# yuz1wan/unified_video_action

Measured on AMD Instinct MI355X. Metric: train samples/sec (video+action step) at 1/2/4/8 MI355X; loss parity, higher is better.
Workload: dtype bf16; 1 GPU; pusht_video: PushT video_model (BASELINE configs[1]); step = frame select+resize -> KL-VAE encode (8 frames) -> mar_base MAR fwd/bwd (N=1024) -> diffusion loss -> backward -> fused AdamW + EMA -> LR step; dropout 0.1; model=UVA mar_base + KL-VAE f16, global_batch=32, seq_len=1024, parallelism=dp1

## Files before the change

include/uva_hip.h:

```cpp
#ifndef UVA_HIP_H
#define UVA_HIP_H
#include <hip/hip_runtime_api.h>

#ifdef __cplusplus
extern "C" {
#endif

#define UVA_DT_F32 0
#define UVA_DT_BF16 1
#define UVA_ACT_NONE 0
#define UVA_ACT_GELU 1
#define UVA_ACT_SILU 2
#define UVA_ACT_RELU 3

int uva_gemm(int in_dtype, int out_dtype, int ta, int tb, const void* A, const void* B, void* C, int M, int N,
             int K, long long lda, long long ldb, long long ldc, int batch, int batch_inner, long long sAo,
             long long sAi, long long sBo, long long sBi, long long sCo, long long sCi, const float* bias,
             const void* residual, long long ldr, long long sRo, long long sRi, void* aux, int act, float alpha,
             float beta, float drop_p, unsigned long long drop_seed, int res_dtype, const void* gate,
             long long ldg, int gate_dtype, int force_generic, float* workspace, long long ws_floats,
             hipStream_t stream);

long long uva_gemm_plan(int in_dtype, int ta, int tb, int M, int N, int K, int batch, int gn_prologue,
                        long long ws_floats);
int uva_gemm_set_persist(int on);
int uva_gemm4_set(int on, int force);
int uva_gemm8w_set(int on, int mode);
int uva_linear_gelu_drop(const void* X, const void* W, const float* bias, void* pre_out, void* out, int M, int N, int K,
                         float drop_p, unsigned long long seed, const void* plane, hipStream_t stream);
int uva_linear_drop_res(const void* X, const void* W, const float* bias, const float* R, float* out, int M, int N,
                        int K, float drop_p, unsigned long long seed, const void* plane, hipStream_t stream);
int uva_linear_dgelu_drop(const void* dY, const void* Wt, const void* pre, void* dpre, float* dbias, int accum_bias,
                          float* part, int M, int N, int K, float drop_p, unsigned long long seed, const void* plane,
                          hipStream_t stream);
int uva_layernorm_bwd_drop(const float* x, const float* w, const void* dy, const float* mean, const float* rstd,
                           const float* dx_base, float* dx, float* dw, float* db, int accum_wb, void* drop_out,
                           float drop_p, unsigned long long seed, float* dbias, int accum_dbias, float* workspace,
                           int rows, int D, hipStream_t stream);
long long uva_dropout_plane_words(long long n);
int uva_dropout_plane(void* plane, long long n, float drop_p, unsigned long long seed, hipStream_t stream);
long long uva_gemm4_plan(int M, int N, int K);
long long uva_gemm4_plan_tt(int M, int N, int K, long long ws_floats);
int uva_conv2d(int dtype, const void* in, const void* w, void* out, const float* bias, const void* residual, int Nimg,
               int Hin, int Win, int Ci, int Co, int ks, int stride, int pad_t, int pad_l, int Hout, int Wout,
               const float* gn_scale, const float* gn_shift, int gn_silu, int act, float* gn_part,
               int force_generic, hipStream_t stream);
int uva_pool4x4_cwh(int dtype, const void* in, void* out, int n, int C, hipStream_t stream);
int uva_pool4x4_relu_bwd(int dtype, const void* post, int gdtype, const void* gpool, void* dpre, int n, int C,
                         hipStream_t stream);
int uva_im2col3x3(int dtype, const void* in, void* cols, int n, int H, int W, int Ci, hipStream_t stream);
int uva_im2col3x3_tc(int dtype, const void* in, void* cols, int n, int H, int W, int Ci, hipStream_t stream);
int uva_pad_nhwc(int dtype, const void* in, void* out, int n, int H, int W, int C, int G, hipStream_t stream);
int uva_conv3x3_dw_scatter_add(const float* part, float* grad, int Co, int Ci, hipStream_t stream);
int uva_conv3x3_weight_layout(const float* w, int out_dtype, void* out, int Co, int Ci, int mode, hipStream_t stream);
int uva_conv3x3_halo_bn(int Nimg, int H, int W, int Ci, int Co);
int uva_conv3x3_halo(const void* in, const void* w, void* out, const float* bias, const void* residual, int Nimg,
                     int H, int W, int Ci, int Co, const float* gn_scale, const float* gn_shift, int gn_silu,
                     float* gn_part, hipStream_t stream);
int uva_conv3x3s2_ok(int Nimg, int Hin, int Win, int Ci, int Co);
int uva_conv3x3s2_halo(const void* in, const void* w, void* out, const float* bias, int Nimg, int Hin, int Win,
                       int Ci, int Co, float* gn_part, hipStream_t stream);
int uva_conv_in8(const void* in, const void* w, void* out, const float* bias, int Nimg, int H, int W,
                 float* gn_part, hipStream_t stream);

int uva_layernorm_fwd(int in_dtype, int out_dtype, const void* x, const float* w, const float* b, const void* scale,
                      const void* shift, long long ldm, void* y, float* mean, float* rstd, int rows, int D, float eps,
                      hipStream_t stream);
int uva_layernorm_bwd(int in_dtype, int out_dtype, const void* x, const float* w, const float* b, const void* scale,
                      long long ldm,
                      const void* dy, int dy_dtype, const float* mean, const float* rstd, const float* dx_base, float* dx,
                      int accum, void* dscale,
                      void* dshift, float* dw, float* db, int accum_wb, float* workspace, int rows, int D,
                      hipStream_t stream);
long long uva_layernorm_bwd_workspace(int rows, int D);

int uva_colsum(int dtype, const void* in, long long ld, float* out, int rows, int cols, int accum, float* workspace,
               hipStream_t stream);
long long uva_colsum_workspace(int rows, int cols);

int uva_softmax_fwd(int dtype, const void* S, void* P, void* Pd, long long rows, int L, float scale, float drop_p,
                    unsigned long long seed, hipStream_t stream);
int uva_softmax_bwd(int dtype, const void* P, const void* dPd, void* dS, long long rows, int L, float scale,
                    float drop_p, unsigned long long seed, hipStream_t stream);

int uva_cast(int sdt, const void* src, long long lds, int ddt, void* dst, long long ldd, long long rows, int cols,
             hipStream_t stream);
int uva_act_fwd(int xdt, const void* x, int ydt, void* y, long long n, int act, hipStream_t stream);
int uva_transpose_bf16(const void* src, void* dst, int rows, int cols, hipStream_t stream);
int uva_act_drop_fwd(int xdt, const void* x, int ydt, void* y, int rdt, const void* residual, long long n, int act,
                     float drop_p, unsigned long long seed, hipStream_t stream);
int uva_act_bwd(int pdt, const void* pre, int gdt, const void* dy, long long ld_dy, int xdt, void* dx,
                long long ld_dx, long long rows, int cols, int act, float drop_p, unsigned long long seed, int accum,
                hipStream_t stream);
int uva_act_bwd_bias(int pdt, const void* pre, int gdt, const void* dy, long long ld_dy, int xdt, void* dx,
                     long long ld_dx, long long rows, int cols, int act, float drop_p, unsigned long long seed,
                     int accum, float* dbias, int accum_bias, float* workspace, hipStream_t stream);
long long uva_act_bwd_bias_workspace(long long rows, int cols);
int uva_gate_bwd(const float* dout, int hdt, const void* h, int gtdt, const void* gate, long long ldg, int dhdt,
                 void* dh, void* dgate, long long rows, int cols, hipStream_t stream);
int uva_fill(float* p, long long n, float v, hipStream_t stream);

int uva_q_sample(const float* x0, const float* noise, const long long* t, const float* const* tables, int xdt,
                 void* xt, int rows, int C, hipStream_t stream);
int uva_timestep_features(const long long* t, const float* freqs, int odt, void* out, int rows, int half,
                          hipStream_t stream);
int uva_diffusion_loss(const float* x0, const float* noise, const long long* t, int odt, const void* out,
                       long long ld_out, const float* const* tables, float* loss_row, float* dl, int rows, int C,
                       hipStream_t stream);
int uva_weighted_mean(const float* l, const float* w, int n, float* res, hipStream_t stream);
int uva_loss_grad(const float* dl, const float* w, const float* wsum, const float* g_up, int ddt, void* dout,
                  long long ld, int rows, int C2, hipStream_t stream);

int uva_p_sample_step(int odt, const void* out, long long ld_out, const float* x, const float* noise,
                      const float* coef, float* x_new, int xdt, void* x_net, int clip, int rows, int C,
                      hipStream_t stream);

int uva_sampler_linear(int ln, const void* A, long long lda, const float* lnw, const float* lnb, const void* shift,
                       const void* scale, long long ldm, float eps, const void* W, const float* bias, int act,
                       const void* gate, long long ldg, const float* res, long long ldr, int odt, void* out,
                       long long ldo, int R, int N, int K, hipStream_t stream);

long long uva_sampler_persistent_workspace(int W);
int uva_sampler_persistent(int R, int C, int W, int depth, int S, int clip, float eps, const void* w1, const float* b1,
                           const void* w2, const float* b2, const float* lnw, const float* lnb, const void* win,
                           const float* bin, const void* wf, const float* bfin, const void* mod, long long ldmod,
                           const float* coef, const float* noise, const float* x0, float* x_out, void* work,
                           long long work_bytes, hipStream_t stream);
int uva_sampler_persistent_status(const void* work, unsigned* flag, hipStream_t stream);
int uva_sampler_persistent_test_hook(int no_publish);

int uva_adamw_ema(float* p, const float* g, float* m, float* v, float* ema, void* p_bf16, long long n,
                  long long n_decay, float lr, float b1, float b2, float eps, float wd, int step, float grad_scale,
                  float ema_decay, hipStream_t stream);
int uva_ema_update(float* ema, const float* p, long long n, float decay, hipStream_t stream);

long long uva_attn_fp8_workspace(int B, int N, int H);
int uva_attn_quant_fp8(void* qkv, void* workspace, int B, int N, int H, hipStream_t stream);
int uva_attn_fwd_fp8(const void* workspace, void* out, float* lse2, const void* mask, int B, int N, int H, float scale,
                     float drop_p, hipStream_t stream);

long long uva_attn_mask_bytes(int B, int N, int H);
long long uva_attn_bwd_workspace(int B, int N, int H, float drop_p);
int uva_attn_dropmask(void* mask, int B, int N, int H, float drop_p, unsigned long long seed, hipStream_t stream);
int uva_attn_fwd(const void* qkv, void* out, float* lse2, const void* mask, int B, int N, int H, float scale,
                 float drop_p, hipStream_t stream);
int uva_attn_bwd(const void* qkv, const void* out, const void* dout, const float* lse2, const void* mask, float* Dvec,
                 void* dqkv, void* workspace, int B, int N, int H, float scale, float drop_p, hipStream_t stream);
int uva_attn_bwd_bias(const void* qkv, const void* out, const void* dout, const float* lse2, const void* mask,
                      float* Dvec, void* dqkv, float* dbias, int accum, float* part, int B, int N, int H, float scale,
                      float drop_p, hipStream_t stream);

int uva_attn_hd_supported(int head_dim);
int uva_attn_fwd_hd(const void* qkv, void* out, float* lse2, const void* mask, int B, int N, int H, int head_dim,
                    float scale, float drop_p, hipStream_t stream);
long long uva_attn_bwd_hd_part_floats(int B, int N, int H, int head_dim);
int uva_attn_bwd_hd(const void* qkv, const void* out, const void* dout, const float* lse2, const void* mask,
                    float* Dvec, void* dqkv, float* dbias, int accum, float* part, int B, int N, int H, int head_dim,
                    float scale, float drop_p, hipStream_t stream);

int uva_resize_select(const float* img, int B, int T, int Hin, int Win, const int* sel, int nsel, int odt, void* out,
                      int Cpad, hipStream_t stream);
long long uva_groupnorm_workspace(int Nimg, int HW);
int uva_groupnorm_stats(int dtype, const void* x, int Nimg, int HW, int C, const float* gamma, const float* beta,
                        float eps, float* scale, float* shift, float* workspace, hipStream_t stream);
int uva_groupnorm_finalize_tiles(const float* part, int Nimg, int HW, int C, int tile_rows, const float* gamma,
                                 const float* beta, float eps, float* scale, float* shift, hipStream_t stream);
int uva_groupnorm_apply(const void* x, const float* scale, const float* shift, void* y, int Nimg, int HW, int C,
                        int do_silu, hipStream_t stream);
int uva_upsample_nearest2x(int dtype, const void* x, void* y, int n, int H, int W, int C, hipStream_t stream);
int uva_pusht_augment(const float* img, float* out, const float* params, int B, int T, int C, int S, int crop_size,
                      hipStream_t stream);
int uva_video_augment(const float* img, float* out, float* scratch, const float* params, int B, int T, int S,
                      hipStream_t stream);
int uva_posterior_sample(int mdt, const void* moments, const float* eps, float* z, int Nimg, float scale,
                         hipStream_t stream);

#ifdef __cplusplus
}
#endif
#endif
```

unified_video_action_amd/csrc/attention.hip:

```cpp
#include "common.h"

#ifndef UVA_ATT_PIPE
#define UVA_ATT_PIPE 0
#endif
#ifndef UVA_ATT_PIPE_DQ
#define UVA_ATT_PIPE_DQ 0
#endif
#ifndef UVA_ATT_PRIO
#define UVA_ATT_PRIO 1
#endif
#ifndef UVA_ATT_PRIO_BWD
#define UVA_ATT_PRIO_BWD 0
#endif
#define ATT_PRIO_HI() do { if (UVA_ATT_PRIO) __builtin_amdgcn_s_setprio(1); } while (0)
#define ATT_PRIO_LO() do { if (UVA_ATT_PRIO) __builtin_amdgcn_s_setprio(0); } while (0)
#define ATT_PRIO_HI_BWD() do { if (UVA_ATT_PRIO_BWD) __builtin_amdgcn_s_setprio(1); } while (0)
#define ATT_PRIO_LO_BWD() do { if (UVA_ATT_PRIO_BWD) __builtin_amdgcn_s_setprio(0); } while (0)
#define AT_LD 80
#define AT_TILE (64 * AT_LD)

__device__ __forceinline__ bf16x8 lds_row_frag(const bf16* lds, int row0, int ks) {
  const int l = threadIdx.x & 63;
  return *(const bf16x8*)(lds + (row0 + (l & 15)) * AT_LD + ks * 32 + 8 * (l >> 4));
}
// ... 690 lines not shown
#pragma unroll
    for (int i = 0; i < 8; ++i) {
      __builtin_amdgcn_sched_group_barrier(0x008, 1, 2);
      __builtin_amdgcn_sched_group_barrier(0x002, 10, 2);
    }
    __builtin_amdgcn_sched_barrier(0);
    dqk(1);
#else
    ATT_PRIO_HI_BWD();
#pragma unroll
    for (int ks = 0; ks < 2; ++ks)
#pragma unroll
      for (int kt = 0; kt < 4; ++kt) {
        const bf16x8 ka = lds_row_frag(sK[cur], kt * 16, ks);
        const bf16x8 va = lds_row_frag(sV[cur], kt * 16, ks);
#pragma unroll
        for (int qt = 0; qt < 2; ++qt) {
          s[kt][qt] = mfma16(ka, qf[qt][ks], s[kt][qt]);
          dp[kt][qt] = mfma16(va, of[qt][ks], dp[kt][qt]);
        }
      }
    ATT_PRIO_LO_BWD();
#pragma unroll
    for (int qt = 0; qt < 2; ++qt)
#pragma unroll
      for (int kt = 0; kt < 4; ++kt)
#pragma unroll
        for (int r = 0; r < 4; ++r) {
          const float p = exp2_fast(fmaf(s[kt][qt][r], c, -L[qt]));
          float dpt = dp[kt][qt][r];
          if (DROP) dpt = keep_bfe(dpt, mw[qt], kt * 4 + r);
          s[kt][qt][r] = p * (dpt - Dq[qt]);
        }
    ATT_PRIO_HI_BWD();
#pragma unroll
    for (int ks = 0; ks < 2; ++ks) {
      bf16x8 sb[2];
#pragma unroll
      for (int qt = 0; qt < 2; ++qt) sb[qt] = pack_pi(s[2 * ks][qt], s[2 * ks + 1][qt]);
#pragma unroll
      for (int dt = 0; dt < 4; ++dt) {
        const bf16x8 ka = lds_tr_frag(sK[cur], 32 * ks, 32 * ks + 16, dt * 16);
#pragma unroll
        for (int qt = 0; qt < 2; ++qt) dq[dt][qt] = mfma16(ka, sb[qt], dq[dt][qt]);
      }
    }
    ATT_PRIO_LO_BWD();
#endif
    if (more) {
      stage_store(sK[cur ^ 1], rk);
      stage_store(sV[cur ^ 1], rv);
      if (DROP) { mw[0] = mwn[0]; mw[1] = mwn[1]; }
    }
    lds_barrier();
    cur ^= 1;
  }
  if (cpart) {
    float* red = (float*)&sK[0][0];
#pragma unroll
    for (int dt = 0; dt < 4; ++dt)
#pragma unroll
      for (int r = 0; r < 4; ++r) {
        float sq = 0.f;
#pragma unroll
        for (int qt = 0; qt < 2; ++qt)
          sq += q0 + qt * 16 + li < N ? (float)(bf16)(dq[dt][qt][r] * scale) : 0.f;
        sq = row16_sum(sq);
        if (li == 0) red[w * 64 + dt * 16 + 4 * g + r] = sq;
      }
    __syncthreads();
    if (threadIdx.x < 64) {
      const int t = threadIdx.x;
      const float v = (red[t] + red[64 + t]) + (red[128 + t] + red[192 + t]);
      const long long rowp = (long long)b * gridDim.x + bx;
      cpart[rowp * (3LL * H * 64) + h * 64 + t] = v;
    }
  }
#pragma unroll
  for (int qt = 0; qt < 2; ++qt) {
    const int q = q0 + qt * 16 + li;
    if (q >= N) continue;
    bf16* qrow = dqkv + ((long long)b * N + q) * ld + h * 64;
#pragma unroll
    for (int dt = 0; dt < 4; ++dt) {
      bf16x4 a = {(bf16)(dq[dt][qt][0] * scale), (bf16)(dq[dt][qt][1] * scale), (bf16)(dq[dt][qt][2] * scale),
                  (bf16)(dq[dt][qt][3] * scale)};
      *(bf16x4*)(qrow + dt * 16 + 4 * g) = a;
    }
  }
}

extern "C" long long uva_attn_mask_bytes(int B, int N, int H) {
  return 2LL * B * H * (long long)N * (N / 64) * 8;
}

extern "C" long long uva_attn_bwd_workspace(int B, int N, int H, float drop_p) {
  (void)B; (void)N; (void)H; (void)drop_p;
  return 0;
}

extern "C" int uva_attn_dropmask(void* mask, int B, int N, int H, float drop_p, unsigned long long seed,
                                 hipStream_t s) {
  if (N % 64 != 0 || !(drop_p > 0.f) || mask == nullptr) return (int)hipErrorInvalidValue;
  uint32_t th;
  float ds;
  uva_drop_params(drop_p, &th, &ds);
  const int nt = N / 64;
  uint64_t* MQ = (uint64_t*)mask;
  uint64_t* MK = MQ + (long long)B * H * N * nt;
  const long long waves = (long long)B * H * nt * ((nt + MASK_TPW - 1) / MASK_TPW);
  if (waves > 0x7FFFFFFFLL) return (int)hipErrorInvalidValue;
  attn_mask_kernel<<<dim3((unsigned)((waves + 3) / 4)), 256, 0, s>>>(MQ, MK, N, nt, waves, th, seed);
  UVA_LAUNCH_CHECK();
  return 0;
}

extern "C" int uva_attn_fwd(const void* qkv, void* out, float* lse2, const void* mask, int B, int N, int H,
                            float scale, float drop_p, hipStream_t s) {
  if (N % 64 != 0) return (int)hipErrorInvalidValue;
  const bool drop = drop_p > 0.f;
  if (drop && mask == nullptr) return (int)hipErrorInvalidValue;
  uint32_t th;
  float ds;
  uva_drop_params(drop_p, &th, &ds);
  dim3 grid((N + 127) / 128, B * H);
  const float c = scale * 1.4426950408889634f;
  const uint64_t* MQ = drop ? (const uint64_t*)mask : nullptr;
  if (drop)
    attn_fwd_kernel<true, 64, 3><<<grid, 256, 0, s>>>((const bf16*)qkv, (bf16*)out, lse2, MQ, N, H, c, ds);
  else
    attn_fwd_kernel<false, 64, 3><<<grid, 256, 0, s>>>((const bf16*)qkv, (bf16*)out, lse2, nullptr, N, H, c, 1.0f);
  UVA_LAUNCH_CHECK();
  return 0;
}

static int attn_bwd_launch(const void* qkv, const void* out, const void* dout, const float* lse2, const void* mask,
                           float* Dvec, void* dqkv, int B, int N, int H, float scale, float drop_p, float* cpart,
                           hipStream_t s);

extern "C" int uva_attn_bwd(const void* qkv, const void* out, const void* dout, const float* lse2, const void* mask,
                            float* Dvec, void* dqkv, void* workspace, int B, int N, int H, float scale, float drop_p,
                            hipStream_t s) {
  (void)workspace;
  return attn_bwd_launch(qkv, out, dout, lse2, mask, Dvec, dqkv, B, N, H, scale, drop_p, nullptr, s);
}

int uva_colsum_final_launch(const float* part, int nrows, int cols, float* out, int accum, hipStream_t s);

extern "C" int uva_attn_bwd_bias(const void* qkv, const void* out, const void* dout, const float* lse2,
                                 const void* mask, float* Dvec, void* dqkv, float* dbias, int accum, float* part, int B,
                                 int N, int H, float scale, float drop_p, hipStream_t s) {
  if (!dbias || !part) return (int)hipErrorInvalidValue;
  int r = attn_bwd_launch(qkv, out, dout, lse2, mask, Dvec, dqkv, B, N, H, scale, drop_p, part, s);
  if (r) return r;
  return uva_colsum_final_launch(part, B * ((N + 127) / 128), 3 * H * 64, dbias, accum, s);
}

static int attn_bwd_launch(const void* qkv, const void* out, const void* dout, const float* lse2, const void* mask,
                           float* Dvec, void* dqkv, int B, int N, int H, float scale, float drop_p, float* cpart,
                           hipStream_t s) {
  if (N % 64 != 0) return (int)hipErrorInvalidValue;
  const bool drop = drop_p > 0.f;
  if (drop && mask == nullptr) return (int)hipErrorInvalidValue;
  uint32_t th;
  float ds;
  uva_drop_params(drop_p, &th, &ds);
  const long long rows = (long long)B * N * H;
  (void)rows;
  const int nt = N / 64;
  const uint64_t* MQ = (const uint64_t*)mask;
  const uint64_t* MK = drop ? MQ + (long long)B * H * N * nt : nullptr;
  const bf16* dO = (const bf16*)dout;
  dim3 grid((N + 127) / 128, B * H);
  const float c = scale * 1.4426950408889634f;
  const float sk = scale * ds;
  const bf16* O = (const bf16*)out;
  if (drop) {
    attn_bwd_dq_kernel<true><<<grid, 256, 0, s>>>((const bf16*)qkv, dO, O, lse2, Dvec, MQ, (bf16*)dqkv, N, H, sk, c,
                                                  1.0f / ds, cpart);
    attn_bwd_dkdv_kernel<true><<<grid, 256, 0, s>>>((const bf16*)qkv, dO, lse2, Dvec, MK, (bf16*)dqkv, N, H, sk, c, ds,
                                                    cpart);
  } else {
    attn_bwd_dq_kernel<false><<<grid, 256, 0, s>>>((const bf16*)qkv, dO, O, lse2, Dvec, nullptr, (bf16*)dqkv, N, H,
                                                   sk, c, 1.0f, cpart);
    attn_bwd_dkdv_kernel<false><<<grid, 256, 0, s>>>((const bf16*)qkv, dO, lse2, Dvec, nullptr, (bf16*)dqkv, N, H,
                                                     sk, c, ds, cpart);
  }
  UVA_LAUNCH_CHECK();
  return 0;
}
```

unified_video_action_amd/csrc/attention_hd.hip:

```cpp
#include "common.h"

namespace {

template <int HD> struct HdCfg;
template <> struct HdCfg<80> { static constexpr int KS = 3, DT = 5, LD = 112; };
template <> struct HdCfg<128> { static constexpr int KS = 4, DT = 8, LD = 144; };

template <int LD>
__device__ __forceinline__ bf16x8 row_frag(const bf16* lds, int row0, int ks) {
  const int l = threadIdx.x & 63;
  return *(const bf16x8*)(lds + (row0 + (l & 15)) * LD + ks * 32 + 8 * (l >> 4));
}

template <int LD>
__device__ __forceinline__ bf16x8 tr_frag(const bf16* lds, int rowA, int rowB, int col0) {
  const int l = threadIdx.x & 63, g = l >> 4, q = (l >> 2) & 3, p = l & 3;
  const bf16* a0 = lds + (rowA + 4 * g + q) * LD + col0 + 4 * p;
  const bf16* a1 = lds + (rowB + 4 * g + q) * LD + col0 + 4 * p;
  s16x4 lo = __builtin_amdgcn_ds_read_tr16_b64_v4i16(LDS_PTR(s16x4, a0));
  s16x4 hi = __builtin_amdgcn_ds_read_tr16_b64_v4i16(LDS_PTR(s16x4, a1));
  s16x8 v = {lo[0], lo[1], lo[2], lo[3], hi[0], hi[1], hi[2], hi[3]};
  return __builtin_bit_cast(bf16x8, v);
}

// ... 428 lines not shown
    for (int ks = 0; ks < 2; ++ks) {
      const bf16x8 pb = pack_pi(s[2 * ks], s[2 * ks + 1]);
      const bf16x8 sb = pack_pi(dp[2 * ks], dp[2 * ks + 1]);
#pragma unroll
      for (int dt = 0; dt < DT; ++dt) {
        const bf16x8 oa = tr_frag<LD>(sO[cur], 32 * ks, 32 * ks + 16, dt * 16);
        const bf16x8 qa = tr_frag<LD>(sQ[cur], 32 * ks, 32 * ks + 16, dt * 16);
        dv[dt] = mfma16(oa, pb, dv[dt]);
        dk[dt] = mfma16(qa, sb, dk[dt]);
      }
    }
    if (more) {
      rq.store(sQ[cur ^ 1]);
      ro.store(sO[cur ^ 1]);
      if (threadIdx.x < 64) { sL[cur ^ 1][threadIdx.x] = nl; sD[cur ^ 1][threadIdx.x] = nd; }
      if (DROP) mw = mwn;
    }
    __syncthreads();
    cur ^= 1;
  }
  if (cpart) {
    float* red = (float*)&sQ[0][0];
#pragma unroll
    for (int dt = 0; dt < DT; ++dt)
#pragma unroll
      for (int r = 0; r < 4; ++r) {
        float sk = ok ? (float)(bf16)(dk[dt][r] * scale) : 0.f;
        float sv = ok ? (float)(bf16)(dv[dt][r] * vsc) : 0.f;
        sk = row16_sum(sk);
        sv = row16_sum(sv);
        if (li == 0) {
          red[w * 2 * HD + dt * 16 + 4 * g + r] = sk;
          red[w * 2 * HD + HD + dt * 16 + 4 * g + r] = sv;
        }
      }
    __syncthreads();
    if (threadIdx.x < 2 * HD) {
      const int t = threadIdx.x;
      float v = 0.f;
#pragma unroll
      for (int ww = 0; ww < 8; ++ww) v += red[ww * 2 * HD + t];
      const long long rowp = (long long)b * gridDim.x + bx;
      cpart[rowp * (3LL * H * HD) + (t < HD ? H * HD + t : 2 * H * HD + t - HD) + h * HD] = v;
    }
  }
  if (ok) {
    bf16* krow = dqkv + ((long long)b * N + row) * ld + H * HD + h * HD;
    bf16* vrow = krow + H * HD;
#pragma unroll
    for (int dt = 0; dt < DT; ++dt) {
      bf16x4 a = {(bf16)(dk[dt][0] * scale), (bf16)(dk[dt][1] * scale), (bf16)(dk[dt][2] * scale),
                  (bf16)(dk[dt][3] * scale)};
      bf16x4 e = {(bf16)(dv[dt][0] * vsc), (bf16)(dv[dt][1] * vsc), (bf16)(dv[dt][2] * vsc),
                  (bf16)(dv[dt][3] * vsc)};
      *(bf16x4*)(krow + dt * 16 + 4 * g) = a;
      *(bf16x4*)(vrow + dt * 16 + 4 * g) = e;
    }
  }
}

template <int HD>
int fwd_launch(const void* qkv, void* out, float* lse2, const void* mask, int B, int N, int H, float scale, bool drop,
               float ds, hipStream_t s) {
  dim3 grid((N + 127) / 128, B * H);
  const float c = scale * 1.4426950408889634f;
  constexpr int lds = 4 * 64 * HdCfg<HD>::LD * (int)sizeof(bf16);
  static const bool once = [] {
    (void)hipFuncSetAttribute((const void*)attn_hd_fwd_kernel<HD, true>, hipFuncAttributeMaxDynamicSharedMemorySize, lds);
    (void)hipFuncSetAttribute((const void*)attn_hd_fwd_kernel<HD, false>, hipFuncAttributeMaxDynamicSharedMemorySize, lds);
    return true;
  }();
  (void)once;
  if (drop)
    attn_hd_fwd_kernel<HD, true><<<grid, 256, lds, s>>>((const bf16*)qkv, (bf16*)out, lse2, (const uint64_t*)mask, N, H,
                                                      c, ds);
  else
    attn_hd_fwd_kernel<HD, false><<<grid, 256, lds, s>>>((const bf16*)qkv, (bf16*)out, lse2, nullptr, N, H, c, 1.0f);
  UVA_LAUNCH_CHECK();
  return 0;
}

template <int HD>
int bwd_launch(const void* qkv, const void* out, const void* dout, const float* lse2, const void* mask, float* Dvec,
               void* dqkv, float* cpart, int B, int N, int H, float scale, bool drop, float ds, hipStream_t s) {
  const int nt = N / 64;
  const uint64_t* MQ = (const uint64_t*)mask;
  const uint64_t* MK = drop ? MQ + (long long)B * H * N * nt : nullptr;
  dim3 grid((N + 127) / 128, B * H);
  const float c = scale * 1.4426950408889634f;
  const float sk = scale * ds;
  constexpr int lds = 4 * 64 * HdCfg<HD>::LD * (int)sizeof(bf16);
  constexpr int ldsk = lds + 4 * 64 * (int)sizeof(float);
  static const bool once = [] {
    (void)hipFuncSetAttribute((const void*)attn_hd_bwd_dq_kernel<HD, true>, hipFuncAttributeMaxDynamicSharedMemorySize, lds);
    (void)hipFuncSetAttribute((const void*)attn_hd_bwd_dq_kernel<HD, false>, hipFuncAttributeMaxDynamicSharedMemorySize, lds);
    (void)hipFuncSetAttribute((const void*)attn_hd_bwd_dkdv_kernel<HD, true>, hipFuncAttributeMaxDynamicSharedMemorySize, ldsk);
    (void)hipFuncSetAttribute((const void*)attn_hd_bwd_dkdv_kernel<HD, false>, hipFuncAttributeMaxDynamicSharedMemorySize, ldsk);
    return true;
  }();
  (void)once;
  if (drop) {
    attn_hd_bwd_dq_kernel<HD, true><<<grid, 512, lds, s>>>((const bf16*)qkv, (const bf16*)dout, (const bf16*)out, lse2,
                                                         Dvec, MQ, (bf16*)dqkv, N, H, sk, c, 1.0f / ds, cpart);
    attn_hd_bwd_dkdv_kernel<HD, true><<<grid, 512, ldsk, s>>>((const bf16*)qkv, (const bf16*)dout, lse2, Dvec, MK,
                                                           (bf16*)dqkv, N, H, sk, c, ds, cpart);
  } else {
    attn_hd_bwd_dq_kernel<HD, false><<<grid, 512, lds, s>>>((const bf16*)qkv, (const bf16*)dout, (const bf16*)out, lse2,
                                                          Dvec, nullptr, (bf16*)dqkv, N, H, sk, c, 1.0f, cpart);
    attn_hd_bwd_dkdv_kernel<HD, false><<<grid, 512, ldsk, s>>>((const bf16*)qkv, (const bf16*)dout, lse2, Dvec, nullptr,
                                                            (bf16*)dqkv, N, H, sk, c, ds, cpart);
  }
  UVA_LAUNCH_CHECK();
  return 0;
}

}

int uva_colsum_final_launch(const float* part, int nrows, int cols, float* out, int accum, hipStream_t s);

extern "C" int uva_attn_hd_supported(int head_dim) { return head_dim == 80 || head_dim == 128; }

extern "C" long long uva_attn_bwd_hd_part_floats(int B, int N, int H, int head_dim) {
  return (long long)B * ((N + 127) / 128) * 3LL * H * head_dim;
}

extern "C" int uva_attn_fwd_hd(const void* qkv, void* out, float* lse2, const void* mask, int B, int N, int H,
                               int head_dim, float scale, float drop_p, hipStream_t s) {
  if (!uva_attn_hd_supported(head_dim) || N <= 0 || N % 64 != 0 || B <= 0 || H <= 0)
    return (int)hipErrorInvalidValue;
  const bool drop = drop_p > 0.f;
  if (drop && mask == nullptr) return (int)hipErrorInvalidValue;
  uint32_t th;
  float ds;
  uva_drop_params(drop_p, &th, &ds);
  return head_dim == 80 ? fwd_launch<80>(qkv, out, lse2, mask, B, N, H, scale, drop, ds, s)
                        : fwd_launch<128>(qkv, out, lse2, mask, B, N, H, scale, drop, ds, s);
}

extern "C" int uva_attn_bwd_hd(const void* qkv, const void* out, const void* dout, const float* lse2, const void* mask,
                               float* Dvec, void* dqkv, float* dbias, int accum, float* part, int B, int N, int H,
                               int head_dim, float scale, float drop_p, hipStream_t s) {
  if (!uva_attn_hd_supported(head_dim) || N <= 0 || N % 64 != 0 || B <= 0 || H <= 0)
    return (int)hipErrorInvalidValue;
  const bool drop = drop_p > 0.f;
  if (drop && mask == nullptr) return (int)hipErrorInvalidValue;
  if (dbias && !part) return (int)hipErrorInvalidValue;
  uint32_t th;
  float ds;
  uva_drop_params(drop_p, &th, &ds);
  float* cpart = dbias ? part : nullptr;
  const int r = head_dim == 80
                    ? bwd_launch<80>(qkv, out, dout, lse2, mask, Dvec, dqkv, cpart, B, N, H, scale, drop, ds, s)
                    : bwd_launch<128>(qkv, out, dout, lse2, mask, Dvec, dqkv, cpart, B, N, H, scale, drop, ds, s);
  if (r || !dbias) return r;
  return uva_colsum_final_launch(part, B * ((N + 127) / 128), 3 * H * head_dim, dbias, accum, s);
}
```

unified_video_action_amd/csrc/common.h:

```cpp
#pragma once
#include <hip/hip_runtime.h>
#include <math.h>
#include <stdint.h>

typedef __bf16 bf16;
typedef __attribute__((ext_vector_type(8))) __bf16 bf16x8;
typedef __attribute__((ext_vector_type(4))) __bf16 bf16x4;
typedef __attribute__((ext_vector_type(2))) float f32x2;
typedef __attribute__((ext_vector_type(4))) float f32x4;
typedef __attribute__((ext_vector_type(16))) float f32x16;
typedef __attribute__((ext_vector_type(4))) short s16x4;
typedef __attribute__((ext_vector_type(8))) short s16x8;

#define UVA_DT_F32 0
#define UVA_DT_BF16 1

#define LDS_PTR(T, p) ((__attribute__((address_space(3))) T*)(p))

__device__ __forceinline__ float to_f32(float x) { return x; }
__device__ __forceinline__ float to_f32(bf16 x) { return (float)x; }
template <typename T> __device__ __forceinline__ T from_f32(float x);
template <> __device__ __forceinline__ float from_f32<float>(float x) { return x; }
template <> __device__ __forceinline__ bf16 from_f32<bf16>(float x) { return (bf16)x; }

__device__ __forceinline__ float wave_sum(float v) {
#pragma unroll
  for (int o = 32; o > 0; o >>= 1) v += __shfl_xor(v, o, 64);
  return v;
}
__device__ __forceinline__ float wave_max(float v) {
#pragma unroll
  for (int o = 32; o > 0; o >>= 1) v = fmaxf(v, __shfl_xor(v, o, 64));
  return v;
}
__device__ __forceinline__ float group16_sum(float v) {
#pragma unroll
  for (int o = 8; o > 0; o >>= 1) v += __shfl_xor(v, o, 64);
  return v;
}
__device__ __forceinline__ float group16_max(float v) {
#pragma unroll
  for (int o = 8; o > 0; o >>= 1) v = fmaxf(v, __shfl_xor(v, o, 64));
  return v;
}

__host__ __device__ __forceinline__ uint32_t drop_key(uint64_t seed) {
  uint32_t k = (uint32_t)seed ^ (((uint32_t)(seed >> 32)) * 0x9E3779B1u);
  k ^= k >> 16;
  k *= 0x7feb352du;
  k ^= k >> 15;
  return k;
}
__host__ __device__ __forceinline__ uint32_t drop_first(uint32_t key, uint64_t pair) {
  return (uint32_t)pair ^ (key + __builtin_rotateleft32((uint32_t)(pair >> 32), 11));
}
__host__ __device__ __forceinline__ uint32_t drop_mix(uint32_t x) {
  x ^= x >> 16;
  x *= 0x7feb352du;
  x ^= x >> 15;
  x *= 0x846ca68bu;
  x ^= x >> 16;
  return x;
}
__host__ __device__ __forceinline__ uint32_t drop_hash(uint32_t key, uint64_t pair) {
  return drop_mix(drop_first(key, pair));
}
__host__ __device__ __forceinline__ bool dropout_keep(uint64_t seed, uint64_t idx, uint32_t thresh) {
  const uint32_t h = drop_hash(drop_key(seed), idx >> 1);
  return ((idx & 1) ? (h >> 16) : (h & 0xFFFFu)) >= thresh;
}
__device__ __forceinline__ void dropout_keep2(uint64_t seed, uint64_t idx_even, uint32_t thresh, bool& k0, bool& k1) {
  const uint32_t h = drop_hash(drop_key(seed), idx_even >> 1);
  k0 = (h & 0xFFFFu) >= thresh;
  k1 = (h >> 16) >= thresh;
}

static inline void uva_drop_params(float p, uint32_t* thresh, float* scale) {
  if (!(p > 0.f)) {
    *thresh = 0;
    *scale = 1.0f;
    return;
  }
  long t = lrintf(p * 65536.0f);
  if (t < 1) t = 1;
  if (t > 65535) t = 65535;
  *thresh = (uint32_t)t;
  *scale = 65536.0f / (float)(65536 - t);
}

#define ACT_NONE 0
#define ACT_GELU 1
#define ACT_SILU 2
#define ACT_RELU 3

__device__ __forceinline__ float erf_fast(float x) {
  const float ax = fabsf(x);
  const float t = __builtin_amdgcn_rcpf(fmaf(0.3275911f, ax, 1.0f));
  float p = fmaf(1.061405429f, t, -1.453152027f);
  p = fmaf(p, t, 1.421413741f);
  p = fmaf(p, t, -0.284496736f);
  p = fmaf(p, t, 0.254829592f);
  p *= t;
  const float e = __builtin_amdgcn_exp2f(-1.4426950408889634f * ax * ax);
  return copysignf(fmaf(-p, e, 1.0f), x);
}
__device__ __forceinline__ float gelu_erf(float x) { return 0.5f * x * (1.0f + erf_fast(x * 0.70710678118654752f)); }
__device__ __forceinline__ float gelu_erf_grad(float x) {
  const float e = __builtin_amdgcn_exp2f(-0.72134752044448170f * x * x);
  const float ax = fabsf(x) * 0.70710678118654752f;
  const float t = __builtin_amdgcn_rcpf(fmaf(0.3275911f, ax, 1.0f));
  float p = fmaf(1.061405429f, t, -1.453152027f);
  p = fmaf(p, t, 1.421413741f);
  p = fmaf(p, t, -0.284496736f);
  p = fmaf(p, t, 0.254829592f);
  p *= t;
  const float erf_ = copysignf(fmaf(-p, e, 1.0f), x);
  return fmaf(x, 0.39894228040143268f * e, fmaf(0.5f, erf_, 0.5f));
}
__device__ __forceinline__ float sigmoid_fast(float x) {
  return __builtin_amdgcn_rcpf(1.0f + __builtin_amdgcn_exp2f(-1.4426950408889634f * x));
}
__device__ __forceinline__ float silu(float x) { return x * sigmoid_fast(x); }
__device__ __forceinline__ float silu_grad(float x) {
  const float s = sigmoid_fast(x);
  return s * (1.0f + x * (1.0f - s));
}
__device__ __forceinline__ float apply_act(int act, float x) {
  switch (act) {
    case ACT_GELU: return gelu_erf(x);
    case ACT_SILU: return silu(x);
    case ACT_RELU: return x > 0.f ? x : 0.f;
    default: return x;
  }
}
__device__ __forceinline__ float act_grad(int act, float x) {
  switch (act) {
    case ACT_GELU: return gelu_erf_grad(x);
    case ACT_SILU: return silu_grad(x);
    case ACT_RELU: return x > 0.f ? 1.f : 0.f;
    default: return 1.f;
  }
}

__device__ __forceinline__ int xcd_remap(int bid, int nblk) {
  const int q = nblk / 8, r = nblk % 8, x = bid % 8;
  return (x < r ? x * (q + 1) : r * (q + 1) + (x - r) * q) + bid / 8;
}
__device__ __forceinline__ void xcd_grid2(int& bx, int& by) {
  const int gx = gridDim.x, T = gx * gridDim.y;
  const int L = blockIdx.y * gx + blockIdx.x;
  const int q = T / 8, r = T % 8, x = L % 8;
  const int Lp = (x < r ? x * (q + 1) : r * (q + 1) + (x - r) * q) + L / 8;
  bx = Lp % gx;
  by = Lp / gx;
}

__device__ __forceinline__ float row16_sum(float v) {
  v += __builtin_bit_cast(float, __builtin_amdgcn_update_dpp(0, __builtin_bit_cast(int, v), 0xB1, 0xF, 0xF, false));
  v += __builtin_bit_cast(float, __builtin_amdgcn_update_dpp(0, __builtin_bit_cast(int, v), 0x4E, 0xF, 0xF, false));
  v += __builtin_bit_cast(float, __builtin_amdgcn_update_dpp(0, __builtin_bit_cast(int, v), 0x124, 0xF, 0xF, false));
  v += __builtin_bit_cast(float, __builtin_amdgcn_update_dpp(0, __builtin_bit_cast(int, v), 0x128, 0xF, 0xF, false));
  return v;
}

__device__ __forceinline__ void lds_barrier() {
  asm volatile("s_waitcnt lgkmcnt(0)" ::: "memory");
  __builtin_amdgcn_s_barrier();
  asm volatile("" ::: "memory");
// ... 5 lines not shown
```

unified_video_action_amd/csrc/elementwise.hip:

```cpp
#include "common.h"

__device__ __forceinline__ float ldx(const void* p, int dt, long long i) {
  return dt == UVA_DT_BF16 ? (float)((const bf16*)p)[i] : ((const float*)p)[i];
}
__device__ __forceinline__ void stx(void* p, int dt, long long i, float v) {
  if (dt == UVA_DT_BF16) ((bf16*)p)[i] = (bf16)v;
  else ((float*)p)[i] = v;
}

#define GRID_STRIDE(i, n) for (long long i = (long long)blockIdx.x * blockDim.x + threadIdx.x; i < (n); i += (long long)gridDim.x * blockDim.x)

static inline dim3 ew_grid(long long n) {
  long long b = (n + 255) / 256;
  if (b > 8192) b = 8192;
  if (b < 1) b = 1;
  return dim3((unsigned)b);
}

__global__ void cast_kernel(const void* src, int sdt, long long lds, void* dst, int ddt, long long ldd, long long rows,
                            int cols) {
  GRID_STRIDE(i, rows * cols) {
    long long r = i / cols, c = i % cols;
    stx(dst, ddt, r * ldd + c, ldx(src, sdt, r * lds + c));
  }
}

__global__ void cast_f32_bf16_vec(const float* __restrict__ src, bf16* __restrict__ dst, long long n8) {
  GRID_STRIDE(i, n8) {
    float4 a = ((const float4*)src)[2 * i], b = ((const float4*)src)[2 * i + 1];
    bf16x8 o = {(bf16)a.x, (bf16)a.y, (bf16)a.z, (bf16)a.w, (bf16)b.x, (bf16)b.y, (bf16)b.z, (bf16)b.w};
    ((bf16x8*)dst)[i] = o;
  }
}

__global__ void act_fwd_kernel(const void* x, int xdt, void* y, int ydt, long long n, int act) {
  GRID_STRIDE(i, n) stx(y, ydt, i, apply_act(act, ldx(x, xdt, i)));
}

__global__ void act_bwd_kernel(const void* pre, int pdt, const void* dy, int gdt, void* dx, int xdt, long long rows,
                               int cols, long long ld_dy, long long ld_dx, int act, uint32_t thresh, float dscale,
                               uint64_t seed, int accum) {
  GRID_STRIDE(i, rows * (long long)cols) {
    long long r = i / cols, c = i % cols;
    float g = ldx(dy, gdt, r * ld_dy + c);
    if (thresh) g = dropout_keep(seed, (uint64_t)i, thresh) ? g * dscale : 0.f;
    if (act != ACT_NONE) g *= act_grad(act, ldx(pre, pdt, i));
    long long o = r * ld_dx + c;
    if (accum) g += ldx(dx, xdt, o);
    stx(dx, xdt, o, g);
  }
}

template <typename T>
__device__ __forceinline__ void ld8(const T* p, float (&v)[8]) {
  if constexpr (sizeof(T) == 2) {
    const bf16x8 x = *(const bf16x8*)p;
#pragma unroll
    for (int e = 0; e < 8; ++e) v[e] = (float)x[e];
  } else {
    const float4 a = *(const float4*)p, b = *(const float4*)(p + 4);
    v[0] = a.x; v[1] = a.y; v[2] = a.z; v[3] = a.w; v[4] = b.x; v[5] = b.y; v[6] = b.z; v[7] = b.w;
  }
}
template <typename T>
__device__ __forceinline__ void st8(T* p, const float (&v)[8]) {
  if constexpr (sizeof(T) == 2) {
    bf16x8 x;
#pragma unroll
    for (int e = 0; e < 8; ++e) x[e] = (bf16)v[e];
    *(bf16x8*)p = x;
  } else {
    *(float4*)p = make_float4(v[0], v[1], v[2], v[3]);
    *(float4*)(p + 4) = make_float4(v[4], v[5], v[6], v[7]);
  }
}

template <typename GT, typename XT>
__global__ void act_bwd_vec_kernel(const void* pre, int pdt, const GT* __restrict__ dy, XT* __restrict__ dx, int rows,
                                   int cols, long long ld_dy, long long ld_dx, int act, uint32_t thresh, float dscale,
                                   uint64_t seed, int accum) {
  const unsigned c8n = (unsigned)cols >> 3;
  const unsigned n8 = (unsigned)rows * c8n;
  for (unsigned i = blockIdx.x * blockDim.x + threadIdx.x; i < n8; i += gridDim.x * blockDim.x) {
    const unsigned r = i / c8n, c0 = (i - r * c8n) * 8;
    float g[8];
    ld8<GT>(dy + (long long)r * ld_dy + c0, g);
    if (thresh) {
      const uint64_t e0 = (uint64_t)r * cols + c0;
#pragma unroll
      for (int e = 0; e < 8; e += 2) {
        bool k0, k1;
        dropout_keep2(seed, e0 + e, thresh, k0, k1);
        g[e] = k0 ? g[e] * dscale : 0.f;
        g[e + 1] = k1 ? g[e + 1] * dscale : 0.f;
      }
    }
    if (act != ACT_NONE) {
      float pv[8];
      const long long pi = (long long)r * cols + c0;
      if (pdt == UVA_DT_BF16) ld8<bf16>((const bf16*)pre + pi, pv);
      else ld8<float>((const float*)pre + pi, pv);
#pragma unroll
      for (int e = 0; e < 8; ++e) g[e] *= act_grad(act, pv[e]);
    }
    XT* o = dx + (long long)r * ld_dx + c0;
    if (accum) {
      float prev[8];
      ld8<XT>(o, prev);
#pragma unroll
      for (int e = 0; e < 8; ++e) g[e] += prev[e];
    }
    st8<XT>(o, g);
  }
}

#define COLSUM_RPB 128
template <typename GT, typename XT, bool STORE>
__global__ __launch_bounds__(256) void act_bwd_colsum_kernel(const void* pre, int pdt, const GT* __restrict__ dy,
                                                             XT* __restrict__ dx, int rows, int cols, long long ld_dy,
                                                             long long ld_dx, int act, uint32_t thresh, float dscale,
                                                             uint64_t seed, int accum, float* __restrict__ part) {
  __shared__ float red[8][32 * 8 + 4];
  const int cg = threadIdx.x & 31, rl = threadIdx.x >> 5;
  const int c0 = (blockIdx.x * 32 + cg) * 8;
  const int r0 = blockIdx.y * COLSUM_RPB, r1 = min(rows, r0 + COLSUM_RPB);
  float s[8] = {0.f, 0.f, 0.f, 0.f, 0.f, 0.f, 0.f, 0.f};
  if (c0 < cols) {
#pragma unroll 4
    for (int r = r0 + rl; r < r1; r += 8) {
      float g[8];
      ld8<GT>(dy + (long long)r * ld_dy + c0, g);
      if (STORE) {
        if (thresh) {
          const uint64_t e0 = (uint64_t)r * cols + c0;
#pragma unroll
          for (int e = 0; e < 8; e += 2) {
            bool k0, k1;
            dropout_keep2(seed, e0 + e, thresh, k0, k1);
            g[e] = k0 ? g[e] * dscale : 0.f;
            g[e + 1] = k1 ? g[e + 1] * dscale : 0.f;
          }
        }
        if (act != ACT_NONE) {
          float pv[8];
          const long long pi = (long long)r * cols + c0;
          if (pdt == UVA_DT_BF16) ld8<bf16>((const bf16*)pre + pi, pv);
          else ld8<float>((const float*)pre + pi, pv);
#pragma unroll
          for (int e = 0; e < 8; ++e) g[e] *= act_grad(act, pv[e]);
        }
        XT* o = dx + (long long)r * ld_dx + c0;
        if (accum) {
          float prev[8];
          ld8<XT>(o, prev);
#pragma unroll
          for (int e = 0; e < 8; ++e) g[e] += prev[e];
        }
        st8<XT>(o, g);
#pragma unroll
        for (int e = 0; e < 8; ++e) s[e] += to_f32(from_f32<XT>(g[e]));
      } else {
#pragma unroll
        for (int e = 0; e < 8; ++e) s[e] += g[e];
      }
    }
  }
#pragma unroll
  for (int e = 0; e < 8; ++e) red[rl][cg * 8 + e] = s[e];
  __syncthreads();
  const int c = blockIdx.x * 256 + threadIdx.x;
  if (c < cols) {
    float t = 0.f;
#pragma unroll
    for (int j = 0; j < 8; ++j) t += red[j][threadIdx.x];
    part[(long long)blockIdx.y * cols + c] = t;
  }
}

__global__ __launch_bounds__(256) void colsum_final_kernel(const float* __restrict__ part, int nrows, int cols,
                                                           float* __restrict__ out, int accum) {
  __shared__ float red[8][33];
  const int cl = threadIdx.x & 31, rl = threadIdx.x >> 5;
  const int c = blockIdx.x * 32 + cl;
  float s = 0.f;
  if (c < cols) {
#pragma unroll 8
    for (int j = rl; j < nrows; j += 8) s += part[(long long)j * cols + c];
  }
  red[rl][cl] = s;
  __syncthreads();
  if (rl == 0 && c < cols) {
    float t = 0.f;
#pragma unroll
    for (int j = 0; j < 8; ++j) t += red[j][cl];
    out[c] = accum ? out[c] + t : t;
  }
}

extern "C" long long uva_act_bwd_bias_workspace(long long rows, int cols) {
  return (rows + COLSUM_RPB - 1) / COLSUM_RPB * (long long)cols;
}

extern "C" int uva_act_bwd_bias(int pdt, const void* pre, int gdt, const void* dy, long long ld_dy, int xdt, void* dx,
                                long long ld_dx, long long rows, int cols, int act, float drop_p,
                                unsigned long long seed, int accum, float* dbias, int accum_bias, float* workspace,
                                hipStream_t s) {
  if (rows <= 0 || cols <= 0) return 0;
  if (cols % 8 || ld_dy % 8 || ld_dx % 8 || rows >= (1ll << 31) ||
      (((uintptr_t)dy | (uintptr_t)dx | (uintptr_t)pre) % 16) || !dbias || !workspace)
    return (int)hipErrorInvalidValue;
  uint32_t th;
  float ds;
  uva_drop_params(drop_p, &th, &ds);
  const int nch = (int)((rows + COLSUM_RPB - 1) / COLSUM_RPB);
  dim3 g1((cols / 8 + 31) / 32, nch);
#define AB(GT, XT)                                                                                               \
  act_bwd_colsum_kernel<GT, XT, true><<<g1, 256, 0, s>>>(pre, pdt, (const GT*)dy, (XT*)dx, (int)rows, cols, ld_dy, \
                                                         ld_dx, act, th, ds, seed, accum, workspace)
  if (gdt == UVA_DT_BF16 && xdt == UVA_DT_BF16) AB(bf16, bf16);
  else if (gdt == UVA_DT_BF16) AB(bf16, float);
  else if (xdt == UVA_DT_BF16) AB(float, bf16);
  else AB(float, float);
#undef AB
  UVA_LAUNCH_CHECK();
  colsum_final_kernel<<<dim3((cols + 31) / 32), 256, 0, s>>>(workspace, nch, cols, dbias, accum_bias);
  UVA_LAUNCH_CHECK();
  return 0;
}

int uva_colsum_final_launch(const float* part, int nrows, int cols, float* out, int accum, hipStream_t s) {
  colsum_final_kernel<<<dim3((cols + 31) / 32), 256, 0, s>>>(part, nrows, cols, out, accum);
  return (int)hipGetLastError();
}

int uva_colsum_vec(int dtype, const void* in, long long ld, float* out, int rows, int cols, int accum,
                   float* workspace, hipStream_t s) {
  if (cols % 8 || ld % 8 || ((uintptr_t)in % 16) || !workspace || rows < 2 * COLSUM_RPB) return 0;
  const int nch = (rows + COLSUM_RPB - 1) / COLSUM_RPB;
  dim3 g1((cols / 8 + 31) / 32, nch);
  if (dtype == UVA_DT_BF16)
    act_bwd_colsum_kernel<bf16, bf16, false><<<g1, 256, 0, s>>>(nullptr, 0, (const bf16*)in, nullptr, rows, cols, ld,
                                                                0, 0, 0, 1.f, 0, 0, workspace);
  else
    act_bwd_colsum_kernel<float, float, false><<<g1, 256, 0, s>>>(nullptr, 0, (const float*)in, nullptr, rows, cols,
                                                                  ld, 0, 0, 0, 1.f, 0, 0, workspace);
  if (hipGetLastError() != hipSuccess) return -1;
  colsum_final_kernel<<<dim3((cols + 31) / 32), 256, 0, s>>>(workspace, nch, cols, out, accum);
  if (hipGetLastError() != hipSuccess) return -1;
  return 1;
}

__global__ void gate_bwd_kernel(const float* dout, const void* h, int hdt, const void* gate, int gtdt, long long ldg,
                                void* dh, int dhdt, void* dgate, long long rows, int cols) {
  GRID_STRIDE(i, rows * (long long)cols) {
    long long r = i / cols, c = i % cols;
    float d = dout[i];
    float g = ldx(gate, gtdt, r * ldg + c);
    stx(dgate, gtdt, r * ldg + c, d * ldx(h, hdt, i));
    stx(dh, dhdt, i, d * g);
  }
}

__global__ void fill_kernel(float* p, long long n, float v) {
  GRID_STRIDE(i, n) p[i] = v;
}

extern "C" int uva_cast(int sdt, const void* src, long long lds, int ddt, void* dst, long long ldd, long long rows,
                        int cols, hipStream_t s) {
  long long n = rows * cols;
  if (n <= 0) return 0;
  if (sdt == UVA_DT_F32 && ddt == UVA_DT_BF16 && lds == cols && ldd == cols && n % 8 == 0 &&
      ((uintptr_t)src % 16 == 0) && ((uintptr_t)dst % 16 == 0)) {
    cast_f32_bf16_vec<<<ew_grid(n / 8), 256, 0, s>>>((const float*)src, (bf16*)dst, n / 8);
  } else {
    cast_kernel<<<ew_grid(n), 256, 0, s>>>(src, sdt, lds, dst, ddt, ldd, rows, cols);
  }
  UVA_LAUNCH_CHECK();
  return 0;
}

__global__ __launch_bounds__(256) void transpose_bf16_kernel(const bf16* __restrict__ src, bf16* __restrict__ dst,
                                                             int rows, int cols) {
  __shared__ bf16 t[64][64 + 8];
  const int r0 = blockIdx.y * 64, c0 = blockIdx.x * 64;
  const int tid = threadIdx.x;
#pragma unroll
  for (int i = 0; i < 2; ++i) {
    const int id = tid + i * 256, rr = id >> 3, cc = (id & 7) * 8;
    const int r = r0 + rr, c = c0 + cc;
    bf16x8 v;
    if (r < rows && c + 8 <= cols) {
      v = *(const bf16x8*)(src + (long long)r * cols + c);
    } else {
#pragma unroll
      for (int e = 0; e < 8; ++e) v[e] = (r < rows && c + e < cols) ? src[(long long)r * cols + c + e] : (bf16)0.f;
    }
#pragma unroll
    for (int e = 0; e < 8; ++e) t[rr][cc + e] = v[e];
  }
  __syncthreads();
#pragma unroll
  for (int i = 0; i < 2; ++i) {
    const int id = tid + i * 256, cc = id >> 3, rr = (id & 7) * 8;
    const int c = c0 + cc, r = r0 + rr;
    bf16x8 v;
#pragma unroll
    for (int e = 0; e < 8; ++e) v[e] = t[rr + e][cc];
    if (c < cols && r + 8 <= rows) {
      *(bf16x8*)(dst + (long long)c * rows + r) = v;
    } else if (c < cols) {
#pragma unroll
      for (int e = 0; e < 8; ++e)
        if (r + e < rows) dst[(long long)c * rows + r + e] = v[e];
    }
  }
}

extern "C" int uva_transpose_bf16(const void* src, void* dst, int rows, int cols, hipStream_t s) {
  if (rows <= 0 || cols <= 0) return 0;
  if ((rows % 8) || (cols % 8) || (((uintptr_t)src | (uintptr_t)dst) % 16)) return (int)hipErrorInvalidValue;
  transpose_bf16_kernel<<<dim3((cols + 63) / 64, (rows + 63) / 64), 256, 0, s>>>((const bf16*)src, (bf16*)dst, rows,
                                                                                 cols);
  UVA_LAUNCH_CHECK();
  return 0;
}

template <typename TX, typename TY, typename TR>
__global__ __launch_bounds__(256) void act_drop_fwd_kernel(const TX* __restrict__ x, TY* __restrict__ y,
                                                           const TR* __restrict__ res, long long n8, int act,
                                                           uint32_t thresh, float dscale, uint64_t seed) {
  GRID_STRIDE(i, n8) {
    float v[8], r[8];
    ld8<TX>(x + i * 8, v);
    if (res) ld8<TR>(res + i * 8, r);
    switch (act) {
      case ACT_GELU:
#pragma unroll
        for (int e = 0; e < 8; ++e) v[e] = gelu_erf(v[e]);
        break;
      case ACT_SILU:
#pragma unroll
        for (int e = 0; e < 8; ++e) v[e] = silu(v[e]);
        break;
      case ACT_RELU:
#pragma unroll
        for (int e = 0; e < 8; ++e) v[e] = v[e] > 0.f ? v[e] : 0.f;
        break;
      default:
        break;
    }
    if (thresh) {
      bool keep[8];
#pragma unroll
      for (int e = 0; e < 8; e += 2) dropout_keep2(seed, (uint64_t)(i * 8 + e), thresh, keep[e], keep[e + 1]);
#pragma unroll
      for (int e = 0; e < 8; ++e) v[e] = keep[e] ? v[e] * dscale : 0.f;
    }
    if (res) {
#pragma unroll
      for (int e = 0; e < 8; ++e) v[e] += r[e];
    }
    st8<TY>(y + i * 8, v);
  }
}

extern "C" int uva_act_drop_fwd(int xdt, const void* x, int ydt, void* y, int rdt, const void* residual, long long n,
                                int act, float drop_p, unsigned long long seed, hipStream_t s) {
  if (n <= 0) return 0;
  if (n % 8 || (((uintptr_t)x | (uintptr_t)y | (uintptr_t)residual) % 16)) return (int)hipErrorInvalidValue;
  uint32_t th;
  float ds;
  uva_drop_params(drop_p, &th, &ds);
  const long long n8 = n / 8;
#define ADF(TX, TY, TR) \
  act_drop_fwd_kernel<TX, TY, TR><<<ew_grid(n8), 256, 0, s>>>((const TX*)x, (TY*)y, (const TR*)residual, n8, act, th, ds, seed)
  if (xdt == UVA_DT_BF16 && ydt == UVA_DT_BF16 && (!residual || rdt == UVA_DT_BF16)) ADF(bf16, bf16, bf16);
  else if (xdt == UVA_DT_BF16 && ydt == UVA_DT_F32 && (!residual || rdt == UVA_DT_F32)) ADF(bf16, float, float);
  else if (xdt == UVA_DT_F32 && ydt == UVA_DT_F32 && (!residual || rdt == UVA_DT_F32)) ADF(float, float, float);
  else return (int)hipErrorInvalidValue;
#undef ADF
  UVA_LAUNCH_CHECK();
  return 0;
}

__global__ __launch_bounds__(256) void drop_plane_kernel(uint32_t* __restrict__ plane, long long nwords, uint32_t key,
                                                         uint32_t thresh) {
  GRID_STRIDE(w, nwords) {
    const uint32_t f0 = drop_first(key, (uint64_t)w * 16);
    uint32_t bits = 0;
#pragma unroll
    for (int j = 0; j < 16; ++j) {
      const uint32_t h = drop_mix(f0 ^ (uint32_t)j);
      bits |= ((h & 0xFFFFu) >= thresh ? 1u : 0u) << (2 * j);
      bits |= ((h >> 16) >= thresh ? 1u : 0u) << (2 * j + 1);
    }
    plane[w] = bits;
  }
}

extern "C" long long uva_dropout_plane_words(long long n) { return (n + 31) / 32; }

extern "C" int uva_dropout_plane(void* plane, long long n, float drop_p, unsigned long long seed, hipStream_t s) {
  if (n <= 0) return 0;
  if (!plane || ((uintptr_t)plane % 4)) return (int)hipErrorInvalidValue;
  uint32_t th;
  float ds;
  uva_drop_params(drop_p, &th, &ds);
  const long long nw = (n + 31) / 32;
  drop_plane_kernel<<<ew_grid(nw), 256, 0, s>>>((uint32_t*)plane, nw, drop_key(seed), th);
  UVA_LAUNCH_CHECK();
  return 0;
}

extern "C" int uva_act_fwd(int xdt, const void* x, int ydt, void* y, long long n, int act, hipStream_t s) {
  if (n <= 0) return 0;
  act_fwd_kernel<<<ew_grid(n), 256, 0, s>>>(x, xdt, y, ydt, n, act);
  UVA_LAUNCH_CHECK();
  return 0;
}

extern "C" int uva_act_bwd(int pdt, const void* pre, int gdt, const void* dy, long long ld_dy, int xdt, void* dx,
                           long long ld_dx, long long rows, int cols, int act, float drop_p, unsigned long long seed,
                           int accum, hipStream_t s) {
  long long n = rows * cols;
  if (n <= 0) return 0;
  uint32_t th;
  float ds;
  uva_drop_params(drop_p, &th, &ds);
  const bool vec = cols % 8 == 0 && ld_dy % 8 == 0 && ld_dx % 8 == 0 && n / 8 < (1ll << 31) &&
                   (((uintptr_t)dy | (uintptr_t)dx | (uintptr_t)pre) % 16 == 0);
  if (vec) {
    const long long n8 = n / 8;
#define AB(GT, XT)                                                                                              \
  act_bwd_vec_kernel<GT, XT><<<ew_grid(n8), 256, 0, s>>>(pre, pdt, (const GT*)dy, (XT*)dx, (int)rows, cols, ld_dy, \
                                                         ld_dx, act, th, ds, seed, accum)
    if (gdt == UVA_DT_BF16 && xdt == UVA_DT_BF16) AB(bf16, bf16);
    else if (gdt == UVA_DT_BF16) AB(bf16, float);
    else if (xdt == UVA_DT_BF16) AB(float, bf16);
    else AB(float, float);
#undef AB
  } else {
    act_bwd_kernel<<<ew_grid(n), 256, 0, s>>>(pre, pdt, dy, gdt, dx, xdt, rows, cols, ld_dy, ld_dx, act, th, ds, seed,
                                              accum);
  }
  UVA_LAUNCH_CHECK();
  return 0;
}

extern "C" int uva_gate_bwd(const float* dout, int hdt, const void* h, int gtdt, const void* gate, long long ldg,
                            int dhdt, void* dh, void* dgate, long long rows, int cols, hipStream_t s) {
  long long n = rows * cols;
  if (n <= 0) return 0;
  gate_bwd_kernel<<<ew_grid(n), 256, 0, s>>>(dout, h, hdt, gate, gtdt, ldg, dh, dhdt, dgate, rows, cols);
  UVA_LAUNCH_CHECK();
  return 0;
}

extern "C" int uva_fill(float* p, long long n, float v, hipStream_t s) {
  if (n <= 0) return 0;
  fill_kernel<<<ew_grid(n), 256, 0, s>>>(p, n, v);
  UVA_LAUNCH_CHECK();
  return 0;
}
```

unified_video_action_amd/csrc/gemm8w.hip:

```cpp
#include "common.h"

#include <algorithm>
#include <type_traits>

typedef __attribute__((ext_vector_type(4))) unsigned u32x4;

#ifndef UVA_G8_DBG
#define UVA_G8_DBG 0
#endif
#ifndef UVA_G8_PREFETCH
#define UVA_G8_PREFETCH 1
#endif

namespace {

template <int FM_, int FN_, int NW_>
struct G8Cfg {
  static constexpr int FM = FM_, FN = FN_, NW = NW_;
  static constexpr int WM = NW / 2, WN = 2;
  static constexpr int BM = 16 * FM * WM, BN = 16 * FN * WN;
  static constexpr int GA = BM / (8 * NW), GB = BN / (8 * NW), G = GA + GB;
  static constexpr int A_BYTES = BM * 128, REGION = (BM + BN) * 128, RING = 2 * REGION;
  static_assert(GA * 8 * NW == BM && GB * 8 * NW == BN, "DMA split");
};
// ... 527 lines not shown
  const long long tiles = (long long)((M + G::BM - 1) / G::BM) * tn;
  const int grid = (int)std::min<long long>(tiles, (long long)g8_cus() * (8 / NW));
  const int lds = G::RING + (NW == 8 && ep.bias ? tn * G::BN * 4 : 0);
  static bool attr = false;
  if (!attr) {
    (void)hipFuncSetAttribute((const void*)gemm_8w<4, FN, NW, EPI, NDEF, TC, DM>,
                              hipFuncAttributeMaxDynamicSharedMemorySize, NW == 8 ? 163840 : G::RING);
    attr = true;
  }
  const int w1ok = (M % G::BM == 0) && (N % G::BN == 0);
  gemm_8w<4, FN, NW, EPI, NDEF, TC, DM><<<dim3(grid), 64 * NW, lds, s>>>((const bf16*)A, (const bf16*)B, (TC*)C, M, N,
                                                                       K, lda, ldb, ldc, ep, w1ok, 1, K, 0);
  UVA_LAUNCH_CHECK();
  return 0;
}

struct G8Split {
  int splits, kps, grid;
};
static G8Split g8_plan_tt(int M, int N, int K, long long ws_floats, bool need_ws) {
  G8Split p{0, 0, 0};
  if (K % 128 != 0 || K < 256 || M < 256 || N < 192) return p;
  const int cus = g8_cus();
  const long long tiles = (long long)((M + 255) / 256) * ((N + 191) / 192);
  int splits = (int)std::max<long long>(1, (cus + tiles / 2) / tiles);
  if (splits > K / 256) splits = K / 256;
  while (splits > 1 && (long long)splits * M * N > ws_floats) --splits;
  if (splits == 1 && need_ws && (long long)M * N > ws_floats) return p;
  int kps = K;
  for (; splits > 1; --splits) {
    kps = ((K + splits - 1) / splits + 127) / 128 * 128;
    const int sp = (K + kps - 1) / kps;
    if (K - (sp - 1) * kps >= 256) {
      splits = sp;
      break;
    }
  }
  if (splits <= 1) {
    splits = 1;
    kps = K;
  }
  p.splits = splits;
  p.kps = kps;
  p.grid = (int)std::min<long long>(tiles * splits, cus);
  return p;
}
static bool g8_nw4(int epi) { return (g_gemm8w_mode & 32) || (!(g_gemm8w_mode & 64) && epi == 3); }
static int g8_part_rows(int M) { return g8_nw4(3) ? (M + 127) / 128 * 2 : (M + 255) / 256 * 4; }

template <int FN, int EPI, int NDEF, typename TC, int NW = 8>
static int g8_launch(const void* A, const void* B, void* C, int M, int N, int K, int lda, int ldb, int ldc,
                     const G8Epi& ep, hipStream_t s) {
  if constexpr (EPI == 0) {
    return g8_launch1<FN, EPI, NDEF, TC, 0, NW>(A, B, C, M, N, K, lda, ldb, ldc, ep, s);
  } else {
    if (!ep.thresh) return g8_launch1<FN, EPI, NDEF, TC, 0, NW>(A, B, C, M, N, K, lda, ldb, ldc, ep, s);
    if (ep.plane) return g8_launch1<FN, EPI, NDEF, TC, 2, NW>(A, B, C, M, N, K, lda, ldb, ldc, ep, s);
    return g8_launch1<FN, EPI, NDEF, TC, 1, NW>(A, B, C, M, N, K, lda, ldb, ldc, ep, s);
  }
}

template <int EPI, typename TC>
static int g8_dispatch(const void* A, const void* B, void* C, int M, int N, int K, int lda, int ldb, int ldc,
                       const G8Epi& ep, hipStream_t s) {
  const int nd = (EPI == 0 && sizeof(TC) == 4) ? 0 : (g_gemm8w_mode >> 2) & 7;
#define G8L(FN_, ND_) g8_launch<FN_, EPI, ND_, TC>(A, B, C, M, N, K, lda, ldb, ldc, ep, s)
  if (g_gemm8w_mode & 32) return g8_launch<6, EPI, 0, TC, 4>(A, B, C, M, N, K, lda, ldb, ldc, ep, s);
  if (g_gemm8w_mode & 2) return (nd && K / 128 >= 3) ? G8L(4, 4) : G8L(4, 0);
  return G8L(6, 0);
#undef G8L
}

static bool g8_ok(const void* A, const void* B, const void* C, int M, int N, int K, long long lda, long long ldb,
                  long long ldc, int csize, const float* bias) {
  if (M < 256 || N < 192 || K < 256 || K % 128) return false;
  if (lda % 8 || ldb % 8 || ldc % 8 || N % 8 || lda < K || ldb < K) return false;
  if (((uintptr_t)A | (uintptr_t)B | (uintptr_t)C) % 16) return false;
  if (bias && ((uintptr_t)bias % 16)) return false;
  if (2.0 * (double)M * (double)lda >= 2147483648.0 || 2.0 * (double)N * (double)ldb >= 2147483648.0) return false;
  if ((double)M * (double)ldc * csize > (double)0x7fff0000) return false;
  const int tn = (N + 191) / 192;
  if (tn * 192 * 4 + 114688 > 163840) return false;
  return true;
}

static uint32_t g8_key(unsigned long long seed) { return drop_key(seed); }

extern "C" int uva_gemm8w_tt_try(const void* A, const void* B, float* C, int M, int N, int K, long long lda,
                                 long long ldb, long long ldc, float alpha, float beta, float* ws, long long ws_floats,
                                 int* reduce, hipStream_t s) {
  *reduce = 0;
  if (!(g_gemm8w_mode & 128)) return 0;
  if (M <= 0 || N <= 0 || K <= 0) return 0;
  if (lda % 8 || ldb % 8 || ldc % 8 || M % 8 || N % 8 || lda < M || ldb < N) return 0;
  if (((uintptr_t)A | (uintptr_t)B | (uintptr_t)C | (uintptr_t)ws) % 16) return 0;
  if (2.0 * (double)K * (double)lda >= 2147483648.0 || 2.0 * (double)K * (double)ldb >= 2147483648.0) return 0;
  const G8Split p = g8_plan_tt(M, N, K, ws ? ws_floats : 0, beta != 0.f);
  if (p.splits == 0) return 0;
  const bool direct = p.splits == 1 && beta == 0.f;
  if (direct ? (double)M * (double)ldc * 4.0 > (double)0x7fff0000
             : (double)p.splits * (double)M * (double)N * 4.0 > (double)0x7fff0000)
    return 0;
  if (!direct && !ws) return 0;
  using G = G8Cfg<4, 6, 8>;
  static bool attr = false;
  if (!attr) {
    (void)hipFuncSetAttribute((const void*)gemm_8w<4, 6, 8, 0, 0, float, 0, 1, 1>,
                              hipFuncAttributeMaxDynamicSharedMemorySize, 163840);
    attr = true;
  }
  const int w1ok = (M % G::BM == 0) && (N % G::BN == 0);
  G8Epi ep{nullptr, direct ? alpha : 1.f, nullptr, nullptr, nullptr, nullptr, 0u, 0u, 1.f};
  gemm_8w<4, 6, 8, 0, 0, float, 0, 1, 1><<<dim3(p.grid), 512, G::RING, s>>>(
      (const bf16*)A, (const bf16*)B, direct ? C : ws, M, N, K, (int)lda, (int)ldb, direct ? (int)ldc : N, ep, w1ok,
      p.splits, p.kps, (int)((long long)M * N * 4));
  UVA_LAUNCH_CHECK();
  if (!direct) *reduce = p.splits;
  return 1;
}

extern "C" int uva_gemm8w_try(int out_dtype, const void* A, const void* B, void* C, int M, int N, int K, long long lda,
                              long long ldb, long long ldc, const float* bias, float alpha, hipStream_t s) {
  if (!g_gemm8w_on) return 0;
  if (!g8_ok(A, B, C, M, N, K, lda, ldb, ldc, out_dtype == UVA_DT_BF16 ? 2 : 4, bias)) return 0;
  G8Epi ep{bias, alpha, nullptr, nullptr, nullptr, nullptr, 0u, 0u, 1.f};
  const int r = out_dtype == UVA_DT_BF16
                    ? g8_dispatch<0, bf16>(A, B, C, M, N, K, (int)lda, (int)ldb, (int)ldc, ep, s)
                    : g8_dispatch<0, float>(A, B, C, M, N, K, (int)lda, (int)ldb, (int)ldc, ep, s);
  return r ? -r : 1;
}

extern "C" int uva_gemm8w_set(int on, int mode) {
  const int prev = g_gemm8w_on | (g_gemm8w_mode << 1);
  if (on != -2) g_gemm8w_on = on;
  if (mode != -2) g_gemm8w_mode = mode;
  return prev;
}

extern "C" int uva_linear_gelu_drop(const void* X, const void* W, const float* bias, void* pre_out, void* out, int M,
                                    int N, int K, float drop_p, unsigned long long seed, const void* plane,
                                    hipStream_t s) {
  if (!g8_ok(X, W, out, M, N, K, K, K, N, 2, bias) || ((uintptr_t)pre_out % 16)) return 0;
  uint32_t th;
  float ds;
  uva_drop_params(drop_p, &th, &ds);
  if (plane && (N % 32 || !th || ((uintptr_t)plane % 4))) return (int)-hipErrorInvalidValue;
  G8Epi ep{bias, 1.f, pre_out, nullptr, nullptr, (const uint32_t*)plane, th ? g8_key(seed) : 0u, th, ds};
  const int r = g8_dispatch<1, bf16>(X, W, out, M, N, K, K, K, N, ep, s);
  return r ? -r : 1;
}

int uva_colsum_final_launch(const float* part, int nrows, int cols, float* out, int accum, hipStream_t s);

extern "C" int uva_linear_dgelu_drop(const void* dY, const void* Wt, const void* pre, void* dpre, float* dbias,
                                     int accum_bias, float* part, int M, int N, int K, float drop_p,
                                     unsigned long long seed, const void* plane, hipStream_t s) {
  if (!g8_ok(dY, Wt, dpre, M, N, K, K, K, N, 2, nullptr) || (((uintptr_t)pre | (uintptr_t)part) % 16) || !dbias)
    return 0;
  uint32_t th;
  float ds;
  uva_drop_params(drop_p, &th, &ds);
  if (plane && (N % 32 || !th || ((uintptr_t)plane % 4))) return (int)-hipErrorInvalidValue;
  G8Epi ep{nullptr, 1.f, (void*)pre, nullptr, part, (const uint32_t*)plane, th ? g8_key(seed) : 0u, th, ds};
  int r = g8_nw4(3) ? g8_launch<6, 3, 0, bf16, 4>(dY, Wt, dpre, M, N, K, K, K, N, ep, s)
                                : g8_launch<6, 3, 0, bf16>(dY, Wt, dpre, M, N, K, K, K, N, ep, s);
  if (r) return -r;
  r = uva_colsum_final_launch(part, g8_part_rows(M), N, dbias, accum_bias, s);
  return r ? -r : 1;
}

extern "C" int uva_linear_drop_res(const void* X, const void* W, const float* bias, const float* R, float* out, int M,
                                   int N, int K, float drop_p, unsigned long long seed, const void* plane,
                                   hipStream_t s) {
  if (!g8_ok(X, W, out, M, N, K, K, K, N, 4, bias) || ((uintptr_t)R % 16)) return 0;
  uint32_t th;
  float ds;
  uva_drop_params(drop_p, &th, &ds);
  if (plane && (N % 32 || !th || ((uintptr_t)plane % 4))) return (int)-hipErrorInvalidValue;
  G8Epi ep{bias, 1.f, nullptr, R, nullptr, (const uint32_t*)plane, th ? g8_key(seed) : 0u, th, ds};
  const int r = g8_dispatch<2, float>(X, W, out, M, N, K, K, K, N, ep, s);
  return r ? -r : 1;
}
```

unified_video_action_amd/csrc/norm.hip:

```cpp
#include "common.h"

template <typename T>
__device__ __forceinline__ void load_vec(const T* p, float* out, int n) {
#pragma unroll
  for (int i = 0; i < n; ++i) out[i] = to_f32(p[i]);
}

template <int VEC, typename T>
__device__ __forceinline__ void ldv(const T* p, float (&o)[VEC]) {
  if constexpr (VEC == 4 && sizeof(T) == 4) {
    float4 v = *(const float4*)p;
    o[0] = v.x; o[1] = v.y; o[2] = v.z; o[3] = v.w;
  } else if constexpr (VEC == 4 && sizeof(T) == 2) {
    bf16x4 v = *(const bf16x4*)p;
    o[0] = (float)v[0]; o[1] = (float)v[1]; o[2] = (float)v[2]; o[3] = (float)v[3];
  } else {
#pragma unroll
    for (int i = 0; i < VEC; ++i) o[i] = to_f32(p[i]);
  }
}

template <int VEC, typename T>
__device__ __forceinline__ void stv(T* p, const float (&o)[VEC]) {
  if constexpr (VEC == 4 && sizeof(T) == 4) {
    *(float4*)p = make_float4(o[0], o[1], o[2], o[3]);
  } else if constexpr (VEC == 4 && sizeof(T) == 2) {
    bf16x4 v = {(bf16)o[0], (bf16)o[1], (bf16)o[2], (bf16)o[3]};
    *(bf16x4*)p = v;
  } else {
#pragma unroll
    for (int i = 0; i < VEC; ++i) p[i] = from_f32<T>(o[i]);
  }
}

template <int VEC>
__device__ __forceinline__ int col_of(int c, int lane, int v) { return (c * 64 + lane) * VEC + v; }

template <typename TI, typename TO, int VEC, int NC>
__global__ __launch_bounds__(256) void ln_fwd(const TI* __restrict__ x, const float* __restrict__ w,
                                              const float* __restrict__ b, const TO* __restrict__ scale,
                                              const TO* __restrict__ shift, long long ldm, TO* __restrict__ y,
                                              float* __restrict__ mean_out, float* __restrict__ rstd_out, int rows,
                                              int D, float eps) {
  const int lane = threadIdx.x & 63;
  const int row = blockIdx.x * 4 + (threadIdx.x >> 6);
  if (row >= rows) return;
  const TI* xr = x + (long long)row * D;
  float v[NC][VEC];
  float s = 0.f;
#pragma unroll
  for (int c = 0; c < NC; ++c) {
    int col = col_of<VEC>(c, lane, 0);
    if (col < D) {
      ldv<VEC>(xr + col, v[c]);
    } else {
#pragma unroll
      for (int i = 0; i < VEC; ++i) v[c][i] = 0.f;
    }
#pragma unroll
    for (int i = 0; i < VEC; ++i) s += v[c][i];
  }
  const float mean = wave_sum(s) / D;
  float q = 0.f;
#pragma unroll
  for (int c = 0; c < NC; ++c)
#pragma unroll
    for (int i = 0; i < VEC; ++i) {
      int col = col_of<VEC>(c, lane, i);
      float d = (col < D) ? v[c][i] - mean : 0.f;
      q += d * d;
    }
  const float var = wave_sum(q) / D;
  const float rstd = 1.0f / sqrtf(var + eps);
  if (lane == 0) {
    mean_out[row] = mean;
    rstd_out[row] = rstd;
  }
  TO* yr = y + (long long)row * D;
#pragma unroll
  for (int c = 0; c < NC; ++c) {
    int col0 = col_of<VEC>(c, lane, 0);
    if (col0 >= D) continue;
    float o[VEC];
    float sc[VEC], sh[VEC], wv[VEC], bv[VEC];
    if (scale) {
      ldv<VEC>(scale + (long long)row * ldm + col0, sc);
      ldv<VEC>(shift + (long long)row * ldm + col0, sh);
    }
    if (w) ldv<VEC>(w + col0, wv);
    if (b) ldv<VEC>(b + col0, bv);
#pragma unroll
    for (int i = 0; i < VEC; ++i) {
      float h = (v[c][i] - mean) * rstd;
      if (w) h = h * wv[i];
      if (b) h = h + bv[i];
      if (scale) h = h * (1.0f + sc[i]) + sh[i];
      o[i] = h;
    }
    stv<VEC>(yr + col0, o);
  }
}

template <int VEC, typename T>
struct RawVec {
  T v[VEC];
};
template <int VEC, typename T>
__device__ __forceinline__ RawVec<VEC, T> ldraw(const T* p) {
  RawVec<VEC, T> r;
  if constexpr (VEC == 4 && sizeof(T) == 4) {
    *(float4*)r.v = *(const float4*)p;
  } else if constexpr (VEC == 4 && sizeof(T) == 2) {
    *(bf16x4*)r.v = *(const bf16x4*)p;
  } else {
#pragma unroll
    for (int i = 0; i < VEC; ++i) r.v[i] = p[i];
  }
  return r;
}

struct LnDrop {
  bf16* out;
  float* part;
  uint32_t key, thresh;
  float dscale;
};

template <typename TI, typename TO, int VEC, int NC, typename TD, bool DROPO = false>
__global__ __launch_bounds__(256) void ln_bwd(const TI* __restrict__ x, const float* __restrict__ w,
                                              const float* __restrict__ b, const TO* __restrict__ scale, long long ldm,
                                              const TD* __restrict__ dy, const float* __restrict__ mean_in,
                                              const float* __restrict__ rstd_in, const float* dx_base,
                                              float* dx, int accum,
                                              TO* __restrict__ dscale, TO* __restrict__ dshift,
                                              float* __restrict__ dw_part, float* __restrict__ db_part, int rows,
                                              int D, int rows_per_block, LnDrop ldrop = LnDrop{}) {
  constexpr int RW = VEC * NC * 64 > 1024 ? VEC * NC * 64 : 1024;
  __shared__ float red_w[4][RW];
  __shared__ float red_b[4][RW];
  __shared__ float red_d[DROPO ? 4 : 1][DROPO ? RW : 1];
  float pd[NC][VEC];
  if constexpr (DROPO) {
#pragma unroll
    for (int c = 0; c < NC; ++c)
#pragma unroll
      for (int i = 0; i < VEC; ++i) pd[c][i] = 0.f;
  }
  const int lane = threadIdx.x & 63, wid = threadIdx.x >> 6;
  float pw[NC][VEC], pb[NC][VEC];
#pragma unroll
  for (int c = 0; c < NC; ++c)
#pragma unroll
    for (int i = 0; i < VEC; ++i) pw[c][i] = pb[c][i] = 0.f;
// ... 25 lines not shown
      const int col0 = col_of<VEC>(c, lane, 0);
      if (col0 < D) {
        R.x[c] = ldraw<VEC>(x + (long long)row * D + col0);
        R.d[c] = ldraw<VEC>(dy + (long long)row * D + col0);
        if (addsrc) R.a[c] = ldraw<VEC>(addsrc + (long long)row * D + col0);
      }
    }
  };
  auto process = [&](int row, const Row& R, Row& L, bool pf) __attribute__((always_inline)) {
    if (pf && row + 4 < r1) load_row(row + 4, L);
    const float mean = R.mean, rstd = R.rstd;
    float xh[NC][VEC], g[NC][VEC];
    float s1 = 0.f, s2 = 0.f;
#pragma unroll
    for (int c = 0; c < NC; ++c) {
      int col0 = col_of<VEC>(c, lane, 0);
      if (col0 >= D) {
#pragma unroll
        for (int i = 0; i < VEC; ++i) xh[c][i] = g[c][i] = 0.f;
        continue;
      }
      float sc[VEC];
      if (scale) ldv<VEC>(scale + (long long)row * ldm + col0, sc);
      float ds[VEC], dsh[VEC];
#pragma unroll
      for (int i = 0; i < VEC; ++i) {
        xh[c][i] = (to_f32(R.x[c].v[i]) - mean) * rstd;
        const float dv = to_f32(R.d[c].v[i]);
        float da = dv;
        if (scale) {
          float ya = w ? xh[c][i] * wv[c][i] + (b ? bv[c][i] : 0.f) : xh[c][i];
          da = dv * (1.0f + sc[i]);
          ds[i] = dv * ya;
          dsh[i] = dv;
        }
        if (w) {
          pw[c][i] += da * xh[c][i];
          pb[c][i] += da;
          g[c][i] = da * wv[c][i];
        } else {
          g[c][i] = da;
        }
        s1 += g[c][i];
        s2 += g[c][i] * xh[c][i];
      }
      if (scale) {
        stv<VEC>(dscale + (long long)row * ldm + col0, ds);
        stv<VEC>(dshift + (long long)row * ldm + col0, dsh);
      }
    }
    const float m1 = wave_sum(s1) / D, m2 = wave_sum(s2) / D;
#pragma unroll
    for (int c = 0; c < NC; ++c) {
      int col0 = col_of<VEC>(c, lane, 0);
      if (col0 >= D) continue;
      float o[VEC];
#pragma unroll
      for (int i = 0; i < VEC; ++i) {
        float d = rstd * (g[c][i] - m1 - xh[c][i] * m2);
        o[i] = addsrc ? R.a[c].v[i] + d : d;
      }
      stv<VEC>(dx + (long long)row * D + col0, o);
      if constexpr (DROPO) {
        static_assert(VEC % 2 == 0, "pairs");
        const unsigned long long e0 = (unsigned long long)row * (unsigned)D + (unsigned)col0;
        float q[VEC];
#pragma unroll
        for (int i = 0; i < VEC; i += 2) {
          const uint32_t h = drop_hash(ldrop.key, (e0 + i) >> 1);
          q[i] = (h & 0xFFFFu) >= ldrop.thresh ? o[i] * ldrop.dscale : 0.f;
          q[i + 1] = (h >> 16) >= ldrop.thresh ? o[i + 1] * ldrop.dscale : 0.f;
        }
        bf16 qb[VEC];
#pragma unroll
        for (int i = 0; i < VEC; ++i) {
          qb[i] = (bf16)q[i];
          pd[c][i] += (float)qb[i];
        }
        if constexpr (VEC == 4) {
          bf16x4 v4 = {qb[0], qb[1], qb[2], qb[3]};
          *(bf16x4*)(ldrop.out + (long long)row * D + col0) = v4;
        } else {
#pragma unroll
          for (int i = 0; i < VEC; ++i) ldrop.out[(long long)row * D + col0 + i] = qb[i];
        }
      }
    }
  };
  Row ra, rb;
  int row = r0 + wid;
  if constexpr (NC <= 3) {
    if (row < r1) load_row(row, ra);
    for (; row < r1; row += 8) {
      process(row, ra, rb, true);
      if (row + 4 < r1) process(row + 4, rb, ra, true);
    }
  } else {
    for (; row < r1; row += 4) {
      load_row(row, ra);
      process(row, ra, rb, false);
    }
  }
  if (dw_part) {
#pragma unroll
    for (int c = 0; c < NC; ++c)
#pragma unroll
      for (int i = 0; i < VEC; ++i) {
        int col = col_of<VEC>(c, lane, i);
        if (col < D) {
          red_w[wid][col] = pw[c][i];
          red_b[wid][col] = pb[c][i];
        }
      }
    __syncthreads();
    for (int col = threadIdx.x; col < D; col += 256) {
      dw_part[(long long)blockIdx.x * D + col] = red_w[0][col] + red_w[1][col] + red_w[2][col] + red_w[3][col];
      db_part[(long long)blockIdx.x * D + col] = red_b[0][col] + red_b[1][col] + red_b[2][col] + red_b[3][col];
    }
  }
  if constexpr (DROPO) {
#pragma unroll
    for (int c = 0; c < NC; ++c)
#pragma unroll
      for (int i = 0; i < VEC; ++i) {
        const int col = col_of<VEC>(c, lane, i);
        if (col < D) red_d[wid][col] = pd[c][i];
      }
    __syncthreads();
    for (int col = threadIdx.x; col < D; col += 256)
      ldrop.part[(long long)blockIdx.x * D + col] = red_d[0][col] + red_d[1][col] + red_d[2][col] + red_d[3][col];
  }
}

template <typename T>
__global__ __launch_bounds__(256) void colsum_kernel(const T* __restrict__ in, long long ld, float* __restrict__ out,
                                                     int rows, int cols, int accum) {
  __shared__ float red[4][64];
  const int cl = threadIdx.x & 63, rl = threadIdx.x >> 6;
  const int col = blockIdx.x * 64 + cl;
  float s = 0.f;
  if (col < cols)
    for (int r = rl; r < rows; r += 4) s += to_f32(in[(long long)r * ld + col]);
  red[rl][cl] = s;
  __syncthreads();
  if (rl == 0 && col < cols) {
    float t = red[0][cl] + red[1][cl] + red[2][cl] + red[3][cl];
    out[col] = accum ? out[col] + t : t;
  }
}

__global__ __launch_bounds__(256) void colsum_partials_kernel(const float* __restrict__ p0, const float* __restrict__ p1,
                                                              float* __restrict__ o0, float* __restrict__ o1, int rows,
                                                              int cols, int accum) {
  const float* in = blockIdx.y ? p1 : p0;
  float* out = blockIdx.y ? o1 : o0;
  __shared__ float4 red[32][8];
  const int cg = threadIdx.x & 7, rl = threadIdx.x >> 3;
  const int c = blockIdx.x * 32 + cg * 4;
  float4 acc = make_float4(0.f, 0.f, 0.f, 0.f);
  if (c < cols) {
#pragma unroll 4
    for (int r = rl; r < rows; r += 32) {
      const float4 v = *(const float4*)(in + (long long)r * cols + c);
      acc.x += v.x; acc.y += v.y; acc.z += v.z; acc.w += v.w;
    }
  }
  red[rl][cg] = acc;
  __syncthreads();
  if (rl < 4 && c < cols) {
    const int cc = c + rl;
    float t = 0.f;
#pragma unroll 8
    for (int k = 0; k < 32; ++k) {
      const float4 v = red[k][cg];
      t += rl == 0 ? v.x : (rl == 1 ? v.y : (rl == 2 ? v.z : v.w));
    }
    out[cc] = accum ? out[cc] + t : t;
  }
}

static void colsum_partials(const float* p0, const float* p1, float* o0, float* o1, int rows, int cols, int accum,
                            hipStream_t stream) {
  if (cols % 4 == 0) {
    colsum_partials_kernel<<<dim3((cols + 31) / 32, p1 ? 2 : 1), 256, 0, stream>>>(p0, p1, o0, o1, rows, cols, accum);
  } else {
    colsum_kernel<float><<<dim3((cols + 63) / 64), 256, 0, stream>>>(p0, cols, o0, rows, cols, accum);
    if (p1) colsum_kernel<float><<<dim3((cols + 63) / 64), 256, 0, stream>>>(p1, cols, o1, rows, cols, accum);
  }
}

template <typename T>
__global__ __launch_bounds__(256) void colsum_part_kernel(const T* __restrict__ in, long long ld,
                                                          float* __restrict__ part, int rows, int cols,
                                                          int rows_per_block) {
  __shared__ float red[4][64];
  const int cl = threadIdx.x & 63, rl = threadIdx.x >> 6;
  const int col = blockIdx.x * 64 + cl;
  const int r0 = blockIdx.y * rows_per_block, r1 = min(rows, r0 + rows_per_block);
  float s = 0.f;
  if (col < cols)
    for (int r = r0 + rl; r < r1; r += 4) s += to_f32(in[(long long)r * ld + col]);
  red[rl][cl] = s;
  __syncthreads();
  if (rl == 0 && col < cols) part[(long long)blockIdx.y * cols + col] = red[0][cl] + red[1][cl] + red[2][cl] + red[3][cl];
}

template <typename T>
__global__ __launch_bounds__(256) void softmax_fwd_kernel(const T* __restrict__ S, T* __restrict__ P,
                                                          T* __restrict__ Pd, long long rows, int L, float scale,
                                                          uint32_t thresh, float dscale, uint64_t seed) {
  const int lane = threadIdx.x & 63;
  const long long row = (long long)blockIdx.x * 4 + (threadIdx.x >> 6);
  if (row >= rows) return;
  const T* s = S + row * L;
  float m = -INFINITY;
  for (int j = lane; j < L; j += 64) m = fmaxf(m, to_f32(s[j]) * scale);
  m = wave_max(m);
  float sum = 0.f;
  for (int j = lane; j < L; j += 64) sum += __expf(to_f32(s[j]) * scale - m);
  sum = wave_sum(sum);
  const float inv = 1.0f / sum;
  for (int j = lane; j < L; j += 64) {
    float p = __expf(to_f32(s[j]) * scale - m) * inv;
    P[row * L + j] = from_f32<T>(p);
    if (Pd) {
      float pd = dropout_keep(seed, (uint64_t)(row * L + j), thresh) ? p * dscale : 0.f;
      Pd[row * L + j] = from_f32<T>(pd);
    }
  }
}

template <typename T>
__global__ __launch_bounds__(256) void softmax_bwd_kernel(const T* __restrict__ P, const T* __restrict__ dPd,
                                                          T* __restrict__ dS, long long rows, int L, float scale,
                                                          uint32_t thresh, float dscale, uint64_t seed) {
  const int lane = threadIdx.x & 63;
  const long long row = (long long)blockIdx.x * 4 + (threadIdx.x >> 6);
  if (row >= rows) return;
  float dot = 0.f;
  for (int j = lane; j < L; j += 64) {
    float dp = to_f32(dPd[row * L + j]);
    if (thresh) dp = dropout_keep(seed, (uint64_t)(row * L + j), thresh) ? dp * dscale : 0.f;
    dot += dp * to_f32(P[row * L + j]);
  }
  dot = wave_sum(dot);
  for (int j = lane; j < L; j += 64) {
    float dp = to_f32(dPd[row * L + j]);
    if (thresh) dp = dropout_keep(seed, (uint64_t)(row * L + j), thresh) ? dp * dscale : 0.f;
    dS[row * L + j] = from_f32<T>(scale * to_f32(P[row * L + j]) * (dp - dot));
  }
}

#define DISPATCH_LNB(TI, TO, TD, ...)                                                       \
  do {                                                                                       \
    if (D == 768) {                                                                          \
      ln_bwd<TI, TO, 4, 3, TD><<<grid, 256, 0, stream>>>(__VA_ARGS__);                       \
    } else if (D % 256 == 0 && D <= 1024) {                                                  \
      ln_bwd<TI, TO, 4, 4, TD><<<grid, 256, 0, stream>>>(__VA_ARGS__);                       \
    } else if (D <= 1024) {                                                                  \
      ln_bwd<TI, TO, 1, 16, TD><<<grid, 256, 0, stream>>>(__VA_ARGS__);                      \
    } else if (D % 256 == 0 && D <= 1280) {  \
      ln_bwd<TI, TO, 4, 5, TD><<<grid, 256, 0, stream>>>(__VA_ARGS__);                       \
    } else if (D % 256 == 0 && D <= 2048) {                                                  \
      ln_bwd<TI, TO, 4, 8, TD><<<grid, 256, 0, stream>>>(__VA_ARGS__);                       \
    } else {                                                                                 \
      return (int)hipErrorInvalidValue;                                                      \
    }                                                                                        \
  } while (0)

#define DISPATCH_LN(KERNEL, TI, TO, ...)                                                    \
  do {                                                                                       \
    if (D == 768) {  \
      KERNEL<TI, TO, 4, 3><<<grid, 256, 0, stream>>>(__VA_ARGS__);                           \
    } else if (D % 256 == 0 && D <= 1024) {                                                  \
      KERNEL<TI, TO, 4, 4><<<grid, 256, 0, stream>>>(__VA_ARGS__);                           \
    } else if (D <= 1024) {                                                                  \
      KERNEL<TI, TO, 1, 16><<<grid, 256, 0, stream>>>(__VA_ARGS__);                          \
    } else if (D % 256 == 0 && D <= 1280) {  \
      KERNEL<TI, TO, 4, 5><<<grid, 256, 0, stream>>>(__VA_ARGS__);                           \
    } else if (D % 256 == 0 && D <= 2048) {                                                  \
      KERNEL<TI, TO, 4, 8><<<grid, 256, 0, stream>>>(__VA_ARGS__);                           \
    } else {                                                                                 \
      return (int)hipErrorInvalidValue;                                                      \
    }                                                                                        \
  } while (0)

extern "C" int uva_layernorm_fwd(int in_dtype, int out_dtype, const void* x, const float* w, const float* b,
                                 const void* scale, const void* shift, long long ldm, void* y, float* mean,
                                 float* rstd, int rows, int D, float eps, hipStream_t stream) {
  if (rows <= 0) return 0;
  dim3 grid((rows + 3) / 4);
  if (in_dtype == UVA_DT_F32 && out_dtype == UVA_DT_F32)
    DISPATCH_LN(ln_fwd, float, float, (const float*)x, w, b, (const float*)scale, (const float*)shift, ldm,
                (float*)y, mean, rstd, rows, D, eps);
  else if (in_dtype == UVA_DT_F32 && out_dtype == UVA_DT_BF16)
    DISPATCH_LN(ln_fwd, float, bf16, (const float*)x, w, b, (const bf16*)scale, (const bf16*)shift, ldm, (bf16*)y,
                mean, rstd, rows, D, eps);
  else if (in_dtype == UVA_DT_BF16 && out_dtype == UVA_DT_BF16)
    DISPATCH_LN(ln_fwd, bf16, bf16, (const bf16*)x, w, b, (const bf16*)scale, (const bf16*)shift, ldm, (bf16*)y,
                mean, rstd, rows, D, eps);
  else
    return (int)hipErrorInvalidValue;
  UVA_LAUNCH_CHECK();
  return 0;
}

extern "C" int uva_layernorm_bwd(int in_dtype, int out_dtype, const void* x, const float* w, const float* b,
                                 const void* scale,
                                 long long ldm, const void* dy, int dy_dtype, const float* mean, const float* rstd,
                                 const float* dx_base, float* dx, int accum, void* dscale, void* dshift, float* dw, float* db, int accum_wb,
                                 float* workspace, int rows, int D, hipStream_t stream) {
  if (rows <= 0) return 0;
  const int rpb = 64;
  const int nblk = (rows + rpb - 1) / rpb;
  dim3 grid(nblk);
  float* pw = dw ? workspace : nullptr;
  float* pb = dw ? workspace + (long long)nblk * D : nullptr;
#define LNB_DY(TI, TO)                                                                                          \
  do {                                                                                                          \
    if (dy_dtype == UVA_DT_BF16)                                                                                \
      DISPATCH_LNB(TI, TO, bf16, (const TI*)x, w, b, (const TO*)scale, ldm, (const bf16*)dy, mean, rstd, dx_base, \
                   dx, accum, (TO*)dscale, (TO*)dshift, pw, pb, rows, D, rpb);                                  \
    else                                                                                                        \
      DISPATCH_LNB(TI, TO, float, (const TI*)x, w, b, (const TO*)scale, ldm, (const float*)dy, mean, rstd,        \
                   dx_base, dx, accum, (TO*)dscale, (TO*)dshift, pw, pb, rows, D, rpb);                         \
  } while (0)
  if (in_dtype == UVA_DT_F32 && out_dtype == UVA_DT_F32)
    LNB_DY(float, float);
  else if (in_dtype == UVA_DT_F32 && out_dtype == UVA_DT_BF16)
    LNB_DY(float, bf16);
  else if (in_dtype == UVA_DT_BF16 && out_dtype == UVA_DT_BF16)
    LNB_DY(bf16, bf16);
  else
    return (int)hipErrorInvalidValue;
#undef LNB_DY
  UVA_LAUNCH_CHECK();
  if (dw) {
    colsum_partials(pw, db ? pb : nullptr, dw, db, nblk, D, accum_wb, stream);
    UVA_LAUNCH_CHECK();
  }
  return 0;
}

extern "C" int uva_layernorm_bwd_drop(const float* x, const float* w, const void* dy, const float* mean,
                                      const float* rstd, const float* dx_base, float* dx, float* dw, float* db,
                                      int accum_wb, void* drop_out, float drop_p, unsigned long long seed,
                                      float* dbias, int accum_dbias, float* workspace, int rows, int D,
                                      hipStream_t stream) {
  if (rows <= 0) return 0;
  if (D != 768 || !w || !dw || !db || !drop_out || !dbias || !workspace || ((uintptr_t)drop_out % 8))
    return (int)hipErrorInvalidValue;
  const int rpb = 64;
  const int nblk = (rows + rpb - 1) / rpb;
  float* pw = workspace;
  float* pb = workspace + (long long)nblk * D;
  float* pd = workspace + 2LL * nblk * D;
  uint32_t th;
  float ds;
  uva_drop_params(drop_p, &th, &ds);
  LnDrop ld{(bf16*)drop_out, pd, drop_key(seed), th, ds};
  ln_bwd<float, float, 4, 3, bf16, true><<<dim3(nblk), 256, 0, stream>>>(
      x, w, nullptr, (const float*)nullptr, 0, (const bf16*)dy, mean, rstd, dx_base, dx, 0, (float*)nullptr,
      (float*)nullptr, pw, pb, rows, D, rpb, ld);
  UVA_LAUNCH_CHECK();
  colsum_partials(pw, pb, dw, db, nblk, D, accum_wb, stream);
  UVA_LAUNCH_CHECK();
  colsum_partials(pd, nullptr, dbias, nullptr, nblk, D, accum_dbias, stream);
  UVA_LAUNCH_CHECK();
  return 0;
}

extern "C" long long uva_layernorm_bwd_workspace(int rows, int D) {
  const int rpb = 64;
  return (long long)((rows + rpb - 1) / rpb) * D * 2;
}

int uva_colsum_vec(int dtype, const void* in, long long ld, float* out, int rows, int cols, int accum,
                   float* workspace, hipStream_t s);

extern "C" int uva_colsum(int dtype, const void* in, long long ld, float* out, int rows, int cols, int accum,
                          float* workspace, hipStream_t stream) {
  if (rows <= 0 || cols <= 0) return 0;
  {
    const int r = uva_colsum_vec(dtype, in, ld, out, rows, cols, accum, workspace, stream);
    if (r < 0) return (int)hipErrorLaunchFailure;
    if (r > 0) return 0;
  }
  const int rpb = 512;
  int nb = (rows + rpb - 1) / rpb;
  dim3 g1((cols + 63) / 64, nb);
  if (nb > 1 && workspace) {
    if (dtype == UVA_DT_BF16) colsum_part_kernel<bf16><<<g1, 256, 0, stream>>>((const bf16*)in, ld, workspace, rows, cols, rpb);
    else colsum_part_kernel<float><<<g1, 256, 0, stream>>>((const float*)in, ld, workspace, rows, cols, rpb);
    colsum_partials(workspace, nullptr, out, nullptr, nb, cols, accum, stream);
  } else {
    if (dtype == UVA_DT_BF16) colsum_kernel<bf16><<<dim3((cols + 63) / 64), 256, 0, stream>>>((const bf16*)in, ld, out, rows, cols, accum);
    else colsum_kernel<float><<<dim3((cols + 63) / 64), 256, 0, stream>>>((const float*)in, ld, out, rows, cols, accum);
  }
  UVA_LAUNCH_CHECK();
  return 0;
}

extern "C" long long uva_colsum_workspace(int rows, int cols) {
  return (long long)((rows + 127) / 128) * cols;
}

extern "C" int uva_softmax_fwd(int dtype, const void* S, void* P, void* Pd, long long rows, int L, float scale,
                               float drop_p, unsigned long long seed, hipStream_t stream) {
  if (rows <= 0) return 0;
  uint32_t th;
  float ds;
  uva_drop_params(drop_p, &th, &ds);
  dim3 grid((unsigned)((rows + 3) / 4));
  if (dtype == UVA_DT_BF16)
    softmax_fwd_kernel<bf16><<<grid, 256, 0, stream>>>((const bf16*)S, (bf16*)P, th ? (bf16*)Pd : nullptr, rows, L, scale, th, ds, seed);
  else
    softmax_fwd_kernel<float><<<grid, 256, 0, stream>>>((const float*)S, (float*)P, th ? (float*)Pd : nullptr, rows, L, scale, th, ds, seed);
  UVA_LAUNCH_CHECK();
  return 0;
}

extern "C" int uva_softmax_bwd(int dtype, const void* P, const void* dPd, void* dS, long long rows, int L, float scale,
                               float drop_p, unsigned long long seed, hipStream_t stream) {
  if (rows <= 0) return 0;
  uint32_t th;
  float ds;
  uva_drop_params(drop_p, &th, &ds);
  dim3 grid((unsigned)((rows + 3) / 4));
  if (dtype == UVA_DT_BF16)
    softmax_bwd_kernel<bf16><<<grid, 256, 0, stream>>>((const bf16*)P, (const bf16*)dPd, (bf16*)dS, rows, L, scale, th, ds, seed);
  else
    softmax_bwd_kernel<float><<<grid, 256, 0, stream>>>((const float*)P, (const float*)dPd, (float*)dS, rows, L, scale, th, ds, seed);
  UVA_LAUNCH_CHECK();
  return 0;
}
```

unified_video_action_amd/model/autoregressive/functional.py:

```python
import math

import torch

from ...native import ops
from ...runtime import RT, cdt

F32 = torch.float32


def as_dtype(t, dtype):
    if t.dtype == dtype and t.is_contiguous():
        return t
    t = t.contiguous()
    if t.dtype == dtype:
        return t
    out = torch.empty(t.shape, dtype=dtype, device=t.device)
    ops.cast(t, out)
    return out


def compute_weight(p):
    if cdt() == F32:
        return p.detach()
    sh = getattr(p, "_uva_shadow", None)
    if sh is not None and getattr(p, "_uva_shadow_owner", None) == id(p):
        return sh
    key = (p._version, p.data_ptr(), RT.param_gen if getattr(p, "_uva_raw_updated", False) else 0)
    if sh is None or getattr(p, "_uva_shadow_ver", None) != key:
        sh = as_dtype(p.detach(), cdt())
        p._uva_shadow = sh
        p._uva_shadow_ver = key
    return sh


def compute_weight_t(p):
    ev = getattr(p, "_uva_t_event", None)
    if ev is not None:
        torch.cuda.current_stream().wait_event(ev)
        p._uva_t_event = None
    w = compute_weight(p)
    key = (p._version, p.data_ptr(), RT.param_gen)
    t = getattr(p, "_uva_shadow_t", None)
    if t is None or getattr(p, "_uva_shadow_t_ver", None) != key:
        if t is None or t.shape != (w.shape[1], w.shape[0]):
            t = torch.empty(w.shape[1], w.shape[0], dtype=w.dtype, device=w.device)
        ops.transpose_bf16(w, t)
        p._uva_shadow_t = t
        p._uva_shadow_t_ver = key
    return t


def prefetch_weight_t(params, side):
    if cdt() != torch.bfloat16:
        return
    todo = []
    for p in params:
        w = compute_weight(p)
        key = (p._version, p.data_ptr(), RT.param_gen)
        if getattr(p, "_uva_shadow_t_ver", None) == key and getattr(p, "_uva_t_event", None) is None:
            continue
        t = getattr(p, "_uva_shadow_t", None)
        if t is None or t.shape != (w.shape[1], w.shape[0]):
            t = torch.empty(w.shape[1], w.shape[0], dtype=w.dtype, device=w.device)
            p._uva_shadow_t = t
        todo.append((p, w, t, key))
    side.wait_stream(torch.cuda.current_stream())
    for p, w, t, key in todo:
        with torch.cuda.stream(side):
            ops.transpose_bf16(w, t)
            ev = torch.cuda.Event()
            ev.record(side)
        p._uva_shadow_t_ver = key
        p._uva_t_event = ev


def linear_bias(x, p, b, out):
    ops.linear(x, compute_weight(p), out, bias=b.detach())


def linear_dx_w(dy, p, dx):
    if cdt() == torch.bfloat16:
        ops.linear(dy, compute_weight_t(p), dx)
    else:
        ops.linear_dx(dy, compute_weight(p), dx)


def grad_buf(p):
    if p.grad is None:
        p.grad = torch.zeros_like(p)
    return p.grad


def _seed():
    return RT.next_seed()


class LinearFn(torch.autograd.Function):

    @staticmethod
    def forward(ctx, x, weight, bias, act, drop_p, out_dtype, residual):
        xc = as_dtype(x, cdt())
        w = compute_weight(weight)
        if w.dim() != 2:
            w = w.reshape(w.shape[0], -1)
        M, N = xc.shape[0], weight.shape[0]
        out = torch.empty(M, N, dtype=out_dtype, device=x.device)
        aux = torch.empty(M, N, dtype=out_dtype, device=x.device) if act != "none" else None
        seed = _seed() if drop_p > 0 else 0
        ops.linear(xc, w, out, bias=None if bias is None else bias.detach(), act=act, aux=aux,
                   residual=residual, drop_p=drop_p, seed=seed)
        ctx.save_for_backward(xc, weight, bias, aux)
        ctx.cfg = (act, drop_p, seed, x.dtype, residual is not None)
        return out

    @staticmethod
    def backward(ctx, g):
        xc, weight, bias, aux = ctx.saved_tensors
        act, drop_p, seed, xdt, has_res = ctx.cfg
        M, N = g.shape
        fused_bias = False
        if act != "none" or drop_p > 0:
            dpre = torch.empty(M, N, dtype=cdt(), device=g.device)
            if bias is not None and N % 8 == 0:
                ops.act_bwd_bias(aux, g.contiguous(), dpre, grad_buf(bias), act, drop_p=drop_p, seed=seed)
                fused_bias = True
            else:
                ops.act_bwd(aux, g.contiguous(), dpre, act, drop_p=drop_p, seed=seed)
        else:
            dpre = as_dtype(g, cdt())
        gx = None
        if ctx.needs_input_grad[0]:
            gx = torch.empty(M, xc.shape[1], dtype=F32, device=g.device)
            ops.linear_dx(dpre, compute_weight(weight).reshape(N, -1), gx)
            gx = as_dtype(gx, xdt)
        ops.linear_dw(dpre, xc, grad_buf(weight).view(N, -1))
        if bias is not None and not fused_bias:
            ops.colsum(dpre, grad_buf(bias), accum=True)
        return gx, None, None, None, None, None, (g if has_res else None)


def linear(x, layer, act="none", drop_p=0.0, out_dtype=F32, residual=None):
    shp = x.shape
    y = LinearFn.apply(x.reshape(-1, shp[-1]), layer.weight, layer.bias, act, drop_p, out_dtype,
                       None if residual is None else residual.reshape(-1, layer.weight.shape[0]))
    return y.reshape(*shp[:-1], layer.weight.shape[0])


class LayerNormFn(torch.autograd.Function):
    @staticmethod
    def forward(ctx, x, weight, bias, eps, out_dtype):
        x = x.contiguous()
        M, D = x.shape
        y = torch.empty(M, D, dtype=out_dtype, device=x.device)
        mean = torch.empty(M, dtype=F32, device=x.device)
        rstd = torch.empty(M, dtype=F32, device=x.device)
        ops.layernorm_fwd(x, None if weight is None else weight.detach(),
                          None if bias is None else bias.detach(), y, mean, rstd, eps)
        ctx.save_for_backward(x, weight, bias, mean, rstd)
        return y

    @staticmethod
    def backward(ctx, g):
        x, weight, bias, mean, rstd = ctx.saved_tensors
        dy = as_dtype(g, F32)
        dx = torch.empty(x.shape, dtype=F32, device=x.device)
        ops.layernorm_bwd(x, None if weight is None else weight.detach(), dy, mean, rstd, dx, accum=False,
                          dw=None if weight is None else grad_buf(weight),
                          db=None if bias is None else grad_buf(bias))
        return as_dtype(dx, x.dtype), None, None, None, None


def layer_norm(x, ln, out_dtype=F32):
    shp = x.shape
    y = LayerNormFn.apply(x.reshape(-1, shp[-1]), ln.weight, ln.bias, ln.eps, out_dtype)
    return y.reshape(shp)


class ActFn(torch.autograd.Function):
    @staticmethod
    def forward(ctx, x, act, out_dtype):
        x = x.contiguous()
        y = torch.empty(x.shape, dtype=out_dtype, device=x.device)
        ops.act_fwd(x, y, act)
        ctx.save_for_backward(x)
        ctx.act = act
        return y

    @staticmethod
    def backward(ctx, g):
        (x,) = ctx.saved_tensors
        dx = torch.empty(x.shape, dtype=x.dtype, device=x.device)
        ops.act_bwd(x.reshape(-1, x.shape[-1]), g.contiguous().reshape(-1, x.shape[-1]),
                    dx.reshape(-1, x.shape[-1]), ctx.act)
        return dx, None, None


def _attn_mat_fwd(qkv, B, N, H, scale, p, seed):
    D = qkv.shape[1] // 3
    hd = D // H
    ld = 3 * D
    q = qkv.float() if qkv.dtype != F32 else qkv
    S = torch.empty(B, H, N, N, dtype=F32, device=q.device)
    ops.gemm(q, q[:, D:], S, N, N, hd, ld, ld, N, 0, 0, batch=B * H, inner=H, sA=(N * ld, hd),
             sB=(N * ld, hd), sC=(H * N * N, N * N))
    P = torch.empty_like(S)
    Pd = torch.empty_like(S) if p > 0 else None
    ops.softmax_fwd(S, P, Pd, N, scale, p, seed)
    del S
    O = torch.empty(B * N, D, dtype=F32, device=q.device)
    ops.gemm(Pd if p > 0 else P, q[:, 2 * D:], O, N, hd, N, N, ld, D, 0, 1, batch=B * H, inner=H,
             sA=(H * N * N, N * N), sB=(N * ld, hd), sC=(N * D, hd))
    return O, P, Pd


def _attn_mat_bwd(qkv, P, Pd, dO, B, N, H, scale, p, seed):
    D = qkv.shape[1] // 3
    hd = D // H
    ld = 3 * D
    q = qkv.float() if qkv.dtype != F32 else qkv
    dO = as_dtype(dO, F32)
    dPd = torch.empty(B, H, N, N, dtype=F32, device=q.device)
    ops.gemm(dO, q[:, 2 * D:], dPd, N, N, hd, D, ld, N, 0, 0, batch=B * H, inner=H, sA=(N * D, hd),
             sB=(N * ld, hd), sC=(H * N * N, N * N))
    dS = torch.empty_like(dPd)
    ops.softmax_bwd(P, dPd, dS, N, scale, p, seed)
    del dPd
    dqkv = torch.empty(B * N, 3 * D, dtype=F32, device=q.device)
    bat = dict(batch=B * H, inner=H)
    ops.gemm(dS, q[:, D:], dqkv, N, hd, N, N, ld, ld, 0, 1, sA=(H * N * N, N * N), sB=(N * ld, hd),
             sC=(N * ld, hd), **bat)
    ops.gemm(dS, q, dqkv[:, D:], N, hd, N, N, ld, ld, 1, 1, sA=(H * N * N, N * N), sB=(N * ld, hd),
             sC=(N * ld, hd), **bat)
    ops.gemm(Pd if p > 0 else P, dO, dqkv[:, 2 * D:], N, hd, N, N, D, ld, 1, 1, sA=(H * N * N, N * N),
             sB=(N * D, hd), sC=(N * ld, hd), **bat)
    return dqkv


def use_flash(N, hd=64):
    return cdt() == torch.bfloat16 and RT.flash_attention and N % 64 == 0 and hd in (64, 80, 128)


class BlockFn(torch.autograd.Function):

    @staticmethod
    def forward(ctx, x, shape, p_attn, p_proj, hook, premask, n1w, n1b, qkvw, qkvb, projw, projb, n2w, n2b, fc1w,
                fc1b, fc2w, fc2b):
        B, N, H = shape
        M, D = x.shape
        dev = x.device
        c = cdt()
        scale = (D // H) ** -0.5
        seeds = [_seed() for _ in range(4)]
        up = RT._drop_pending.pop(x.data_ptr(), None)
        if up is not None and not (up[0].shape == x.shape and up[0].dtype == x.dtype):
            up = None
        if premask is not None:
            seeds[0] = premask[0]
        h1 = torch.empty(M, D, dtype=c, device=dev)
        m1 = torch.empty(M, dtype=F32, device=dev)
        r1 = torch.empty(M, dtype=F32, device=dev)
        ops.layernorm_fwd(x, n1w.detach(), n1b.detach(), h1, m1, r1)
        qkv = torch.empty(M, 3 * D, dtype=c, device=dev)
        linear_bias(h1, qkvw, qkvb, qkv)
        flash = use_flash(N, D // H)
        if flash and D // H != 64:
            o = torch.empty(M, D, dtype=c, device=dev)
            lse = torch.empty(B, H, N, dtype=F32, device=dev)
            pm = premask[1] if premask is not None else None
            P, Pd = None, ops.attn_fwd_hd(qkv, o, lse, B, N, H, D // H, scale, p_attn, seeds[0], mask=pm)
        elif flash:
            o = torch.empty(M, D, dtype=c, device=dev)
            lse = torch.empty(B, H, N, dtype=F32, device=dev)
            pm = premask[1] if premask is not None else None
            if RT.attn_fp8:
                ws = ops.attn_fp8_workspace(B, N, H, dev)
                ops.attn_quant_fp8(qkv, ws, B, N, H)
                amask = ops.attn_fwd_fp8(ws, o, lse, B, N, H, scale, p_attn, seeds[0], mask=pm)
                del ws
            else:
                amask = ops.attn_fwd(qkv, o, lse, B, N, H, scale, p_attn, seeds[0], mask=pm)
            P, Pd = None, amask
        else:
            o, P, Pd = _attn_mat_fwd(qkv, B, N, H, scale, p_attn, seeds[0])
            o = as_dtype(o, c)
            lse = None
        Hd = fc1w.shape[0]
        planes = (None, None, None)
        if c == torch.bfloat16 and RT.drop_planes and p_proj > 0 and D % 32 == 0 and Hd % 32 == 0:
            planes = (ops.dropout_plane(M * D, p_proj, seeds[1], dev), ops.dropout_plane(M * Hd, p_proj, seeds[2], dev),
                      ops.dropout_plane(M * D, p_proj, seeds[3], dev))
        x1 = torch.empty(M, D, dtype=F32, device=dev)
        if not (c == torch.bfloat16 and RT.proj_8w and
                ops.linear_drop_res(o, compute_weight(projw), projb.detach(), x, x1, p_proj, seeds[1], planes[0])):
            ops.linear(o, compute_weight(projw), x1, bias=projb.detach(), residual=x, drop_p=p_proj,
                       seed=seeds[1])
        h2 = torch.empty(M, D, dtype=c, device=dev)
        m2 = torch.empty(M, dtype=F32, device=dev)
        r2 = torch.empty(M, dtype=F32, device=dev)
        ops.layernorm_fwd(x1, n2w.detach(), n2b.detach(), h2, m2, r2)
        a = torch.empty(M, Hd, dtype=c, device=dev)
        pre1 = torch.empty(M, Hd, dtype=c, device=dev)
        x2 = torch.empty(M, D, dtype=F32, device=dev)
        if c == torch.bfloat16:
            fused = not RT.mlp_split_epilogue
            if not (fused and ops.linear_gelu_drop(h2, compute_weight(fc1w), fc1b.detach(), pre1, a, p_proj,
                                                   seeds[2], planes[1])):
                linear_bias(h2, fc1w, fc1b, pre1)
                ops.act_drop_fwd(pre1, a, "gelu", drop_p=p_proj, seed=seeds[2])
            if not (fused and ops.linear_drop_res(a, compute_weight(fc2w), fc2b.detach(), x1, x2, p_proj, seeds[3],
                                                  planes[2])):
                t2 = torch.empty(M, D, dtype=c, device=dev)
                linear_bias(a, fc2w, fc2b, t2)
                ops.act_drop_fwd(t2, x2, "none", drop_p=p_proj, seed=seeds[3], residual=x1)
                del t2
        else:
            ops.linear(h2, compute_weight(fc1w), a, bias=fc1b.detach(), act="gelu", aux=pre1, drop_p=p_proj,
                       seed=seeds[2])
            ops.linear(a, compute_weight(fc2w), x2, bias=fc2b.detach(), residual=x1, drop_p=p_proj, seed=seeds[3])
        ctx.save_for_backward(x, h1, m1, r1, qkv, o, lse, P, Pd, x1, h2, m2, r2, pre1, a,
                              n1w, n1b, qkvw, qkvb, projw, projb, n2w, n2b, fc1w, fc1b, fc2w, fc2b)
        ctx.cfg = (B, N, H, p_attn, p_proj, seeds, flash)
        ctx.plane1 = planes[1]
        ctx.up = up[1:] if up is not None else None
        if c == torch.bfloat16 and RT.ln_bwd_drop and any(ctx.needs_input_grad):
            RT._drop_pending[x2.data_ptr()] = (x2, p_proj, seeds[3], fc2b)
        ctx.hook = hook
        return x2

    @staticmethod
    def backward(ctx, g2):
        (x, h1, m1, r1, qkv, o, lse, P, Pd, x1, h2, m2, r2, pre1, a,
         n1w, n1b, qkvw, qkvb, projw, projb, n2w, n2b, fc1w, fc1b, fc2w, fc2b) = ctx.saved_tensors
        B, N, H, p_attn, p_proj, seeds, flash = ctx.cfg
        M, D = x.shape
        dev = x.device
        c = cdt()
        scale = (D // H) ** -0.5
        g2 = as_dtype(g2, F32)
        ready = RT._drop_ready.pop(seeds[3], None)
        if ready is not None and ready[0] == g2.data_ptr() and ready[1].shape == (M, D):
            dpre2 = ready[1]
        else:
            dpre2 = torch.empty(M, D, dtype=c, device=dev)
            ops.act_bwd_bias(None, g2, dpre2, grad_buf(fc2b), "none", drop_p=p_proj, seed=seeds[3])
        ops.linear_dw(dpre2, a, grad_buf(fc2w))
        Hd = fc1w.shape[0]
        dpre1 = torch.empty(M, Hd, dtype=c, device=dev)
        if c == torch.bfloat16 and RT.act_bwd_in_gemm and ops.linear_dgelu_drop(
                dpre2, compute_weight_t(fc2w), pre1, dpre1, grad_buf(fc1b), p_proj, seeds[2], plane=ctx.plane1):
            pass
        elif RT.act_bwd_in_gemm:
            ops.linear_dx_act(dpre2, compute_weight(fc2w), dpre1, pre1, "gelu", drop_p=p_proj, seed=seeds[2])
            ops.colsum(dpre1, grad_buf(fc1b))
        else:
            da = torch.empty(M, Hd, dtype=c, device=dev)
            linear_dx_w(dpre2, fc2w, da)
            ops.act_bwd_bias(pre1, da, dpre1, grad_buf(fc1b), "gelu", drop_p=p_proj, seed=seeds[2])
            del da
        del dpre2
        ops.linear_dw(dpre1, h2, grad_buf(fc1w))
        dh2 = torch.empty(M, D, dtype=c if RT.ln_dy_lowp else F32, device=dev)
        linear_dx_w(dpre1, fc1w, dh2)
        del dpre1
        g1 = torch.empty(M, D, dtype=F32, device=dev)
        dprep = torch.empty(M, D, dtype=c, device=dev)
        if not (c == torch.bfloat16 and RT.ln_bwd_drop and dh2.dtype == c and
                ops.layernorm_bwd_drop(x1, n2w.detach(), dh2, m2, r2, g1, grad_buf(n2w), grad_buf(n2b), g2, dprep,
                                       p_proj, seeds[1], grad_buf(projb))):
            ops.layernorm_bwd(x1, n2w.detach(), dh2, m2, r2, g1, accum=False, dw=grad_buf(n2w), db=grad_buf(n2b),
                              dx_base=g2)
            ops.act_bwd_bias(None, g1, dprep, grad_buf(projb), "none", drop_p=p_proj, seed=seeds[1])
        del dh2
        ops.linear_dw(dprep, o, grad_buf(projw))
        do = torch.empty(M, D, dtype=c, device=dev)
        linear_dx_w(dprep, projw, do)
        del dprep
        if flash and D // H != 64:
            dqkv = torch.empty(M, 3 * D, dtype=c, device=dev)
            dvec = torch.empty(B, H, N, dtype=F32, device=dev)
            ops.attn_bwd_hd(qkv, o, do, lse, dvec, dqkv, B, N, H, D // H, scale, p_attn, seeds[0], mask=Pd,
                            dbias=grad_buf(qkvb) if RT.attn_bias_grad else None)
        elif flash:
            dqkv = torch.empty(M, 3 * D, dtype=c, device=dev)
            dvec = torch.empty(B, H, N, dtype=F32, device=dev)
            ops.attn_bwd(qkv, o, do, lse, dvec, dqkv, B, N, H, scale, p_attn, seeds[0], mask=Pd,
                         dbias=grad_buf(qkvb) if RT.attn_bias_grad else None)
        else:
            dqkv = as_dtype(_attn_mat_bwd(qkv, P, Pd, do, B, N, H, scale, p_attn, seeds[0]), c)
        del do
        ops.linear_dw(dqkv, h1, grad_buf(qkvw))
        if not (flash and RT.attn_bias_grad):
            ops.colsum(dqkv, grad_buf(qkvb))
        dh1 = torch.empty(M, D, dtype=c if RT.ln_dy_lowp else F32, device=dev)
        linear_dx_w(dqkv, qkvw, dh1)
        del dqkv
        gx = torch.empty(M, D, dtype=F32, device=dev)
        up = ctx.up
        if up is not None and dh1.dtype == c:
            p_up, seed_up, fc2b_up = up
            d_up = torch.empty(M, D, dtype=c, device=dev)
            if ops.layernorm_bwd_drop(x, n1w.detach(), dh1, m1, r1, gx, grad_buf(n1w), grad_buf(n1b), g1, d_up,
                                      p_up, seed_up, grad_buf(fc2b_up)):
                RT._drop_ready[seed_up] = (gx.data_ptr(), d_up)
            else:
                up = None
        if up is None or dh1.dtype != c:
            ops.layernorm_bwd(x, n1w.detach(), dh1, m1, r1, gx, accum=False, dw=grad_buf(n1w), db=grad_buf(n1b),
                              dx_base=g1)
        if ctx.hook is not None:
            ctx.hook()
        return (gx,) + (None,) * 17


def block_forward(blk, x, B, N, p_attn, p_proj):
    D = x.shape[-1]
    a, m = blk.attn, blk.mlp
    premask = None
    if p_attn > 0 and use_flash(N, D // a.num_heads) and x.is_cuda:
        shape = (B, N, a.num_heads, float(p_attn))
        premask = RT.take_attn_mask(id(blk), shape)
        RT.note_attn_shape(id(blk), shape)
    y = BlockFn.apply(x.reshape(B * N, D).contiguous(), (B, N, a.num_heads), p_attn, p_proj,
                      getattr(blk, "_uva_bucket_hook", None), premask, blk.norm1.weight, blk.norm1.bias,
                      a.qkv.weight, a.qkv.bias, a.proj.weight, a.proj.bias,
                      blk.norm2.weight, blk.norm2.bias, m.fc1.weight, m.fc1.bias, m.fc2.weight, m.fc2.bias)
    return y.reshape(B, N, D)


class AdaLNTrunkFn(torch.autograd.Function):

    @staticmethod
    def forward(ctx, x0, y, depth, hook, *params):
        R, W = x0.shape
        dev = x0.device
        c = cdt()
        sy = torch.empty(R, W, dtype=c, device=dev)
        ops.act_fwd(y.contiguous(), sy, "silu")
        x = x0.contiguous()
        saved = []
        for i in range(depth):
            modw, modb, w1, b1, w2, b2, lnw, lnb = params[8 * i:8 * i + 8]
            mod = torch.empty(R, 3 * W, dtype=c, device=dev)
            ops.linear(sy, compute_weight(modw), mod, bias=modb.detach())
            h = torch.empty(R, W, dtype=c, device=dev)
            mean = torch.empty(R, dtype=F32, device=dev)
            rstd = torch.empty(R, dtype=F32, device=dev)
            _ln_mod_fwd(x, lnw, lnb, mod, W, h, mean, rstd)
            a = torch.empty(R, W, dtype=c, device=dev)
            pre1 = torch.empty(R, W, dtype=c, device=dev)
            ops.linear(h, compute_weight(w1), a, bias=b1.detach(), act="silu", aux=pre1)
            xn = torch.empty(R, W, dtype=F32, device=dev)
            hm2 = torch.empty(R, W, dtype=F32, device=dev)
            ops.linear(a, compute_weight(w2), xn, bias=b2.detach(), aux=hm2, gate=mod[:, 2 * W:], residual=x)
            saved += [x, mod, h, mean, rstd, a, pre1, hm2]
            x = xn
        fmw, fmb, lw, lb = params[8 * depth:8 * depth + 4]
        fmod = torch.empty(R, 2 * W, dtype=c, device=dev)
        ops.linear(sy, compute_weight(fmw), fmod, bias=fmb.detach())
        hf = torch.empty(R, W, dtype=c, device=dev)
        meanf = torch.empty(R, dtype=F32, device=dev)
        rstdf = torch.empty(R, dtype=F32, device=dev)
        ops.layernorm_fwd(x, None, None, hf, meanf, rstdf, scale=fmod[:, W:], shift=fmod[:, :W], ldm=2 * W)
        out = torch.empty(R, lw.shape[0], dtype=F32, device=dev)
        ops.linear(hf, compute_weight(lw), out, bias=lb.detach())
        saved += [x, fmod, hf, meanf, rstdf]
        ctx.save_for_backward(y, sy, *saved, *params)
        ctx.depth = depth
        ctx.hook = hook
        return out

    @staticmethod
    def backward(ctx, gout):
        depth = ctx.depth
        t = ctx.saved_tensors
        y, sy = t[0], t[1]
        blocks = [t[2 + 8 * i:2 + 8 * i + 8] for i in range(depth)]
        xf, fmod, hf, meanf, rstdf = t[2 + 8 * depth:2 + 8 * depth + 5]
        params = t[2 + 8 * depth + 5:]
        R, W = y.shape
        dev = y.device
        c = cdt()
        fmw, fmb, lw, lb = params[8 * depth:8 * depth + 4]
        dout = as_dtype(gout, c)
        ops.linear_dw(dout, hf, grad_buf(lw))
        ops.colsum(dout, grad_buf(lb))
        dhf = torch.empty(R, W, dtype=F32, device=dev)
        ops.linear_dx(dout, compute_weight(lw), dhf)
        dfmod = torch.empty(R, 2 * W, dtype=c, device=dev)
        dx = torch.empty(R, W, dtype=F32, device=dev)
        ops.layernorm_bwd(xf, None, dhf, meanf, rstdf, dx, accum=False, scale=fmod[:, W:], ldm=2 * W,
                          dscale=dfmod[:, W:], dshift=dfmod[:, :W])
        ops.linear_dw(dfmod, sy, grad_buf(fmw))
        ops.colsum(dfmod, grad_buf(fmb))
        dsy = torch.empty(R, W, dtype=F32, device=dev)
        ops.linear_dx(dfmod, compute_weight(fmw), dsy)
        del dfmod, dhf
        for i in reversed(range(depth)):
            x, mod, h, mean, rstd, a, pre1, hm2 = blocks[i]
            modw, modb, w1, b1, w2, b2, lnw, lnb = params[8 * i:8 * i + 8]
            dmod = torch.empty(R, 3 * W, dtype=c, device=dev)
            dhm2 = torch.empty(R, W, dtype=c, device=dev)
            ops.gate_bwd(dx, hm2, mod[:, 2 * W:], dhm2, dmod[:, 2 * W:])
            ops.linear_dw(dhm2, a, grad_buf(w2))
            ops.colsum(dhm2, grad_buf(b2))
            dpre1 = torch.empty(R, W, dtype=c, device=dev)
            if RT.trunk_act_bwd_in_gemm and pre1.dtype == c:
                ops.linear_dx_act(dhm2, compute_weight(w2), dpre1, pre1, "silu")
                ops.colsum(dpre1, grad_buf(b1))
            else:
                da = torch.empty(R, W, dtype=c, device=dev)
                ops.linear_dx(dhm2, compute_weight(w2), da)
                ops.act_bwd_bias(pre1, da, dpre1, grad_buf(b1), "silu")
            ops.linear_dw(dpre1, h, grad_buf(w1))
            dh = torch.empty(R, W, dtype=F32, device=dev)
            ops.linear_dx(dpre1, compute_weight(w1), dh)
            dxn = torch.empty(R, W, dtype=F32, device=dev)
            _ln_mod_bwd(x, lnw, lnb, mod, W, dh, mean, rstd, dxn, dmod, dx)
            ops.linear_dw(dmod, sy, grad_buf(modw))
            ops.colsum(dmod, grad_buf(modb))
            ops.linear_dx(dmod, compute_weight(modw), dsy, beta=1.0)
            dx = dxn
        dy = torch.empty(R, W, dtype=F32, device=dev)
        ops.act_bwd(y, dsy, dy, "silu")
        if ctx.hook is not None:
            ctx.hook()
        return (dx, dy, None, None) + (None,) * len(params)


def _ln_mod_fwd(x, lnw, lnb, mod, W, h, mean, rstd):
    ops.layernorm_fwd(x, lnw.detach(), lnb.detach(), h, mean, rstd, scale=mod[:, W:2 * W], shift=mod[:, :W],
                      ldm=3 * W)


def _ln_mod_bwd(x, lnw, lnb, mod, W, dh, mean, rstd, dx_out, dmod, dx_base):
    R = x.shape[0]
    ops.layernorm_bwd(x, lnw.detach(), dh, mean, rstd, dx_out, accum=False, dw=grad_buf(lnw), db=grad_buf(lnb),
                      scale=mod[:, W:2 * W], ldm=3 * W, dscale=dmod[:, W:2 * W], dshift=dmod[:, :W],
                      dx_base=dx_base, b=lnb.detach())
```

unified_video_action_amd/native/ops.py:

```python
import ctypes

import torch

from .lib import lib

F32, BF16 = 0, 1
ACT = {"none": 0, "gelu": 1, "silu": 2, "relu": 3}


def dt(t):
    if t.dtype == torch.bfloat16:
        return BF16
    if t.dtype == torch.float32:
        return F32
    raise TypeError(f"unsupported dtype {t.dtype}")


def ptr(t):
    return None if t is None else t.data_ptr()


def stream():
    return torch.cuda.current_stream().cuda_stream


TRACE = None
TRACE_ONLY = None


class _traced:
    __slots__ = ("tag", "flops", "ev")
    depth = 0

    def __init__(self, tag, flops):
        self.tag, self.flops, self.ev = tag, flops, None

    def __enter__(self):
        if TRACE is not None and _traced.depth == 0 and (TRACE_ONLY is None or self.tag in TRACE_ONLY):
            self.ev = (torch.cuda.Event(enable_timing=True), torch.cuda.Event(enable_timing=True))
            self.ev[0].record()
        _traced.depth += 1
        return self

    def __exit__(self, *a):
        _traced.depth -= 1
        if self.ev is not None:
            self.ev[1].record()
            if TRACE is not None:
                side = torch.cuda.current_stream() != torch.cuda.default_stream()
                TRACE.setdefault(self.tag, []).append((self.ev[0], self.ev[1], self.flops, side))


def _call(name, *args):
    if TRACE is None:
        return lib().call(name, *args)
    with _traced(name[4:] if name.startswith("uva_") else name, 0.0):
        return lib().call(name, *args)


def _ld(t):
    assert t.dim() == 2 and t.stride(1) == 1, (t.shape, t.stride())
    return t.stride(0)


def gemm(A, B, C, M, N, K, lda, ldb, ldc, ta=0, tb=0, batch=1, inner=1, sA=(0, 0), sB=(0, 0), sC=(0, 0),
         bias=None, residual=None, ldr=0, sR=(0, 0), aux=None, act="none", alpha=1.0, beta=0.0,
         drop_p=0.0, seed=0, force_generic=False, splitk=True, gate=None, ldg=0):
    assert A.dtype == B.dtype, (A.dtype, B.dtype)
    ws = workspace(SPLITK_WS_FLOATS, A.device) if (splitk and batch == 1) else None
    if bias is not None:
        assert bias.dtype == torch.float32 and bias.is_contiguous()
    if aux is not None:
        assert aux.dtype == C.dtype
    with _traced(f"gemm[{'NT'[ta]}{'NT'[tb]}] {'bf16' if dt(A) else 'f32'} M{M} N{N} K{K} b{batch}",
                 2.0 * M * N * K * batch):
        _call("uva_gemm", dt(A), dt(C), ta, tb, ptr(A), ptr(B), ptr(C), M, N, K, lda, ldb, ldc, batch, inner,
                   sA[0], sA[1], sB[0], sB[1], sC[0], sC[1], ptr(bias), ptr(residual), ldr, sR[0], sR[1], ptr(aux),
                   ACT[act] if isinstance(act, str) else act, float(alpha), float(beta), float(drop_p),
                   int(seed) & 0xFFFFFFFFFFFFFFFF, dt(residual) if residual is not None else 0, ptr(gate), ldg,
                   dt(gate) if gate is not None else 0, int(force_generic), ptr(ws),
                   ws.numel() if ws is not None else 0, stream())


SPLITK_WS_FLOATS = 1 << 25


def gemm_plan(M, N, K, ta=0, tb=0, batch=1, splitk=True, gn_prologue=False, dtype=torch.bfloat16):
    code = lib().query("uva_gemm_plan", 1 if dtype == torch.bfloat16 else 0, ta, tb, M, N, K, batch, int(gn_prologue),
                       SPLITK_WS_FLOATS if splitk else 0)
    return code & 15, (code >> 4) & 4095, code >> 16


def gemm_set_persist(on):
    return bool(lib().query("uva_gemm_set_persist", int(bool(on))))


def gemm4_set(on=-2, force=-2):
    prev = lib().query("uva_gemm4_set", int(on), int(force))
    return prev & 1, (prev >> 1) - 1


def gemm8w_set(on=-2, mode=-2):
    prev = lib().query("uva_gemm8w_set", int(on), int(mode))
    return prev & 1, prev >> 1


def linear_gelu_drop(x, w, bias, pre_out, out, drop_p=0.0, seed=0, plane=None):
    M, K = x.shape
    N = w.shape[0]
    assert x.is_contiguous() and w.is_contiguous() and pre_out.is_contiguous() and out.is_contiguous()
    with _traced(f"gemm+gelu+drop bf16 M{M} N{N} K{K}", 2.0 * M * N * K):
        r = lib().query("uva_linear_gelu_drop", ptr(x), ptr(w), ptr(bias), ptr(pre_out), ptr(out), M, N, K,
                        float(drop_p), int(seed) & 0xFFFFFFFFFFFFFFFF, ptr(plane), stream())
    if r < 0:
        raise RuntimeError(f"fused Mlp GEMM failed with hipError {-r}")
    return r == 1


def linear_drop_res(x, w, bias, residual, out, drop_p=0.0, seed=0, plane=None):
    M, K = x.shape
    N = w.shape[0]
    assert x.is_contiguous() and w.is_contiguous() and residual.is_contiguous() and out.is_contiguous()
    with _traced(f"gemm+drop+res bf16 M{M} N{N} K{K}", 2.0 * M * N * K):
        r = lib().query("uva_linear_drop_res", ptr(x), ptr(w), ptr(bias), ptr(residual), ptr(out), M, N, K,
                        float(drop_p), int(seed) & 0xFFFFFFFFFFFFFFFF, ptr(plane), stream())
    if r < 0:
        raise RuntimeError(f"fused Mlp GEMM failed with hipError {-r}")
    return r == 1


def linear_dgelu_drop(dy, wt, pre, dpre, dbias, drop_p=0.0, seed=0, accum_bias=True, plane=None):
    M, K = dy.shape
    N = wt.shape[0]
    assert dy.is_contiguous() and wt.is_contiguous() and pre.is_contiguous() and dpre.is_contiguous()
    ws = workspace((M + 255) // 256 * 4 * N, dy.device)
    with _traced(f"gemm+dgelu+drop bf16 M{M} N{N} K{K}", 2.0 * M * N * K):
        r = lib().query("uva_linear_dgelu_drop", ptr(dy), ptr(wt), ptr(pre), ptr(dpre), ptr(dbias), int(accum_bias),
                        ptr(ws), M, N, K, float(drop_p), int(seed) & 0xFFFFFFFFFFFFFFFF, ptr(plane), stream())
    if r < 0:
        raise RuntimeError(f"fused Mlp GEMM failed with hipError {-r}")
    return r == 1


def dropout_plane(n, drop_p, seed, device, out=None):
    words = lib().query("uva_dropout_plane_words", int(n))
    if out is None:
        out = torch.empty(words, dtype=torch.int32, device=device)
    _call("uva_dropout_plane", ptr(out), int(n), float(drop_p), int(seed) & 0xFFFFFFFFFFFFFFFF, stream())
    return out


def gemm4_plan(M, N, K):
    code = lib().query("uva_gemm4_plan", M, N, K)
    return None if code < 0 else (code & 255, code >> 8)


def gemm4_plan_tt(M, N, K, ws_floats=None):
    code = lib().query("uva_gemm4_plan_tt", M, N, K, SPLITK_WS_FLOATS if ws_floats is None else ws_floats)
    return None if code < 0 else (code & 255, code >> 8)


def linear(x, w, out, bias=None, act="none", aux=None, residual=None, drop_p=0.0, seed=0, beta=0.0, gate=None):
    M, K = x.shape
    N = w.shape[0]
    assert w.shape[1] == K and out.shape == (M, N)
    gemm(x, w, out, M, N, K, _ld(x), _ld(w), _ld(out), 0, 0, bias=bias, act=act, aux=aux,
         residual=residual, ldr=_ld(residual) if residual is not None else 0, drop_p=drop_p, seed=seed,
         beta=beta, gate=gate, ldg=_ld(gate) if gate is not None else 0)


def linear_dx(dy, w, dx, beta=0.0):
    M, N = dy.shape
    K = w.shape[1]
    assert dx.shape == (M, K)
    gemm(dy, w, dx, M, K, N, _ld(dy), _ld(w), _ld(dx), 0, 1, beta=beta)


def linear_dx_act(dy, w, dx, pre, act, drop_p=0.0, seed=0):
    M, N = dy.shape
    K = w.shape[1]
    assert dx.shape == (M, K) and pre.shape == (M, K) and pre.is_contiguous() and dx.is_contiguous()
    gemm(dy, w, dx, M, K, N, _ld(dy), _ld(w), _ld(dx), 0, 1, residual=pre, ldr=_ld(pre), act=16 + ACT[act],
         drop_p=drop_p, seed=seed)


def linear_dw(dy, x, dw, beta=1.0):
    M, N = dy.shape
    K = x.shape[1]
    assert dw.shape == (N, K)
    gemm(dy, x, dw, N, K, M, _ld(dy), _ld(x), _ld(dw), 1, 1, beta=beta)


_WS = {}


def workspace(n_floats, device):
    key = (device, "ws")
    t = _WS.get(key)
    if t is None or t.numel() < n_floats:
        t = torch.empty(max(int(n_floats), 1 << 20), dtype=torch.float32, device=device)
        _WS[key] = t
    return t


def colsum(x, out, accum=True):
    rows, cols = x.shape
    ws = workspace(lib().query("uva_colsum_workspace", rows, cols), x.device)
    _call("uva_colsum", dt(x), ptr(x), _ld(x), ptr(out), rows, cols, int(accum), ptr(ws), stream())


def layernorm_fwd(x, w, b, y, mean, rstd, eps=1e-6, scale=None, shift=None, ldm=0):
    rows, D = x.shape
    assert x.is_contiguous() and y.is_contiguous()
    _call("uva_layernorm_fwd", dt(x), dt(y), ptr(x), ptr(w), ptr(b), ptr(scale), ptr(shift), ldm, ptr(y),
               ptr(mean), ptr(rstd), rows, D, float(eps), stream())


def layernorm_bwd(x, w, dy, mean, rstd, dx, accum, dw=None, db=None, scale=None, ldm=0, dscale=None, dshift=None,
                  out_dtype=None, accum_wb=True, dx_base=None, b=None):
    rows, D = x.shape
    assert dy.dtype in (torch.float32, torch.bfloat16) and dx.dtype == torch.float32
    odt = out_dtype if out_dtype is not None else (dt(scale) if scale is not None else dt(x))
    ws = None
    if dw is not None:
        ws = workspace(lib().query("uva_layernorm_bwd_workspace", rows, D), x.device)
    _call("uva_layernorm_bwd", dt(x), odt, ptr(x), ptr(w), ptr(b), ptr(scale), ldm, ptr(dy), dt(dy), ptr(mean),
               ptr(rstd),
               ptr(dx_base), ptr(dx), int(accum), ptr(dscale), ptr(dshift), ptr(dw), ptr(db), int(accum_wb), ptr(ws), rows, D,
               stream())


def layernorm_bwd_drop(x, w, dy, mean, rstd, dx, dw, db, dx_base, drop_out, drop_p, seed, dbias, accum_wb=True,
                       accum_dbias=True):
    rows, D = x.shape
    if not (D == 768 and x.dtype == torch.float32 and dy.dtype == torch.bfloat16 and dx_base is not None
            and drop_out.dtype == torch.bfloat16 and drop_out.is_contiguous() and dx_base.is_contiguous()):
        return False
    ws = workspace(3 * ((rows + 63) // 64) * D, x.device)
    _call("uva_layernorm_bwd_drop", ptr(x), ptr(w), ptr(dy), ptr(mean), ptr(rstd), ptr(dx_base), ptr(dx), ptr(dw),
          ptr(db), int(accum_wb), ptr(drop_out), float(drop_p), int(seed) & 0xFFFFFFFFFFFFFFFF, ptr(dbias),
          int(accum_dbias), ptr(ws), rows, D, stream())
    return True


def softmax_fwd(S, P, Pd, L, scale, drop_p=0.0, seed=0):
    rows = S.numel() // L
    _call("uva_softmax_fwd", dt(S), ptr(S), ptr(P), ptr(Pd), rows, L, float(scale), float(drop_p),
               int(seed) & 0xFFFFFFFFFFFFFFFF, stream())


def softmax_bwd(P, dPd, dS, L, scale, drop_p=0.0, seed=0):
    rows = P.numel() // L
    _call("uva_softmax_bwd", dt(P), ptr(P), ptr(dPd), ptr(dS), rows, L, float(scale), float(drop_p),
               int(seed) & 0xFFFFFFFFFFFFFFFF, stream())


def transpose_bf16(src, dst):
    R, C = src.shape
    assert src.dtype == dst.dtype == torch.bfloat16 and src.is_contiguous() and dst.is_contiguous()
    assert tuple(dst.shape) == (C, R)
    _call("uva_transpose_bf16", ptr(src), ptr(dst), R, C, stream())


def cast(src, dst):
    if src.dim() == 1 or (src.is_contiguous() and dst.is_contiguous()):
        rows, cols = 1, src.numel()
        lds = ldd = cols
    else:
        rows, cols = src.shape
        lds, ldd = _ld(src), _ld(dst)
    _call("uva_cast", dt(src), ptr(src), lds, dt(dst), ptr(dst), ldd, rows, cols, stream())


def act_fwd(x, y, act):
    _call("uva_act_fwd", dt(x), ptr(x), dt(y), ptr(y), x.numel(), ACT[act], stream())


def act_drop_fwd(x, y, act="none", drop_p=0.0, seed=0, residual=None):
    assert x.is_contiguous() and y.is_contiguous() and x.numel() == y.numel()
    if residual is not None:
        assert residual.is_contiguous() and residual.numel() == x.numel()
    _call("uva_act_drop_fwd", dt(x), ptr(x), dt(y), ptr(y), dt(residual) if residual is not None else 0,
               ptr(residual), x.numel(), ACT[act], float(drop_p), int(seed) & 0xFFFFFFFFFFFFFFFF, stream())


def act_bwd(pre, dy, dx, act, drop_p=0.0, seed=0, accum=False):
    rows, cols = dy.shape
    _call("uva_act_bwd", dt(pre) if pre is not None else F32, ptr(pre), dt(dy), ptr(dy), _ld(dy), dt(dx),
               ptr(dx), _ld(dx), rows, cols, ACT[act], float(drop_p), int(seed) & 0xFFFFFFFFFFFFFFFF, int(accum),
               stream())


def act_bwd_bias(pre, dy, dx, dbias, act, drop_p=0.0, seed=0, accum=False, accum_bias=True):
    rows, cols = dy.shape
    ws = workspace(lib().query("uva_act_bwd_bias_workspace", rows, cols), dy.device)
    _call("uva_act_bwd_bias", dt(pre) if pre is not None else F32, ptr(pre), dt(dy), ptr(dy), _ld(dy), dt(dx),
               ptr(dx), _ld(dx), rows, cols, ACT[act], float(drop_p), int(seed) & 0xFFFFFFFFFFFFFFFF, int(accum),
               ptr(dbias), int(accum_bias), ptr(ws), stream())


def gate_bwd(dout, h, gate, dh, dgate):
    rows, cols = dout.shape
    _call("uva_gate_bwd", ptr(dout), dt(h), ptr(h), dt(gate), ptr(gate), _ld(gate), dt(dh), ptr(dh),
               ptr(dgate), rows, cols, stream())


def fill(t, v):
    _call("uva_fill", ptr(t), t.numel(), float(v), stream())


def _tables_arg(tables):
    arr = (ctypes.c_void_p * 8)(*[t.data_ptr() for t in tables])
    return arr


def q_sample(x0, noise, t, tables, xt):
    rows, C = x0.shape
    arr = _tables_arg(tables)
    _call("uva_q_sample", ptr(x0), ptr(noise), ptr(t), ctypes.cast(arr, ctypes.c_void_p), dt(xt), ptr(xt),
               rows, C, stream())


def timestep_features(t, freqs, out):
    rows = t.numel()
    _call("uva_timestep_features", ptr(t), ptr(freqs), dt(out), ptr(out), rows, freqs.numel(), stream())


def diffusion_loss(x0, noise, t, out, tables, loss_row, dl):
    rows, C = x0.shape
    arr = _tables_arg(tables)
    _call("uva_diffusion_loss", ptr(x0), ptr(noise), ptr(t), dt(out), ptr(out), _ld(out),
               ctypes.cast(arr, ctypes.c_void_p), ptr(loss_row), ptr(dl), rows, C, stream())


def sampler_persistent(pack, mod, coef, noise, x0, x_out, work, clip=True, eps=1e-6):
    S, R, C = noise.shape
    depth, W = pack["b1"].shape
    for t in (coef, noise, x0, x_out, mod):
        if not t.is_contiguous():
            raise ValueError("sampler_persistent: contiguous operands required")
    if mod.shape[:2] != (S, R) or coef.shape != (S, 8) or x0.shape != (R, C) or x_out.shape != (R, C):
        raise ValueError("sampler_persistent: shape mismatch")
    _call("uva_sampler_persistent", R, C, W, depth, S, int(clip), float(eps), ptr(pack["w1"]), ptr(pack["b1"]),
               ptr(pack["w2"]), ptr(pack["b2"]), ptr(pack["lnw"]), ptr(pack["lnb"]), ptr(pack["win"]),
               ptr(pack["bin"]), ptr(pack["wf"]), ptr(pack["bfin"]), ptr(mod), mod.shape[2], ptr(coef), ptr(noise),
               ptr(x0), ptr(x_out), ptr(work), work.numel(), stream())


def sampler_persistent_test_hook(no_publish=True):
    _call("uva_sampler_persistent_test_hook", int(bool(no_publish)))


PERSISTENT_SAMPLER_CUS = 64


def sampler_persistent_fits(device):
    return torch.cuda.get_device_properties(device).multi_processor_count >= PERSISTENT_SAMPLER_CUS


def sampler_persistent_workspace(W, device):
    return torch.empty(lib().query("uva_sampler_persistent_workspace", W), dtype=torch.uint8, device=device)


def sampler_persistent_status(work):
    flag = ctypes.c_uint(0)
    _call("uva_sampler_persistent_status", ptr(work), ctypes.cast(ctypes.pointer(flag), ctypes.c_void_p),
               stream())
    return flag.value


def p_sample_step(out, x, noise, coef, x_new, x_net=None, clip=True):
    rows, C = x.shape
    if out.shape[0] != rows or out.shape[1] != 2 * C or out.stride(1) != 1:
        raise ValueError(f"p_sample_step: out {tuple(out.shape)} vs x {tuple(x.shape)}")
    for t in (x, noise, x_new):
        if t.dtype != torch.float32 or not t.is_contiguous() or t.shape != x.shape:
            raise ValueError("p_sample_step: x / noise / x_new must be contiguous fp32 [rows, C]")
    if x_net is not None and (not x_net.is_contiguous() or x_net.shape != x.shape):
        raise ValueError("p_sample_step: x_net must be contiguous [rows, C]")
    k = (ctypes.c_float * 8)(*coef)
    _call("uva_p_sample_step", dt(out), ptr(out), out.stride(0), ptr(x), ptr(noise),
               ctypes.cast(k, ctypes.c_void_p), ptr(x_new), dt(x_net) if x_net is not None else 0,
               ptr(x_net), int(clip), rows, C, stream())


def sampler_linear(A, W, out, bias=None, act="none", ln=False, lnw=None, lnb=None, shift=None, scale=None,
                   eps=1e-6, gate=None, residual=None):
    R, K = A.shape
    N = W.shape[0]
    if W.shape[1] != K or W.dtype != torch.bfloat16 or W.stride(1) != 1 or W.stride(0) != K:
        raise ValueError(f"sampler_linear: W {tuple(W.shape)} must be contiguous bf16 [N, {K}]")
    if out.shape != (R, N) or out.stride(1) != 1:
        raise ValueError(f"sampler_linear: out {tuple(out.shape)} != {(R, N)}")
    if A.stride(1) != 1 or A.dtype != (torch.float32 if ln else torch.bfloat16):
        raise ValueError("sampler_linear: A must be row-major fp32 (ln) or bf16")
    ldm = 0
    if ln:
        if shift is None or scale is None or shift.stride(0) != scale.stride(0) or shift.dtype != torch.bfloat16:
            raise ValueError("sampler_linear: ln needs bf16 shift/scale views with one row stride")
        ldm = shift.stride(0)
    ldg = gate.stride(0) if gate is not None else 0
    ldr = residual.stride(0) if residual is not None else 0
    _call("uva_sampler_linear", int(ln), ptr(A), A.stride(0), ptr(lnw), ptr(lnb), ptr(shift), ptr(scale), ldm,
               float(eps), ptr(W), ptr(bias), ACT[act], ptr(gate), ldg, ptr(residual), ldr, dt(out), ptr(out),
               out.stride(0), R, N, K, stream())


def weighted_mean(l, w, res):
    _call("uva_weighted_mean", ptr(l), ptr(w), l.numel(), ptr(res), stream())


def loss_grad(dl, w, wsum, g_up, dout):
    rows, C2 = dl.shape
    _call("uva_loss_grad", ptr(dl), ptr(w), ptr(wsum), ptr(g_up), dt(dout), ptr(dout), _ld(dout), rows, C2,
               stream())


def adamw_ema(p, g, m, v, ema, p_bf16, n_decay, lr, b1, b2, eps, wd, step, grad_scale, ema_decay):
    _call("uva_adamw_ema", ptr(p), ptr(g), ptr(m), ptr(v), ptr(ema), ptr(p_bf16), p.numel(), int(n_decay),
               float(lr), float(b1), float(b2), float(eps), float(wd), int(step), float(grad_scale),
               float(ema_decay), stream())


def ema_update(ema, p, decay):
    if ema.dtype != torch.float32 or p.dtype != torch.float32 or ema.numel() != p.numel():
        raise ValueError("ema_update: two fp32 buffers of equal size")
    _call("uva_ema_update", ptr(ema), ptr(p), ema.numel(), float(decay), stream())


def attn_mask_alloc(B, N, H, device):
    return torch.empty(lib().query("uva_attn_mask_bytes", B, N, H), dtype=torch.uint8, device=device)


def attn_dropmask(B, N, H, drop_p, seed, device, out=None):
    mask = attn_mask_alloc(B, N, H, device) if out is None else out
    assert mask.numel() == lib().query("uva_attn_mask_bytes", B, N, H) and mask.dtype == torch.uint8
    _call("uva_attn_dropmask", ptr(mask), B, N, H, float(drop_p), int(seed) & 0xFFFFFFFFFFFFFFFF, stream())
    return mask


def attn_fwd(qkv, out, lse2, B, N, H, scale, drop_p=0.0, seed=0, mask=None):
    assert qkv.dtype == torch.bfloat16 and qkv.is_contiguous() and out.is_contiguous()
    assert N % 64 == 0 and qkv.shape[-1] == 3 * H * 64
    assert qkv.numel() == B * N * 3 * H * 64 and out.numel() == B * N * H * 64 and lse2.numel() == B * H * N
    with _traced(f"attn_fwd B{B} N{N} H{H}", 4.0 * B * H * N * N * 64):
        if drop_p > 0 and mask is None:
            mask = attn_dropmask(B, N, H, drop_p, seed, qkv.device)
        _call("uva_attn_fwd", ptr(qkv), ptr(out), ptr(lse2), ptr(mask) if drop_p > 0 else None, B, N, H,
                   float(scale), float(drop_p), stream())
    return mask if drop_p > 0 else None


def attn_fp8_workspace(B, N, H, device):
    return torch.empty(lib().query("uva_attn_fp8_workspace", B, N, H), dtype=torch.uint8, device=device)


def attn_quant_fp8(qkv, ws, B, N, H):
    assert qkv.dtype == torch.bfloat16 and qkv.is_contiguous() and qkv.numel() == B * N * 3 * H * 64
    assert N % 64 == 0 and ws.dtype == torch.uint8 and ws.numel() >= lib().query("uva_attn_fp8_workspace", B, N, H)
    _call("uva_attn_quant_fp8", ptr(qkv), ptr(ws), B, N, H, stream())


def attn_fwd_fp8(ws, out, lse2, B, N, H, scale, drop_p=0.0, seed=0, mask=None, device=None):
    assert out.dtype == torch.bfloat16 and out.is_contiguous() and out.numel() == B * N * H * 64
    assert lse2.numel() == B * H * N and N % 64 == 0
    with _traced(f"attn_fwd_fp8 B{B} N{N} H{H}", 4.0 * B * H * N * N * 64):
        if drop_p > 0 and mask is None:
            mask = attn_dropmask(B, N, H, drop_p, seed, out.device)
        _call("uva_attn_fwd_fp8", ptr(ws), ptr(out), ptr(lse2), ptr(mask) if drop_p > 0 else None, B, N, H,
                   float(scale), float(drop_p), stream())
    return mask if drop_p > 0 else None


def attn_bwd(qkv, out, dout, lse2, dvec, dqkv, B, N, H, scale, drop_p=0.0, seed=0, mask=None, dbias=None,
             accum_bias=True):
    assert dout.dtype == torch.bfloat16 and dout.is_contiguous() and dqkv.is_contiguous()
    assert dout.numel() == B * N * H * 64 and dqkv.numel() == B * N * 3 * H * 64 and dvec.numel() == B * H * N
    with _traced(f"attn_bwd B{B} N{N} H{H}", 8.0 * B * H * N * N * 64):
        if drop_p > 0 and mask is None:
            mask = attn_dropmask(B, N, H, drop_p, seed, qkv.device)
        if dbias is not None:
            assert dbias.dtype == torch.float32 and dbias.numel() == 3 * H * 64 and dbias.is_contiguous()
            ws = workspace(B * ((N + 127) // 128) * 3 * H * 64, qkv.device)
            _call("uva_attn_bwd_bias", ptr(qkv), ptr(out), ptr(dout), ptr(lse2), ptr(mask) if drop_p > 0 else None,
                  ptr(dvec), ptr(dqkv), ptr(dbias), int(accum_bias), ptr(ws), B, N, H, float(scale), float(drop_p),
                  stream())
            return
        nb = lib().query("uva_attn_bwd_workspace", B, N, H, float(drop_p))
        ws = torch.empty(nb, dtype=torch.uint8, device=qkv.device) if nb else None
        _call("uva_attn_bwd", ptr(qkv), ptr(out), ptr(dout), ptr(lse2), ptr(mask) if drop_p > 0 else None,
                   ptr(dvec), ptr(dqkv), ptr(ws), B, N, H, float(scale), float(drop_p), stream())


def attn_hd_supported(head_dim):
    return bool(lib().query("uva_attn_hd_supported", int(head_dim)))


def attn_fwd_hd(qkv, out, lse2, B, N, H, head_dim, scale, drop_p=0.0, seed=0, mask=None):
    hd = int(head_dim)
    assert qkv.dtype == torch.bfloat16 and qkv.is_contiguous() and out.is_contiguous()
    assert attn_hd_supported(hd), f"head_dim {hd}: the fused kernels serve 80 and 128 (64: attn_fwd)"
    assert N % 64 == 0 and qkv.shape[-1] == 3 * H * hd
    assert qkv.numel() == B * N * 3 * H * hd and out.numel() == B * N * H * hd and lse2.numel() == B * H * N
    with _traced(f"attn_fwd_hd{hd} B{B} N{N} H{H}", 4.0 * B * H * N * N * hd):
        if drop_p > 0 and mask is None:
            mask = attn_dropmask(B, N, H, drop_p, seed, qkv.device)
        _call("uva_attn_fwd_hd", ptr(qkv), ptr(out), ptr(lse2), ptr(mask) if drop_p > 0 else None, B, N, H, hd,
              float(scale), float(drop_p), stream())
    return mask if drop_p > 0 else None


def attn_bwd_hd(qkv, out, dout, lse2, dvec, dqkv, B, N, H, head_dim, scale, drop_p=0.0, seed=0, mask=None,
                dbias=None, accum_bias=True):
    hd = int(head_dim)
    assert dout.dtype == torch.bfloat16 and dout.is_contiguous() and dqkv.is_contiguous()
    assert attn_hd_supported(hd), f"head_dim {hd}: the fused kernels serve 80 and 128 (64: attn_bwd)"
    assert N % 64 == 0 and qkv.dtype == torch.bfloat16 and qkv.is_contiguous() and out.is_contiguous()
    assert dout.numel() == B * N * H * hd and dqkv.numel() == B * N * 3 * H * hd and dvec.numel() == B * H * N
    assert qkv.numel() == dqkv.numel() and out.numel() == dout.numel() and lse2.numel() == B * H * N
    with _traced(f"attn_bwd_hd{hd} B{B} N{N} H{H}", 8.0 * B * H * N * N * hd):
        if drop_p > 0 and mask is None:
            mask = attn_dropmask(B, N, H, drop_p, seed, qkv.device)
        ws = None
        if dbias is not None:
            assert dbias.dtype == torch.float32 and dbias.numel() == 3 * H * hd and dbias.is_contiguous()
            ws = workspace(lib().query("uva_attn_bwd_hd_part_floats", B, N, H, hd), qkv.device)
        _call("uva_attn_bwd_hd", ptr(qkv), ptr(out), ptr(dout), ptr(lse2), ptr(mask) if drop_p > 0 else None,
              ptr(dvec), ptr(dqkv), ptr(dbias), int(accum_bias), ptr(ws), B, N, H, hd, float(scale), float(drop_p),
              stream())


def conv2d(x, w, out, Nimg, Hin, Win, Ci, Co, ks, stride, pad_t, pad_l, Hout, Wout, bias=None, residual=None,
           gn_scale=None, gn_shift=None, gn_silu=True, act="none", force_generic=False, gn_part=None):
    assert x.dtype == w.dtype == out.dtype
    assert w.numel() == Co * ks * ks * Ci and out.numel() == Nimg * Hout * Wout * Co
    if residual is not None:
        assert residual.dtype == out.dtype and residual.numel() == out.numel()
    with _traced(f"conv{ks}x{ks}/s{stride} {'bf16' if dt(x) else 'f32'} {Hin}x{Win} Ci{Ci} Co{Co} n{Nimg}",
                 2.0 * Nimg * Hout * Wout * Co * ks * ks * Ci):
        _conv_call(x, w, out, Nimg, Hin, Win, Ci, Co, ks, stride, pad_t, pad_l, Hout, Wout, bias, residual, gn_scale,
                   gn_shift, gn_silu, act, force_generic, gn_part)


def _conv_call(x, w, out, Nimg, Hin, Win, Ci, Co, ks, stride, pad_t, pad_l, Hout, Wout, bias, residual, gn_scale,
               gn_shift, gn_silu, act, force_generic, gn_part):
    _call("uva_conv2d", dt(x), ptr(x), ptr(w), ptr(out), ptr(bias), ptr(residual), Nimg, Hin, Win, Ci, Co, ks,
               stride, pad_t, pad_l, Hout, Wout, ptr(gn_scale), ptr(gn_shift), int(gn_silu), ACT[act], ptr(gn_part),
               int(force_generic), stream())


def conv_fuses_gn(Nimg, H, W, Ci, Co, ks, stride, dtype=torch.bfloat16):
    return (dtype == torch.bfloat16 and ks == 3 and stride == 1 and
            lib().query("uva_conv3x3_halo_bn", Nimg, H, W, Ci, Co) > 0)


def pool4x4_cwh(x, out, n, C):
    assert x.is_contiguous() and out.is_contiguous() and x.dtype == out.dtype
    assert x.numel() == n * 256 * C and out.numel() == n * 16 * C
    _call("uva_pool4x4_cwh", dt(x), ptr(x), ptr(out), n, C, stream())


def pool4x4_relu_bwd(post, gpool, dpre, n, C):
    assert post.is_contiguous() and gpool.is_contiguous() and dpre.is_contiguous() and post.dtype == dpre.dtype
    assert post.numel() == dpre.numel() == n * 256 * C and gpool.numel() == n * 16 * C
    _call("uva_pool4x4_relu_bwd", dt(post), ptr(post), dt(gpool), ptr(gpool), ptr(dpre), n, C, stream())


def im2col3x3(x, cols, n, H, W, Ci):
    assert x.is_contiguous() and cols.is_contiguous() and x.dtype == cols.dtype
    assert x.numel() == n * H * W * Ci and cols.numel() == n * H * W * Ci * 9
    _call("uva_im2col3x3", dt(x), ptr(x), ptr(cols), n, H, W, Ci, stream())


def im2col3x3_tc(x, cols, n, H, W, Ci):
    assert x.is_contiguous() and cols.is_contiguous() and x.dtype == cols.dtype
    assert x.numel() == n * H * W * Ci and cols.numel() == n * H * W * Ci * 9
    _call("uva_im2col3x3_tc", dt(x), ptr(x), ptr(cols), n, H, W, Ci, stream())


def pad_nhwc(x, out, n, H, W, C, G):
    assert x.is_contiguous() and out.is_contiguous() and x.dtype == out.dtype
    assert out.numel() == (2 * G + n * (H + 2) * (W + 2)) * C
    _call("uva_pad_nhwc", dt(x), ptr(x), ptr(out), n, H, W, C, G, stream())


def conv3x3_dw_implicit(dy, x, part, n, H, W, Co, Ci):
    G = W + 3
    K = n * (H + 2) * (W + 2)
    dyp = torch.empty(2 * G + K, Co, dtype=dy.dtype, device=dy.device)
    xp = torch.empty(2 * G + K, Ci, dtype=x.dtype, device=x.device)
    pad_nhwc(dy, dyp, n, H, W, Co, G)
    pad_nhwc(x, xp, n, H, W, Ci, G)
    for kh in range(3):
        for kw in range(3):
            tap = kh * 3 + kw
            d = (kh - 1) * (W + 2) + (kw - 1)
            gemm(dyp[G:], xp[G + d:], part[:, tap * Ci:], Co, Ci, K, Co, Ci, 9 * Ci, 1, 1, beta=0.0)


def conv3x3_dw_scatter_add(part, grad):
    Co, Ci = grad.shape[0], grad.shape[1]
    assert part.dtype == grad.dtype == torch.float32 and part.is_contiguous() and grad.is_contiguous()
    assert part.numel() == grad.numel() == Co * Ci * 9
    _call("uva_conv3x3_dw_scatter_add", ptr(part), ptr(grad), Co, Ci, stream())


def conv3x3_weight_layout(w, out, mode):
    Co, Ci = w.shape[0], w.shape[1]
    assert w.dtype == torch.float32 and w.is_contiguous() and out.is_contiguous() and out.numel() == w.numel()
    _call("uva_conv3x3_weight_layout", ptr(w), dt(out), ptr(out), Co, Ci, int(mode), stream())


def groupnorm_finalize_tiles(part, Nimg, HW, C, gamma, beta, scale, shift, eps=1e-6, tile_rows=128):
    _call("uva_groupnorm_finalize_tiles", ptr(part), Nimg, HW, C, tile_rows, ptr(gamma), ptr(beta), float(eps),
               ptr(scale), ptr(shift), stream())


def groupnorm_apply(x, scale, shift, y, Nimg, HW, C, silu=True):
    _call("uva_groupnorm_apply", ptr(x), ptr(scale), ptr(shift), ptr(y), Nimg, HW, C, int(silu), stream())


def groupnorm_stats(x, Nimg, HW, C, gamma, beta, scale, shift, eps=1e-6):
    ws = workspace(lib().query("uva_groupnorm_workspace", Nimg, HW), x.device)
    _call("uva_groupnorm_stats", dt(x), ptr(x), Nimg, HW, C, ptr(gamma), ptr(beta), float(eps), ptr(scale),
               ptr(shift), ptr(ws), stream())


def resize_select(img, sel, out, Cpad):
    B, T, C, H, W = img.shape
    assert C == 3 and img.dtype == torch.float32 and img.is_contiguous()
    _call("uva_resize_select", ptr(img), B, T, H, W, ptr(sel), sel.numel(), dt(out), ptr(out), Cpad, stream())


def posterior_sample(moments, eps, z, Nimg, scale=0.2325):
    _call("uva_posterior_sample", dt(moments), ptr(moments), ptr(eps), ptr(z), Nimg, float(scale), stream())


def upsample_nearest2x(x, y):
    n, H, W, C = x.shape
    if not (x.is_contiguous() and y.is_contiguous() and y.shape == (n, 2 * H, 2 * W, C) and y.dtype == x.dtype):
        raise ValueError(f"upsample_nearest2x: {tuple(x.shape)} -> {tuple(y.shape)}")
    _call("uva_upsample_nearest2x", dt(x), ptr(x), ptr(y), n, H, W, C, stream())
```

unified_video_action_amd/runtime.py:

```python
import itertools

import torch


class _Runtime:
    def __init__(self):
        self.compute_dtype = torch.bfloat16
        self.flash_attention = True
        self.attn_fp8 = False
        self.vae_gn_in_conv = True
        self.ln_dy_lowp = True
        self.mlp_split_epilogue = False
        self.proj_8w = True
        self.gemm8w_plain = True
        self._gemm8w_plain_set = None
        self.drop_planes = False
        self.attn_bias_grad = True
        self.ln_bwd_drop = True
        self.act_bwd_in_gemm = True
        self.trunk_act_bwd_in_gemm = False
        self._seed_base = 0x5EED
        self._ctr = itertools.count()
        self.attn_prefetch = True
        self.attn_prefetch_level = 2
        self._prefetch_pending = None
        self.weight_t_prefetch = True
        self._weight_t_params = []
        self._attn_shapes = {}
        self._attn_ready = {}
        self._side = None
        self._drop_pending = {}
        self._drop_ready = {}
        self.param_gen = 0

    def set_precision(self, name):
        name = str(name).lower()
        self.attn_fp8 = False
        if name in ("fp32", "float32", "no"):
            self.compute_dtype = torch.float32
        elif name in ("bf16", "bfloat16", "fp16"):
            self.compute_dtype = torch.bfloat16
        elif name in ("fp8_attn", "fp8"):
            self.compute_dtype = torch.bfloat16
            self.attn_fp8 = True
        else:
            raise ValueError(f"unknown precision {name}")

    def begin_forward(self):
        self._drop_pending.clear()
        self._drop_ready.clear()
        if self._gemm8w_plain_set is not self.gemm8w_plain:
            from .native import ops
            ops.gemm8w_set(int(self.gemm8w_plain), -2)
            self._gemm8w_plain_set = self.gemm8w_plain

    def bump_params(self):
        self.param_gen += 1

    def seed(self, base):
        self._seed_base = int(base)
        self._ctr = itertools.count()

    def next_seed(self):
        return (self._seed_base * 0x9E3779B97F4A7C15 + next(self._ctr) * 0xBF58476D1CE4E5B9) & 0xFFFFFFFFFFFFFFFF


    def note_attn_shape(self, key, shape):
        self._attn_shapes[key] = shape

    def arm_attn_prefetch(self, device):
        if self.attn_prefetch_level <= 0:
            self.prefetch_attn_masks(device)
        else:
            self._prefetch_pending = device

    def fire_attn_prefetch(self, level=None):
        dev = self._prefetch_pending
        if dev is not None and (level is None or level >= self.attn_prefetch_level):
            self._prefetch_pending = None
            self.prefetch_attn_masks(dev)

    def prefetch_attn_masks(self, device):
        self._prefetch_masks(device)
        if self.weight_t_prefetch and self._weight_t_params and self._side is not None:
            from .model.autoregressive.functional import prefetch_weight_t
            self._side.wait_stream(torch.cuda.current_stream(device))
            prefetch_weight_t(self._weight_t_params, self._side)

    def _prefetch_masks(self, device):
        if not (self.attn_prefetch and self._attn_shapes and torch.cuda.is_available()):
            return
        from .native import ops
        if self._side is None:
            self._side = torch.cuda.Stream(device=device)
        main = torch.cuda.current_stream(device)
        self._side.wait_stream(main)
        ready = {}
        for key, (B, N, H, p) in self._attn_shapes.items():
            seed = self.next_seed()
            mask = ops.attn_mask_alloc(B, N, H, device)
            with torch.cuda.stream(self._side):
                ops.attn_dropmask(B, N, H, p, seed, device, out=mask)
            ev = torch.cuda.Event()
            ev.record(self._side)
            mask.record_stream(self._side)
            ready[key] = ((B, N, H, p), seed, mask, ev)
        self._attn_ready = ready

    def take_attn_mask(self, key, shape):
        hit = self._attn_ready.pop(key, None)
        if hit is None or hit[0] != shape:
            return None
        torch.cuda.current_stream().wait_event(hit[3])
        return hit[1], hit[2]


RT = _Runtime()


def cdt():
    return RT.compute_dtype
```

Baseline: 265.3 samples/s.

## Defer bias-gradient column sums into grouped launches and batch weight transposes

Adds a deferral mode so attention, dgelu-GEMM and layernorm backward kernels write their per-block partial bias/weight gradient sums to group-owned buffers. A single grouped colsum kernel then reduces all of them in one launch instead of one small reduction launch each. It also adds a batched bf16 transpose kernel that handles up to 128 matrices per launch. The aim is to cut kernel launch count and tail overhead in the backward pass, at the cost of holding the partial buffers alive longer and searching for each block's item inside the kernel.

```diff
diff --git a/include/uva_hip.h b/include/uva_hip.h
--- a/include/uva_hip.h
+++ b/include/uva_hip.h
@@ -33,6 +33,7 @@
 int uva_linear_dgelu_drop(const void* dY, const void* Wt, const void* pre, void* dpre, float* dbias, int accum_bias,
                           float* part, int M, int N, int K, float drop_p, unsigned long long seed, const void* plane,
                           hipStream_t stream);
+int uva_linear_dgelu_drop_part_rows(int M);
 int uva_layernorm_bwd_drop(const float* x, const float* w, const void* dy, const float* mean, const float* rstd,
                            const float* dx_base, float* dx, float* dw, float* db, int accum_wb, void* drop_out,
                            float drop_p, unsigned long long seed, float* dbias, int accum_dbias, float* workspace,
@@ -77,6 +78,20 @@
 int uva_colsum(int dtype, const void* in, long long ld, float* out, int rows, int cols, int accum, float* workspace,
                hipStream_t stream);
 long long uva_colsum_workspace(int rows, int cols);
+#define UVA_COLSUM_FINAL 0
+#define UVA_COLSUM_PARTIALS 1
+#define UVA_COLSUM_DEFER 2
+typedef struct uva_colsum_item {
+  const float* p0;
+  const float* p1;
+  float* o0;
+  float* o1;
+  int rows, cols, accum, kind;
+} uva_colsum_item;
+int uva_colsum_group(const uva_colsum_item* items, int n, hipStream_t stream);
+int uva_colsum_final(const float* part, int nrows, int cols, float* out, int accum, hipStream_t stream);
+int uva_colsum_partials(const float* p0, const float* p1, float* o0, float* o1, int rows, int cols, int accum,
+                        hipStream_t stream);
 
 int uva_softmax_fwd(int dtype, const void* S, void* P, void* Pd, long long rows, int L, float scale, float drop_p,
                     unsigned long long seed, hipStream_t stream);
@@ -87,6 +102,13 @@
              hipStream_t stream);
 int uva_act_fwd(int xdt, const void* x, int ydt, void* y, long long n, int act, hipStream_t stream);
 int uva_transpose_bf16(const void* src, void* dst, int rows, int cols, hipStream_t stream);
+#define UVA_TRANSPOSE_BATCH_MAX 128
+typedef struct uva_transpose_item {
+  const void* src;
+  void* dst;
+  int rows, cols;
+} uva_transpose_item;
+int uva_transpose_bf16_batched(const uva_transpose_item* items, int n, hipStream_t stream);
 int uva_act_drop_fwd(int xdt, const void* x, int ydt, void* y, int rdt, const void* residual, long long n, int act,
                      float drop_p, unsigned long long seed, hipStream_t stream);
 int uva_act_bwd(int pdt, const void* pre, int gdt, const void* dy, long long ld_dy, int xdt, void* dx,
diff --git a/unified_video_action_amd/csrc/attention.hip b/unified_video_action_amd/csrc/attention.hip
--- a/unified_video_action_amd/csrc/attention.hip
+++ b/unified_video_action_amd/csrc/attention.hip
@@ -866,7 +866,7 @@
                                  int N, int H, float scale, float drop_p, hipStream_t s) {
   if (!dbias || !part) return (int)hipErrorInvalidValue;
   int r = attn_bwd_launch(qkv, out, dout, lse2, mask, Dvec, dqkv, B, N, H, scale, drop_p, part, s);
-  if (r) return r;
+  if (r || accum == UVA_COLSUM_DEFER) return r;
   return uva_colsum_final_launch(part, B * ((N + 127) / 128), 3 * H * 64, dbias, accum, s);
 }
 
diff --git a/unified_video_action_amd/csrc/attention_hd.hip b/unified_video_action_amd/csrc/attention_hd.hip
--- a/unified_video_action_amd/csrc/attention_hd.hip
+++ b/unified_video_action_amd/csrc/attention_hd.hip
@@ -604,6 +604,6 @@
   const int r = head_dim == 80
                     ? bwd_launch<80>(qkv, out, dout, lse2, mask, Dvec, dqkv, cpart, B, N, H, scale, drop, ds, s)
                     : bwd_launch<128>(qkv, out, dout, lse2, mask, Dvec, dqkv, cpart, B, N, H, scale, drop, ds, s);
-  if (r || !dbias) return r;
+  if (r || !dbias || accum == UVA_COLSUM_DEFER) return r;
   return uva_colsum_final_launch(part, B * ((N + 127) / 128), 3 * H * head_dim, dbias, accum, s);
 }
diff --git a/unified_video_action_amd/csrc/colsum.h b/unified_video_action_amd/csrc/colsum.h
--- /dev/null
+++ b/unified_video_action_amd/csrc/colsum.h
@@ -0,0 +1,65 @@
+#pragma once
+#include "common.h"
+
+__device__ __forceinline__ void colsum_final_body(const float* __restrict__ part, int nrows, int cols,
+                                                  float* __restrict__ out, int accum, int bx) {
+  __shared__ float red[8][33];
+  const int cl = threadIdx.x & 31, rl = threadIdx.x >> 5;
+  const int c = bx * 32 + cl;
+  float s = 0.f;
+  if (c < cols) {
+#pragma unroll 8
+    for (int j = rl; j < nrows; j += 8) s += part[(long long)j * cols + c];
+  }
+  red[rl][cl] = s;
+  __syncthreads();
+  if (rl == 0 && c < cols) {
+    float t = 0.f;
+#pragma unroll
+    for (int j = 0; j < 8; ++j) t += red[j][cl];
+    out[c] = accum ? out[c] + t : t;
+  }
+}
+
+__device__ __forceinline__ void colsum_partials_body(const float* __restrict__ in, float* __restrict__ out, int rows,
+                                                     int cols, int accum, int bx) {
+  __shared__ float4 red[32][8];
+  const int cg = threadIdx.x & 7, rl = threadIdx.x >> 3;
+  const int c = bx * 32 + cg * 4;
+  float4 acc = make_float4(0.f, 0.f, 0.f, 0.f);
+  if (c < cols) {
+#pragma unroll 4
+    for (int r = rl; r < rows; r += 32) {
+      const float4 v = *(const float4*)(in + (long long)r * cols + c);
+      acc.x += v.x; acc.y += v.y; acc.z += v.z; acc.w += v.w;
+    }
+  }
+  red[rl][cg] = acc;
+  __syncthreads();
+  if (rl < 4 && c < cols) {
+    const int cc = c + rl;
+    float t = 0.f;
+#pragma unroll 8
+    for (int k = 0; k < 32; ++k) {
+      const float4 v = red[k][cg];
+      t += rl == 0 ? v.x : (rl == 1 ? v.y : (rl == 2 ? v.z : v.w));
+    }
+    out[cc] = accum ? out[cc] + t : t;
+  }
+}
+
+#define UVA_COLSUM_FINAL 0
+#define UVA_COLSUM_PARTIALS 1
+struct ColsumItem {
+  const float* p0;
+  const float* p1;
+  float* o0;
+  float* o1;
+  int rows, cols, accum, kind;
+};
+#define COLSUM_GROUP_MAX 16
+struct ColsumGroup {
+  ColsumItem it[COLSUM_GROUP_MAX];
+  int blk0[COLSUM_GROUP_MAX + 1];
+  int n;
+};
diff --git a/unified_video_action_amd/csrc/common.h b/unified_video_action_amd/csrc/common.h
--- a/unified_video_action_amd/csrc/common.h
+++ b/unified_video_action_amd/csrc/common.h
@@ -14,6 +14,7 @@
 
 #define UVA_DT_F32 0
 #define UVA_DT_BF16 1
+#define UVA_COLSUM_DEFER 2
 
 #define LDS_PTR(T, p) ((__attribute__((address_space(3))) T*)(p))
 
diff --git a/unified_video_action_amd/csrc/elementwise.hip b/unified_video_action_amd/csrc/elementwise.hip
--- a/unified_video_action_amd/csrc/elementwise.hip
+++ b/unified_video_action_amd/csrc/elementwise.hip
@@ -1,4 +1,5 @@
 #include "common.h"
+#include "colsum.h"
 
 __device__ __forceinline__ float ldx(const void* p, int dt, long long i) {
   return dt == UVA_DT_BF16 ? (float)((const bf16*)p)[i] : ((const float*)p)[i];
@@ -179,22 +180,7 @@
 
 __global__ __launch_bounds__(256) void colsum_final_kernel(const float* __restrict__ part, int nrows, int cols,
                                                            float* __restrict__ out, int accum) {
-  __shared__ float red[8][33];
-  const int cl = threadIdx.x & 31, rl = threadIdx.x >> 5;
-  const int c = blockIdx.x * 32 + cl;
-  float s = 0.f;
-  if (c < cols) {
-#pragma unroll 8
-    for (int j = rl; j < nrows; j += 8) s += part[(long long)j * cols + c];
-  }
-  red[rl][cl] = s;
-  __syncthreads();
-  if (rl == 0 && c < cols) {
-    float t = 0.f;
-#pragma unroll
-    for (int j = 0; j < 8; ++j) t += red[j][cl];
-    out[c] = accum ? out[c] + t : t;
-  }
+  colsum_final_body(part, nrows, cols, out, accum, blockIdx.x);
 }
 
 extern "C" long long uva_act_bwd_bias_workspace(long long rows, int cols) {
@@ -233,6 +219,12 @@
   return (int)hipGetLastError();
 }
 
+extern "C" int uva_colsum_final(const float* part, int nrows, int cols, float* out, int accum, hipStream_t s) {
+  if (cols <= 0) return 0;
+  if (nrows < 0 || (nrows && !part) || !out) return (int)hipErrorInvalidValue;
+  return uva_colsum_final_launch(part, nrows, cols, out, accum, s);
+}
+
 int uva_colsum_vec(int dtype, const void* in, long long ld, float* out, int rows, int cols, int accum,
                    float* workspace, hipStream_t s) {
   if (cols % 8 || ld % 8 || ((uintptr_t)in % 16) || !workspace || rows < 2 * COLSUM_RPB) return 0;
@@ -279,17 +271,16 @@
   return 0;
 }
 
-__global__ __launch_bounds__(256) void transpose_bf16_kernel(const bf16* __restrict__ src, bf16* __restrict__ dst,
-                                                             int rows, int cols) {
-  __shared__ bf16 t[64][64 + 8];
-  const int r0 = blockIdx.y * 64, c0 = blockIdx.x * 64;
+__device__ __forceinline__ void transpose_bf16_tile(const bf16* __restrict__ src, bf16* __restrict__ dst, int rows,
+                                                    int cols, int r0, int c0, bool vl, bool vs,
+                                                    bf16 (*t)[64 + 8]) {
   const int tid = threadIdx.x;
 #pragma unroll
   for (int i = 0; i < 2; ++i) {
     const int id = tid + i * 256, rr = id >> 3, cc = (id & 7) * 8;
     const int r = r0 + rr, c = c0 + cc;
     bf16x8 v;
-    if (r < rows && c + 8 <= cols) {
+    if (vl && r < rows && c + 8 <= cols) {
       v = *(const bf16x8*)(src + (long long)r * cols + c);
     } else {
 #pragma unroll
@@ -306,7 +297,7 @@
     bf16x8 v;
 #pragma unroll
     for (int e = 0; e < 8; ++e) v[e] = t[rr + e][cc];
-    if (c < cols && r + 8 <= rows) {
+    if (vs && c < cols && r + 8 <= rows) {
       *(bf16x8*)(dst + (long long)c * rows + r) = v;
     } else if (c < cols) {
 #pragma unroll
@@ -314,6 +305,12 @@
         if (r + e < rows) dst[(long long)c * rows + r + e] = v[e];
     }
   }
+}
+
+__global__ __launch_bounds__(256) void transpose_bf16_kernel(const bf16* __restrict__ src, bf16* __restrict__ dst,
+                                                             int rows, int cols) {
+  __shared__ bf16 t[64][64 + 8];
+  transpose_bf16_tile(src, dst, rows, cols, blockIdx.y * 64, blockIdx.x * 64, true, true, t);
 }
 
 extern "C" int uva_transpose_bf16(const void* src, void* dst, int rows, int cols, hipStream_t s) {
@@ -321,6 +318,66 @@
   if ((rows % 8) || (cols % 8) || (((uintptr_t)src | (uintptr_t)dst) % 16)) return (int)hipErrorInvalidValue;
   transpose_bf16_kernel<<<dim3((cols + 63) / 64, (rows + 63) / 64), 256, 0, s>>>((const bf16*)src, (bf16*)dst, rows,
                                                                                  cols);
+  UVA_LAUNCH_CHECK();
+  return 0;
+}
+
+#define UVA_TRANSPOSE_BATCH_MAX 128
+struct uva_transpose_item {
+  const void* src;
+  void* dst;
+  int rows, cols;
+};
+struct TransposeBatch {
+  struct {
+    const bf16* src;
+    bf16* dst;
+    int rows, cols;
+  } it[UVA_TRANSPOSE_BATCH_MAX];
+  int tile0[UVA_TRANSPOSE_BATCH_MAX + 1];
+  int n;
+};
+static_assert(sizeof(TransposeBatch) <= 3840, "kernel argument segment");
+
+__global__ __launch_bounds__(256) void transpose_bf16_batched_kernel(const TransposeBatch b) {
+  __shared__ bf16 t[64][64 + 8];
+  const int bid = blockIdx.x;
+  int lo = 0, hi = b.n;
+  while (hi - lo > 1) {
+    const int mid = (lo + hi) >> 1;
+    if (b.tile0[mid] <= bid) lo = mid;
+    else hi = mid;
+  }
+  const bf16* src = b.it[lo].src;
+  bf16* dst = b.it[lo].dst;
+  const int rows = b.it[lo].rows, cols = b.it[lo].cols;
+  const int l = bid - b.tile0[lo], tx = (cols + 63) / 64;
+  const bool vl = cols % 8 == 0 && (uintptr_t)src % 16 == 0, vs = rows % 8 == 0 && (uintptr_t)dst % 16 == 0;
+  transpose_bf16_tile(src, dst, rows, cols, (l / tx) * 64, (l % tx) * 64, vl, vs, t);
+}
+
+extern "C" int uva_transpose_bf16_batched(const uva_transpose_item* items, int n, hipStream_t s) {
+  if (n < 0 || n > UVA_TRANSPOSE_BATCH_MAX || (n && !items)) return (int)hipErrorInvalidValue;
+  TransposeBatch b{};
+  long long tiles = 0;
+  int m = 0;
+  for (int i = 0; i < n; ++i) {
+    const uva_transpose_item& it = items[i];
+    if (it.rows < 0 || it.cols < 0) return (int)hipErrorInvalidValue;
+    if (it.rows == 0 || it.cols == 0) continue;
+    if (!it.src || !it.dst || (((uintptr_t)it.src | (uintptr_t)it.dst) % 2)) return (int)hipErrorInvalidValue;
+    b.it[m].src = (const bf16*)it.src;
+    b.it[m].dst = (bf16*)it.dst;
+    b.it[m].rows = it.rows;
+    b.it[m].cols = it.cols;
+    b.tile0[m++] = (int)tiles;
+    tiles += (long long)((it.rows + 63) / 64) * ((it.cols + 63) / 64);
+    if (tiles > 0x7FFFFFFFLL) return (int)hipErrorInvalidValue;
+  }
+  if (!m) return 0;
+  for (int i = m; i <= UVA_TRANSPOSE_BATCH_MAX; ++i) b.tile0[i] = (int)tiles;
+  b.n = m;
+  transpose_bf16_batched_kernel<<<dim3((unsigned)tiles), 256, 0, s>>>(b);
   UVA_LAUNCH_CHECK();
   return 0;
 }
diff --git a/unified_video_action_amd/csrc/gemm8w.hip b/unified_video_action_amd/csrc/gemm8w.hip
--- a/unified_video_action_amd/csrc/gemm8w.hip
+++ b/unified_video_action_amd/csrc/gemm8w.hip
@@ -703,6 +703,8 @@
 
 int uva_colsum_final_launch(const float* part, int nrows, int cols, float* out, int accum, hipStream_t s);
 
+extern "C" int uva_linear_dgelu_drop_part_rows(int M) { return g8_part_rows(M); }
+
 extern "C" int uva_linear_dgelu_drop(const void* dY, const void* Wt, const void* pre, void* dpre, float* dbias,
                                      int accum_bias, float* part, int M, int N, int K, float drop_p,
                                      unsigned long long seed, const void* plane, hipStream_t s) {
@@ -716,6 +718,7 @@
   int r = g8_nw4(3) ? g8_launch<6, 3, 0, bf16, 4>(dY, Wt, dpre, M, N, K, K, K, N, ep, s)
                                 : g8_launch<6, 3, 0, bf16>(dY, Wt, dpre, M, N, K, K, K, N, ep, s);
   if (r) return -r;
+  if (accum_bias == UVA_COLSUM_DEFER) return 1;
   r = uva_colsum_final_launch(part, g8_part_rows(M), N, dbias, accum_bias, s);
   return r ? -r : 1;
 }
diff --git a/unified_video_action_amd/csrc/norm.hip b/unified_video_action_amd/csrc/norm.hip
--- a/unified_video_action_amd/csrc/norm.hip
+++ b/unified_video_action_amd/csrc/norm.hip
@@ -1,4 +1,5 @@
 #include "common.h"
+#include "colsum.h"
 
 template <typename T>
 __device__ __forceinline__ void load_vec(const T* p, float* out, int n) {
@@ -330,31 +331,7 @@
 __global__ __launch_bounds__(256) void colsum_partials_kernel(const float* __restrict__ p0, const float* __restrict__ p1,
                                                               float* __restrict__ o0, float* __restrict__ o1, int rows,
                                                               int cols, int accum) {
-  const float* in = blockIdx.y ? p1 : p0;
-  float* out = blockIdx.y ? o1 : o0;
-  __shared__ float4 red[32][8];
-  const int cg = threadIdx.x & 7, rl = threadIdx.x >> 3;
-  const int c = blockIdx.x * 32 + cg * 4;
-  float4 acc = make_float4(0.f, 0.f, 0.f, 0.f);
-  if (c < cols) {
-#pragma unroll 4
-    for (int r = rl; r < rows; r += 32) {
-      const float4 v = *(const float4*)(in + (long long)r * cols + c);
-      acc.x += v.x; acc.y += v.y; acc.z += v.z; acc.w += v.w;
-    }
-  }
-  red[rl][cg] = acc;
-  __syncthreads();
-  if (rl < 4 && c < cols) {
-    const int cc = c + rl;
-    float t = 0.f;
-#pragma unroll 8
-    for (int k = 0; k < 32; ++k) {
-      const float4 v = red[k][cg];
-      t += rl == 0 ? v.x : (rl == 1 ? v.y : (rl == 2 ? v.z : v.w));
-    }
-    out[cc] = accum ? out[cc] + t : t;
-  }
+  colsum_partials_body(blockIdx.y ? p1 : p0, blockIdx.y ? o1 : o0, rows, cols, accum, blockIdx.x);
 }
 
 static void colsum_partials(const float* p0, const float* p1, float* o0, float* o1, int rows, int cols, int accum,
@@ -365,6 +342,61 @@
     colsum_kernel<float><<<dim3((cols + 63) / 64), 256, 0, stream>>>(p0, cols, o0, rows, cols, accum);
     if (p1) colsum_kernel<float><<<dim3((cols + 63) / 64), 256, 0, stream>>>(p1, cols, o1, rows, cols, accum);
   }
+}
+
+extern "C" int uva_colsum_partials(const float* p0, const float* p1, float* o0, float* o1, int rows, int cols,
+                                   int accum, hipStream_t stream) {
+  if (cols <= 0) return 0;
+  if (rows < 0 || (rows && !p0) || !o0 || (p1 && !o1) || (cols % 4 == 0 && (((uintptr_t)p0 | (uintptr_t)p1) % 16)))
+    return (int)hipErrorInvalidValue;
+  colsum_partials(p0, p1, o0, o1, rows, cols, accum, stream);
+  UVA_LAUNCH_CHECK();
+  return 0;
+}
+
+__global__ __launch_bounds__(256) void colsum_group_kernel(const ColsumGroup g) {
+  const int bid = blockIdx.x;
+  int i = 0;
+  while (i + 1 < g.n && g.blk0[i + 1] <= bid) ++i;
+  const ColsumItem& it = g.it[i];
+  const int l = bid - g.blk0[i], nbx = (it.cols + 31) / 32;
+  if (it.kind == UVA_COLSUM_FINAL) {
+    colsum_final_body(it.p0, it.rows, it.cols, it.o0, it.accum, l);
+  } else {
+    const bool second = l >= nbx;
+    colsum_partials_body(second ? it.p1 : it.p0, second ? it.o1 : it.o0, it.rows, it.cols, it.accum,
+                         second ? l - nbx : l);
+  }
+}
+
+extern "C" int uva_colsum_group(const ColsumItem* items, int n, hipStream_t stream) {
+  if (n < 0 || n > COLSUM_GROUP_MAX || (n && !items)) return (int)hipErrorInvalidValue;
+  ColsumGroup g{};
+  int m = 0;
+  long long blocks = 0;
+  for (int i = 0; i < n; ++i) {
+    const ColsumItem& it = items[i];
+    if (it.cols <= 0) continue;
+    if (it.rows < 0 || (it.rows && !it.p0) || !it.o0 || ((uintptr_t)it.p0 % 4) || ((uintptr_t)it.o0 % 4))
+      return (int)hipErrorInvalidValue;
+    int nb = (it.cols + 31) / 32;
+    if (it.kind == UVA_COLSUM_PARTIALS) {
+      if (it.cols % 4 || ((uintptr_t)it.p0 % 16) || ((uintptr_t)it.p1 % 16) || (it.p1 && !it.o1))
+        return (int)hipErrorInvalidValue;
+      if (it.p1) nb *= 2;
+    } else if (it.kind != UVA_COLSUM_FINAL) {
+      return (int)hipErrorInvalidValue;
+    }
+    g.it[m] = it;
+    g.blk0[m++] = (int)blocks;
+    blocks += nb;
+  }
+  if (!m) return 0;
+  for (int i = m; i <= COLSUM_GROUP_MAX; ++i) g.blk0[i] = (int)blocks;
+  g.n = m;
+  colsum_group_kernel<<<dim3((unsigned)blocks), 256, 0, stream>>>(g);
+  UVA_LAUNCH_CHECK();
+  return 0;
 }
 
 template <typename T>
@@ -513,7 +545,7 @@
     return (int)hipErrorInvalidValue;
 #undef LNB_DY
   UVA_LAUNCH_CHECK();
-  if (dw) {
+  if (dw && accum_wb != UVA_COLSUM_DEFER) {
     colsum_partials(pw, db ? pb : nullptr, dw, db, nblk, D, accum_wb, stream);
     UVA_LAUNCH_CHECK();
   }
@@ -541,6 +573,7 @@
       x, w, nullptr, (const float*)nullptr, 0, (const bf16*)dy, mean, rstd, dx_base, dx, 0, (float*)nullptr,
       (float*)nullptr, pw, pb, rows, D, rpb, ld);
   UVA_LAUNCH_CHECK();
+  if (accum_wb == UVA_COLSUM_DEFER) return 0;
   colsum_partials(pw, pb, dw, db, nblk, D, accum_wb, stream);
   UVA_LAUNCH_CHECK();
   colsum_partials(pd, nullptr, dbias, nullptr, nblk, D, accum_dbias, stream);
diff --git a/unified_video_action_amd/model/autoregressive/functional.py b/unified_video_action_amd/model/autoregressive/functional.py
--- a/unified_video_action_amd/model/autoregressive/functional.py
+++ b/unified_video_action_amd/model/autoregressive/functional.py
@@ -65,11 +65,13 @@
             p._uva_shadow_t = t
         todo.append((p, w, t, key))
     side.wait_stream(torch.cuda.current_stream())
+    if not todo:
+        return
+    with torch.cuda.stream(side):
+        ops.transpose_bf16_batched([(w, t) for _, w, t, _ in todo])
+        ev = torch.cuda.Event()
+        ev.record(side)
     for p, w, t, key in todo:
-        with torch.cuda.stream(side):
-            ops.transpose_bf16(w, t)
-            ev = torch.cuda.Event()
-            ev.record(side)
         p._uva_shadow_t_ver = key
         p._uva_t_event = ev
 
@@ -337,6 +339,7 @@
         c = cdt()
         scale = (D // H) ** -0.5
         g2 = as_dtype(g2, F32)
+        grp = ops.ColsumGroup(dev) if c == torch.bfloat16 and RT.colsum_group else None
         ready = RT._drop_ready.pop(seeds[3], None)
         if ready is not None and ready[0] == g2.data_ptr() and ready[1].shape == (M, D):
             dpre2 = ready[1]
@@ -347,7 +350,8 @@
         Hd = fc1w.shape[0]
         dpre1 = torch.empty(M, Hd, dtype=c, device=dev)
         if c == torch.bfloat16 and RT.act_bwd_in_gemm and ops.linear_dgelu_drop(
-                dpre2, compute_weight_t(fc2w), pre1, dpre1, grad_buf(fc1b), p_proj, seeds[2], plane=ctx.plane1):
+                dpre2, compute_weight_t(fc2w), pre1, dpre1, grad_buf(fc1b), p_proj, seeds[2], plane=ctx.plane1,
+                group=grp):
             pass
         elif RT.act_bwd_in_gemm:
             ops.linear_dx_act(dpre2, compute_weight(fc2w), dpre1, pre1, "gelu", drop_p=p_proj, seed=seeds[2])
@@ -366,9 +370,9 @@
         dprep = torch.empty(M, D, dtype=c, device=dev)
         if not (c == torch.bfloat16 and RT.ln_bwd_drop and dh2.dtype == c and
                 ops.layernorm_bwd_drop(x1, n2w.detach(), dh2, m2, r2, g1, grad_buf(n2w), grad_buf(n2b), g2, dprep,
-                                       p_proj, seeds[1], grad_buf(projb))):
+                                       p_proj, seeds[1], grad_buf(projb), group=grp)):
             ops.layernorm_bwd(x1, n2w.detach(), dh2, m2, r2, g1, accum=False, dw=grad_buf(n2w), db=grad_buf(n2b),
-                              dx_base=g2)
+                              dx_base=g2, group=grp)
             ops.act_bwd_bias(None, g1, dprep, grad_buf(projb), "none", drop_p=p_proj, seed=seeds[1])
         del dh2
         ops.linear_dw(dprep, o, grad_buf(projw))
@@ -379,12 +383,12 @@
             dqkv = torch.empty(M, 3 * D, dtype=c, device=dev)
             dvec = torch.empty(B, H, N, dtype=F32, device=dev)
             ops.attn_bwd_hd(qkv, o, do, lse, dvec, dqkv, B, N, H, D // H, scale, p_attn, seeds[0], mask=Pd,
-                            dbias=grad_buf(qkvb) if RT.attn_bias_grad else None)
+                            dbias=grad_buf(qkvb) if RT.attn_bias_grad else None, group=grp)
         elif flash:
             dqkv = torch.empty(M, 3 * D, dtype=c, device=dev)
             dvec = torch.empty(B, H, N, dtype=F32, device=dev)
             ops.attn_bwd(qkv, o, do, lse, dvec, dqkv, B, N, H, scale, p_attn, seeds[0], mask=Pd,
-                         dbias=grad_buf(qkvb) if RT.attn_bias_grad else None)
+                         dbias=grad_buf(qkvb) if RT.attn_bias_grad else None, group=grp)
         else:
             dqkv = as_dtype(_attn_mat_bwd(qkv, P, Pd, do, B, N, H, scale, p_attn, seeds[0]), c)
         del do
@@ -400,13 +404,15 @@
             p_up, seed_up, fc2b_up = up
             d_up = torch.empty(M, D, dtype=c, device=dev)
             if ops.layernorm_bwd_drop(x, n1w.detach(), dh1, m1, r1, gx, grad_buf(n1w), grad_buf(n1b), g1, d_up,
-                                      p_up, seed_up, grad_buf(fc2b_up)):
+                                      p_up, seed_up, grad_buf(fc2b_up), group=grp):
                 RT._drop_ready[seed_up] = (gx.data_ptr(), d_up)
             else:
                 up = None
         if up is None or dh1.dtype != c:
             ops.layernorm_bwd(x, n1w.detach(), dh1, m1, r1, gx, accum=False, dw=grad_buf(n1w), db=grad_buf(n1b),
-                              dx_base=g1)
+                              dx_base=g1, group=grp)
+        if grp is not None:
+            grp.flush()
         if ctx.hook is not None:
             ctx.hook()
         return (gx,) + (None,) * 17
diff --git a/unified_video_action_amd/native/ops.py b/unified_video_action_amd/native/ops.py
--- a/unified_video_action_amd/native/ops.py
+++ b/unified_video_action_amd/native/ops.py
@@ -129,16 +129,20 @@
     return r == 1
 
 
-def linear_dgelu_drop(dy, wt, pre, dpre, dbias, drop_p=0.0, seed=0, accum_bias=True, plane=None):
+def linear_dgelu_drop(dy, wt, pre, dpre, dbias, drop_p=0.0, seed=0, accum_bias=True, plane=None, group=None):
     M, K = dy.shape
     N = wt.shape[0]
     assert dy.is_contiguous() and wt.is_contiguous() and pre.is_contiguous() and dpre.is_contiguous()
-    ws = workspace((M + 255) // 256 * 4 * N, dy.device)
+    nfl = (M + 255) // 256 * 4 * N
+    ws = workspace(nfl, dy.device) if group is None else group.buffer(nfl)
     with _traced(f"gemm+dgelu+drop bf16 M{M} N{N} K{K}", 2.0 * M * N * K):
-        r = lib().query("uva_linear_dgelu_drop", ptr(dy), ptr(wt), ptr(pre), ptr(dpre), ptr(dbias), int(accum_bias),
+        r = lib().query("uva_linear_dgelu_drop", ptr(dy), ptr(wt), ptr(pre), ptr(dpre), ptr(dbias),
+                        COLSUM_DEFER if group is not None else int(accum_bias),
                         ptr(ws), M, N, K, float(drop_p), int(seed) & 0xFFFFFFFFFFFFFFFF, ptr(plane), stream())
     if r < 0:
         raise RuntimeError(f"fused Mlp GEMM failed with hipError {-r}")
+    if r == 1 and group is not None:
+        group.final(ws, lib().query("uva_linear_dgelu_drop_part_rows", M), N, dbias, accum_bias)
     return r == 1
 
 
@@ -209,6 +213,60 @@
     _call("uva_colsum", dt(x), ptr(x), _ld(x), ptr(out), rows, cols, int(accum), ptr(ws), stream())
 
 
+COLSUM_FINAL, COLSUM_PARTIALS, COLSUM_DEFER = 0, 1, 2
+COLSUM_GROUP_MAX = 16
+
+
+class _ColsumItem(ctypes.Structure):
+    _fields_ = [("p0", ctypes.c_void_p), ("p1", ctypes.c_void_p), ("o0", ctypes.c_void_p), ("o1", ctypes.c_void_p),
+                ("rows", ctypes.c_int), ("cols", ctypes.c_int), ("accum", ctypes.c_int), ("kind", ctypes.c_int)]
+
+
+def colsum_group(items):
+    for i in range(0, len(items), COLSUM_GROUP_MAX):
+        chunk = items[i:i + COLSUM_GROUP_MAX]
+        arr = (_ColsumItem * len(chunk))()
+        for a, (kind, p0, p1, o0, o1, rows, cols, accum) in zip(arr, chunk):
+            for t in (p0, p1, o0, o1):
+                assert t is None or (t.dtype == torch.float32 and t.is_contiguous())
+            assert p0.numel() >= rows * cols and o0.numel() >= cols
+            assert (p1 is None) == (o1 is None) and (p1 is None or (p1.numel() >= rows * cols and o1.numel() >= cols))
+            assert kind == COLSUM_FINAL and p1 is None or kind == COLSUM_PARTIALS and cols % 4 == 0
+            a.p0, a.p1, a.o0, a.o1 = ptr(p0), ptr(p1), ptr(o0), ptr(o1)
+            a.rows, a.cols, a.accum, a.kind = int(rows), int(cols), int(bool(accum)), kind
+        _call("uva_colsum_group", ctypes.cast(arr, ctypes.c_void_p), len(chunk), stream())
+
+
+def colsum_final(part, nrows, cols, out, accum=True):
+    _call("uva_colsum_final", ptr(part), int(nrows), int(cols), ptr(out), int(bool(accum)), stream())
+
+
+def colsum_partials(p0, p1, o0, o1, rows, cols, accum=True):
+    _call("uva_colsum_partials", ptr(p0), ptr(p1), ptr(o0), ptr(o1), int(rows), int(cols), int(bool(accum)), stream())
+
+
+class ColsumGroup:
+
+    def __init__(self, device):
+        self.device, self.items, self.bufs = device, [], []
+
+    def buffer(self, n_floats):
+        t = torch.empty(max(int(n_floats), 1), dtype=torch.float32, device=self.device)
+        self.bufs.append(t)
+        return t
+
+    def final(self, part, nrows, cols, out, accum):
+        self.items.append((COLSUM_FINAL, part, None, out, None, nrows, cols, accum))
+
+    def partials(self, p0, p1, o0, o1, rows, cols, accum):
+        self.items.append((COLSUM_PARTIALS, p0, p1, o0, o1, rows, cols, accum))
+
+    def flush(self):
+        if self.items:
+            colsum_group(self.items)
+        self.items, self.bufs = [], []
+
+
 def layernorm_fwd(x, w, b, y, mean, rstd, eps=1e-6, scale=None, shift=None, ldm=0):
     rows, D = x.shape
     assert x.is_contiguous() and y.is_contiguous()
@@ -217,29 +275,40 @@
 
 
 def layernorm_bwd(x, w, dy, mean, rstd, dx, accum, dw=None, db=None, scale=None, ldm=0, dscale=None, dshift=None,
-                  out_dtype=None, accum_wb=True, dx_base=None, b=None):
+                  out_dtype=None, accum_wb=True, dx_base=None, b=None, group=None):
     rows, D = x.shape
     assert dy.dtype in (torch.float32, torch.bfloat16) and dx.dtype == torch.float32
     odt = out_dtype if out_dtype is not None else (dt(scale) if scale is not None else dt(x))
     ws = None
+    defer = group is not None and dw is not None and D % 4 == 0
     if dw is not None:
-        ws = workspace(lib().query("uva_layernorm_bwd_workspace", rows, D), x.device)
+        nfl = lib().query("uva_layernorm_bwd_workspace", rows, D)
+        ws = group.buffer(nfl) if defer else workspace(nfl, x.device)
     _call("uva_layernorm_bwd", dt(x), odt, ptr(x), ptr(w), ptr(b), ptr(scale), ldm, ptr(dy), dt(dy), ptr(mean),
                ptr(rstd),
-               ptr(dx_base), ptr(dx), int(accum), ptr(dscale), ptr(dshift), ptr(dw), ptr(db), int(accum_wb), ptr(ws), rows, D,
-               stream())
+               ptr(dx_base), ptr(dx), int(accum), ptr(dscale), ptr(dshift), ptr(dw), ptr(db),
+               COLSUM_DEFER if defer else int(accum_wb), ptr(ws), rows, D, stream())
+    if defer and rows > 0:
+        nblk = (rows + 63) // 64
+        group.partials(ws[:nblk * D], ws[nblk * D:2 * nblk * D] if db is not None else None, dw, db, nblk, D,
+                       accum_wb)
 
 
 def layernorm_bwd_drop(x, w, dy, mean, rstd, dx, dw, db, dx_base, drop_out, drop_p, seed, dbias, accum_wb=True,
-                       accum_dbias=True):
+                       accum_dbias=True, group=None):
     rows, D = x.shape
     if not (D == 768 and x.dtype == torch.float32 and dy.dtype == torch.bfloat16 and dx_base is not None
             and drop_out.dtype == torch.bfloat16 and drop_out.is_contiguous() and dx_base.is_contiguous()):
         return False
-    ws = workspace(3 * ((rows + 63) // 64) * D, x.device)
+    nblk = (rows + 63) // 64
+    ws = workspace(3 * nblk * D, x.device) if group is None else group.buffer(3 * nblk * D)
     _call("uva_layernorm_bwd_drop", ptr(x), ptr(w), ptr(dy), ptr(mean), ptr(rstd), ptr(dx_base), ptr(dx), ptr(dw),
-          ptr(db), int(accum_wb), ptr(drop_out), float(drop_p), int(seed) & 0xFFFFFFFFFFFFFFFF, ptr(dbias),
-          int(accum_dbias), ptr(ws), rows, D, stream())
+          ptr(db), COLSUM_DEFER if group is not None else int(accum_wb), ptr(drop_out), float(drop_p),
+          int(seed) & 0xFFFFFFFFFFFFFFFF, ptr(dbias), int(accum_dbias), ptr(ws), rows, D, stream())
+    if group is not None and rows > 0:
+        n = nblk * D
+        group.partials(ws[:n], ws[n:2 * n], dw, db, nblk, D, accum_wb)
+        group.partials(ws[2 * n:3 * n], None, dbias, None, nblk, D, accum_dbias)
     return True
 
 
@@ -260,6 +329,25 @@
     assert src.dtype == dst.dtype == torch.bfloat16 and src.is_contiguous() and dst.is_contiguous()
     assert tuple(dst.shape) == (C, R)
     _call("uva_transpose_bf16", ptr(src), ptr(dst), R, C, stream())
+
+
+TRANSPOSE_BATCH_MAX = 128
+
+
+class _TransposeItem(ctypes.Structure):
+    _fields_ = [("src", ctypes.c_void_p), ("dst", ctypes.c_void_p), ("rows", ctypes.c_int), ("cols", ctypes.c_int)]
+
+
+def transpose_bf16_batched(pairs):
+    for i in range(0, len(pairs), TRANSPOSE_BATCH_MAX):
+        chunk = pairs[i:i + TRANSPOSE_BATCH_MAX]
+        arr = (_TransposeItem * len(chunk))()
+        for a, (src, dst) in zip(arr, chunk):
+            R, C = src.shape
+            assert src.dtype == dst.dtype == torch.bfloat16 and src.is_contiguous() and dst.is_contiguous()
+            assert tuple(dst.shape) == (C, R)
+            a.src, a.dst, a.rows, a.cols = ptr(src), ptr(dst), R, C
+        _call("uva_transpose_bf16_batched", ctypes.cast(arr, ctypes.c_void_p), len(chunk), stream())
 
 
 def cast(src, dst):
@@ -473,7 +561,7 @@
 
 
 def attn_bwd(qkv, out, dout, lse2, dvec, dqkv, B, N, H, scale, drop_p=0.0, seed=0, mask=None, dbias=None,
-             accum_bias=True):
+             accum_bias=True, group=None):
     assert dout.dtype == torch.bfloat16 and dout.is_contiguous() and dqkv.is_contiguous()
     assert dout.numel() == B * N * H * 64 and dqkv.numel() == B * N * 3 * H * 64 and dvec.numel() == B * H * N
     with _traced(f"attn_bwd B{B} N{N} H{H}", 8.0 * B * H * N * N * 64):
@@ -481,10 +569,13 @@
             mask = attn_dropmask(B, N, H, drop_p, seed, qkv.device)
         if dbias is not None:
             assert dbias.dtype == torch.float32 and dbias.numel() == 3 * H * 64 and dbias.is_contiguous()
-            ws = workspace(B * ((N + 127) // 128) * 3 * H * 64, qkv.device)
+            nrows = B * ((N + 127) // 128)
+            ws = workspace(nrows * 3 * H * 64, qkv.device) if group is None else group.buffer(nrows * 3 * H * 64)
             _call("uva_attn_bwd_bias", ptr(qkv), ptr(out), ptr(dout), ptr(lse2), ptr(mask) if drop_p > 0 else None,
-                  ptr(dvec), ptr(dqkv), ptr(dbias), int(accum_bias), ptr(ws), B, N, H, float(scale), float(drop_p),
-                  stream())
+                  ptr(dvec), ptr(dqkv), ptr(dbias), COLSUM_DEFER if group is not None else int(accum_bias), ptr(ws),
+                  B, N, H, float(scale), float(drop_p), stream())
+            if group is not None:
+                group.final(ws, nrows, 3 * H * 64, dbias, accum_bias)
             return
         nb = lib().query("uva_attn_bwd_workspace", B, N, H, float(drop_p))
         ws = torch.empty(nb, dtype=torch.uint8, device=qkv.device) if nb else None
@@ -511,7 +602,7 @@
 
 
 def attn_bwd_hd(qkv, out, dout, lse2, dvec, dqkv, B, N, H, head_dim, scale, drop_p=0.0, seed=0, mask=None,
-                dbias=None, accum_bias=True):
+                dbias=None, accum_bias=True, group=None):
     hd = int(head_dim)
     assert dout.dtype == torch.bfloat16 and dout.is_contiguous() and dqkv.is_contiguous()
     assert attn_hd_supported(hd), f"head_dim {hd}: the fused kernels serve 80 and 128 (64: attn_bwd)"
@@ -524,10 +615,14 @@
         ws = None
         if dbias is not None:
             assert dbias.dtype == torch.float32 and dbias.numel() == 3 * H * hd and dbias.is_contiguous()
-            ws = workspace(lib().query("uva_attn_bwd_hd_part_floats", B, N, H, hd), qkv.device)
+            nfl = lib().query("uva_attn_bwd_hd_part_floats", B, N, H, hd)
+            ws = workspace(nfl, qkv.device) if group is None else group.buffer(nfl)
+        defer = group is not None and dbias is not None
         _call("uva_attn_bwd_hd", ptr(qkv), ptr(out), ptr(dout), ptr(lse2), ptr(mask) if drop_p > 0 else None,
-              ptr(dvec), ptr(dqkv), ptr(dbias), int(accum_bias), ptr(ws), B, N, H, hd, float(scale), float(drop_p),
-              stream())
+              ptr(dvec), ptr(dqkv), ptr(dbias), COLSUM_DEFER if defer else int(accum_bias), ptr(ws), B, N, H, hd,
+              float(scale), float(drop_p), stream())
+        if defer:
+            group.final(ws, B * ((N + 127) // 128), 3 * H * hd, dbias, accum_bias)
 
 
 def conv2d(x, w, out, Nimg, Hin, Win, Ci, Co, ks, stride, pad_t, pad_l, Hout, Wout, bias=None, residual=None,
diff --git a/unified_video_action_amd/runtime.py b/unified_video_action_amd/runtime.py
--- a/unified_video_action_amd/runtime.py
+++ b/unified_video_action_amd/runtime.py
@@ -17,6 +17,7 @@
         self.drop_planes = False
         self.attn_bias_grad = True
         self.ln_bwd_drop = True
+        self.colsum_group = True
         self.act_bwd_in_gemm = True
         self.trunk_act_bwd_in_gemm = False
         self._seed_base = 0x5EED
```

Measured after the change: 265.1 samples/s. About the same (-0.1%).
